# cbs228/sameold

Hardware: AMD Instinct MI355X
Metric: Msamples/s demodulated (batched 22.05 kHz channels) + % HBM roofline, 1/8 GPU (higher is better)
Workload: dtype f32

## Files before the change

### include/same_rx.h

```cpp
#ifndef SAME_RX_H
#define SAME_RX_H

#include <stddef.h>
#include <stdint.h>

#ifdef __cplusplus
extern "C" {
#endif

#define SAME_RX_ABI_VERSION 2

enum {
    SAME_OK = 0,
    SAME_EINVAL = -1,
    SAME_EDCLEN = -2,
    SAME_EAGCLIMITS = -3,
    SAME_EEQORDER = -4,
    SAME_ENODEVICE = -5,
    SAME_EHIP = -6,
    SAME_EOVERFLOW = -7,
    SAME_ENOMEM = -8,
    SAME_ERATE = -9,
    SAME_EKERNEL = -10
};
// ... 73 lines not shown
    SAME_BATCH_TRACE_SYMBOLS = 1u << 1,
    SAME_BATCH_GENERIC_KERNEL = 1u << 2,
    SAME_BATCH_TIME_PARALLEL = 1u << 3,
    SAME_BATCH_RELAXED = 1u << 4,
    SAME_BATCH_CALL_INVARIANT = 1u << 5,
    SAME_BATCH_MESSAGES_ONLY = 1u << 6
};
#define SAME_TP_EVENT_TOLERANCE_SYMBOLS 2

typedef struct same_batch same_batch;

int same_batch_new(const same_rx_builder *b, uint32_t n_channels, int device,
                   uint32_t flags, same_batch **out);
void same_batch_free(same_batch *rx);
int same_batch_reset(same_batch *rx);
int same_batch_reset_channels(same_batch *rx, const uint32_t *channels, size_t n);
uint64_t same_batch_channel_input_sample_counter(const same_batch *rx, uint32_t channel);
uint32_t same_batch_input_rate(const same_batch *rx);
uint32_t same_batch_n_channels(const same_batch *rx);
uint64_t same_batch_input_sample_counter(const same_batch *rx);
int same_batch_device(const same_batch *rx);

#define SAME_STREAM_OWN ((void *)(intptr_t)-1)
int same_batch_process_device(same_batch *rx, const float *d_x, size_t n_samples,
                              uint32_t layout, void *hip_stream);
int same_batch_set_call_window(same_batch *rx, uint32_t samples);
int same_batch_order_after(same_batch *rx, void *producer_stream);
int same_batch_process_device_i16(same_batch *rx, const int16_t *d_x, size_t n_samples,
                                  uint32_t layout, void *hip_stream);
int same_batch_process_host(same_batch *rx, const float *h_x, size_t n_samples, uint32_t layout);
int same_batch_process_host_i16(same_batch *rx, const int16_t *h_x, size_t n_samples, uint32_t layout);
int same_batch_process_device_ragged(same_batch *rx, const float *d_x, size_t n_rows, const uint32_t *counts,
                                     uint32_t layout, void *hip_stream);
int same_batch_process_device_ragged_i16(same_batch *rx, const int16_t *d_x, size_t n_rows, const uint32_t *counts,
                                         uint32_t layout, void *hip_stream);
int same_batch_process_host_ragged(same_batch *rx, const float *h_x, size_t n_rows, const uint32_t *counts, uint32_t layout);
int same_batch_process_host_ragged_i16(same_batch *rx, const int16_t *h_x, size_t n_rows, const uint32_t *counts,
                                       uint32_t layout);
int same_batch_flush(same_batch *rx);
int same_batch_sync(same_batch *rx);

int same_batch_poll_events(same_batch *rx, same_rx_event *out, size_t cap, size_t *n_out,
                           size_t *n_left);
size_t same_batch_pending_events(same_batch *rx);
int same_batch_peek_events(same_batch *rx, const same_rx_event **events, size_t *n);
int same_batch_drop_events(same_batch *rx, size_t n);
#define SAME_BURST_RECORD_BYTES 304
int same_batch_pack_bursts(same_batch *rx, uint32_t first_channel, uint8_t *out, size_t cap, size_t *n_records);

int same_batch_time_parallel_config(same_batch *rx, uint32_t max_chunks, uint32_t min_own_samples,
                                    uint32_t warmup_samples);
uint32_t same_batch_time_parallel_chunks(const same_batch *rx);
int same_batch_time_parallel_per_channel(const same_batch *rx);

int same_batch_transport_on_device(const same_batch *rx);

enum {
    SAME_AUDIO_FIRST = 1,
    SAME_AUDIO_END_MESSAGE = 2,
    SAME_AUDIO_END_FLUSH = 4,
    SAME_AUDIO_END_RESET = 8,
    SAME_AUDIO_TRUNCATED = 16
};
typedef struct same_audio_chunk {
    uint32_t channel, flags;
    uint64_t sample_counter;
    uint64_t n_samples;
    const float *samples;
} same_audio_chunk;
int same_batch_set_audio_capture(same_batch *rx, size_t samples_per_launch);
int same_batch_peek_audio(same_batch *rx, const same_audio_chunk **chunks, size_t *n);
int same_batch_drop_audio(same_batch *rx, size_t n);

typedef struct same_symbol_trace {
    uint64_t sample_counter;
    float zero, sym, err, samples_until_next_ted;
} same_symbol_trace;
int same_batch_read_trace(same_batch *rx, uint32_t channel, same_symbol_trace *out,
                          size_t cap, size_t *n_out);

int same_batch_last_kernel_ms(same_batch *rx, float *ms);
int same_batch_last_demod_kernel_ms(same_batch *rx, float *ms);
void same_batch_set_kernel_timing(same_batch *rx, int enable);
const char *same_batch_kernel_name(const same_batch *rx);

typedef struct same_rx same_rx;
int same_rx_build(const same_rx_builder *b, int device, same_rx **out);
void same_rx_free(same_rx *rx);
int same_rx_process(same_rx *rx, const float *x, size_t n, size_t *consumed, same_rx_event *ev);
int same_rx_flush(same_rx *rx, same_rx_event *msg);
int same_rx_reset(same_rx *rx);
uint32_t same_rx_input_rate(const same_rx *rx);
uint64_t same_rx_input_sample_counter(const same_rx *rx);

int same_synth_afsk_device(float *d_x, uint32_t n_channels, size_t n_samples,
                           uint32_t input_rate, uint64_t seed, float noise_sigma,
                           uint32_t flags, int device, void *hip_stream);
uint32_t same_synth_payload(uint64_t seed, uint32_t channel, uint8_t *out, uint32_t cap);
int same_synth_trials_device(float *d_x, uint32_t n_trials, uint32_t first_trial, size_t n_samples,
                             uint32_t input_rate, uint64_t seed, float ebn0_db_lo, float ebn0_db_step,
                             uint32_t n_grid, int device, void *hip_stream);

#ifdef __cplusplus
}
#endif
#endif
// ... 1 lines not shown
```

### sameold_amd/build.py

```python
from __future__ import annotations

import hashlib
import os
import re
import shutil
import subprocess
import sys

HERE = os.path.dirname(os.path.abspath(__file__))
CSRC = os.path.join(HERE, "csrc")
VARIANT = os.environ.get("SAME_BUILD_VARIANT", "")
LIB = os.path.join(HERE, f"libsame_rx.{VARIANT}.so" if VARIANT else "libsame_rx.so")
SOURCES = ["same_kernels.hip", "same_kernels_fast.hip", "same_kernels_pipe.hip", "same_kernels_relaxed.hip", "same_kernels_sym.hip", "same_kernels_sym_hi.hip", "same_synth.hip", "same_transport.hip", "same_capture.hip", "same_resample.hip", "same_batch.cpp", "same_select.cpp", "same_config.cpp", "same_transport.cpp", "same_place.cpp"]
SOURCE_FLAGS = {"same_kernels_sym_hi.hip": ["-mllvm", "-amdgpu-sched-strategy=max-ilp"],
                "same_kernels_pipe.hip": ["-mllvm", "-amdgpu-sched-strategy=max-ilp"]}
HEADERS = ["same_dev_common.h", "same_fast_common.h", "same_relaxed_common.h", "same_pipe_common.h", "same_profile.h", "same_device.h", "same_hipmem.h", "same_launch.h", "same_select.h", "same_config.h", "same_transport.h", "same_transport_dev.h", "same_capture_dev.h", "same_resets.h", "same_resample_dev.h", "same_resample_plan.h", "../../include/same_rx.h", "../../include/same_resample.h",
           "../../include/same_place.h", "samedec_main.cpp"]
SAMEDEC = os.path.join(HERE, "samedec_gpu")
ARCH = "gfx950"


def hipcc() -> str:
    for cand in (os.environ.get("HIPCC"), shutil.which("hipcc"), "/opt/rocm/bin/hipcc"):
        if cand and os.path.exists(cand):
            return cand
    raise RuntimeError("hipcc not found: the MI355X library cannot be built (there is no CPU build)")


def flags() -> list:
    return [
        f"--offload-arch={ARCH}", "-O3", "-std=c++17", "-fPIC",
        "-ffp-contract=off", "-fno-fast-math",
        "-fhip-fp32-correctly-rounded-divide-sqrt",
        "-fgpu-rdc" if False else "-fno-gpu-rdc",
        "-Wall", "-Wno-unused-function", "-Wno-unused-variable",
        "-x", "hip",
    ] + (["-DSAME_PROFILE=1"] if os.environ.get("SAME_PROFILE") else []) \
      + (["-DSAME_P3_MARKS=1"] if os.environ.get("SAME_P3_MARKS") else []) \
      + (["-DSAME_P1_SPLIT=1"] if os.environ.get("SAME_P1_SPLIT") else []) \
      + (["-DSAME_SYM_TL=1"] if os.environ.get("SAME_SYM_TL") else []) \
      + ([f"-DSYM_PRIOS=0x{os.environ['SAME_SYM_PRIOS']}"] if os.environ.get("SAME_SYM_PRIOS") else []) \
      + ([f"-DSYM_TL_GROUP={int(os.environ['SAME_SYM_TL_GROUP'])}u"] if os.environ.get("SAME_SYM_TL_GROUP") else []) \
      + [f"-D{d}" for d in os.environ.get("SAME_EXTRA_DEFS", "").split() if d] \
      + [f for f in os.environ.get("SAME_EXTRA_FLAGS", "").split() if f]


def source_hash() -> str:
    h = hashlib.sha256()
    for f in sorted(SOURCES + HEADERS):
        with open(os.path.join(CSRC, f), "rb") as fh:
            h.update(f.encode() + b"\0" + fh.read() + b"\0")
    h.update(" ".join(flags()).encode())
    h.update(repr(sorted(SOURCE_FLAGS.items())).encode())
    return h.hexdigest()


_MARK = re.compile(rb"SAME_SOURCE_HASH=([0-9a-f]{64})")


def built_hash(path: str = LIB):
    try:
        with open(path, "rb") as fh:
            m = _MARK.search(fh.read())
    except OSError:
        return None
    return m.group(1).decode() if m else None


def is_stale() -> bool:
# ... 55 lines not shown
```

### sameold_amd/csrc/same_batch.cpp

```cpp
#include <hip/hip_runtime.h>

#include <algorithm>
#include <chrono>
#include <cstdarg>
#include <cstdio>
#include <cstdlib>
#include <condition_variable>
#include <cstring>
#include <deque>
#include <functional>
#include <mutex>
#include <new>
#include <string>
#include <thread>
#include <utility>
#include <vector>

#include "../../include/same_rx.h"
#include "same_config.h"
#include "same_device.h"
#include "same_hipmem.h"
#include "same_launch.h"
#include "same_resets.h"
#include "same_transport.h"
// ... 145 lines not shown
                std::unique_lock<std::mutex> lk(mu_);
                cv_.wait(lk, [&] { return stop_ || generation_ != seen; });
                if (stop_) return;
                seen = generation_;
            }
            work();
        }
    }
    std::vector<std::thread> threads_;
    std::mutex mu_;
    std::condition_variable cv_, done_;
    const std::function<void(size_t)> *fn_ = nullptr;
    size_t next_ = 0, count_ = 0, pending_ = 0;
    uint64_t generation_ = 0;
    bool stop_ = false;
};

struct same_batch {
    same_rx_builder builder{};
    same::Params P{};
    same::State S{};
    int device = 0;
    uint32_t flags = 0;
    uint64_t counter = 0;
    hipStream_t own_stream = nullptr;
    hipStream_t last_stream = nullptr;
    same::DevBuf<float4> d_taps;
    same::DevBuf<void> d_state_blob;
    struct Slot {
        same::DevBuf<same::DevEvent> d_events;
        uint32_t event_cap() const { return (uint32_t)d_events.size(); }
        same::DevBuf<uint32_t> d_sort;
        same::PinnedBuf<uint32_t> h_sort;
        same::DevBuf<same::DevEvent> d_sorted;
        uint32_t sort_bins = 0;
        same::DevBuf<uint8_t> d_bursts;
        uint32_t burst_cap() const { return (uint32_t)(d_bursts.size() / same::kBurstCap); }
        same::DevBuf<uint32_t> d_counters;
        same::MappedBuf<uint32_t> h_counters;
        same::Event ev_start, ev_stop, ev_done, ev_planned;
        same::Event ev_k0, ev_k1;
        bool have_k = false;
        bool timed = false;
        same::PinnedBuf<void> h_events, h_bursts;
        bool in_flight = false;
        uint64_t seq = 0;
        uint64_t end_counter = 0;
        bool chunked = false;
        same::ChunkGeom geom{};
        uint64_t end_blocks = 0;
        same::DevBuf<uint64_t> d_handover;
        same::PinnedBuf<uint64_t> h_handover;
        bool per_channel = false;
        same::DevBuf<uint32_t> d_geom;
        same::PinnedBuf<uint32_t> h_geom;
        same::CoherentBuf<uint32_t> h_reset;
        same::CoherentBuf<uint32_t> h_counts;
        same::PinnedBuf<uint64_t> h_wake_up;
        bool dev_transport = false;
        same::CoherentBuf<same::DevMessage> h_near;
        uint32_t near_cap() const { return (uint32_t)h_near.size(); }
        same::DevBuf<same::DevMessage> d_msgs;
        uint32_t msg_cap() const { return (uint32_t)d_msgs.size(); }
        same::PinnedBuf<void> h_msgs;
        bool captured = false;
        same::DevBuf<same::cap::Span> d_spans;
        uint32_t span_cap() const { return (uint32_t)d_spans.size(); }
        same::DevBuf<float> d_pool;
        same::DevBuf<same::cap::Cursors> d_cap_cur;
        same::MappedBuf<same::cap::Cursors> h_cap_cur;
        same::PinnedBuf<void> h_spans, h_pool;
    } slot[2];
    struct TimePar {
        bool enabled = false;
        uint32_t max_chunks = 0, min_own = 0, warmup = 0;
        uint32_t cap_columns = 0;
        uint32_t carved_columns = 0;
        int carved_family = -1;
        same::Params Pv{};
        same::State Sv{};
        same::DevBuf<void> blob;
        same::DevBuf<void> blob_fresh;
        size_t fresh_bytes = 0;
        same::DevBuf<same::StateArrayDesc> d_desc_in, d_desc_out;
        uint32_t n_desc = 0;
        same::DevBuf<uint32_t> d_final_col;
        same::DevBuf<float> d_energy;
        same::DevBuf<float> d_hist;
        same::Event ev_plan_prev; bool plan_recorded = false;
        int knob_plan_stream = 0;
        int sort_mode = -1;
        uint32_t last_chunks = 1;
        bool last_per_channel = false;
        same::Family family = same::Family::kPipe;
        int knob_prologue = 0;
        std::vector<int64_t> sym_off;
        std::vector<TickSynth> synth;
    } tp;
    uint64_t launch_seq = 0;
    hipStream_t copy_stream = nullptr;
    struct Windowed {
        bool on = false;
        uint32_t window = 0;
        uint32_t fill = 0;
        same::DevBuf<void> d_buf;
        same::Event ev_buf;
        hipStream_t buf_stream = nullptr; bool buf_used = false;
        same::Event ev_read[2];
        uint64_t n_reads = 0;
        hipStream_t read_stream = nullptr;
    } inv;
    hipStream_t plan_stream = nullptr;
    float last_ms = 0.0f;
    bool overflowed = false;
    std::string record_path;
    bool kernel_fault = false;
    same::Request want;
    same::Mode mode;
    same::Choice plain;
    same::Params Pfm{};
    same::Family last_family = same::Family::kGeneric;
    bool sym_launched = false;
    bool debug = false;
    int host_threads = 0;
    same::DevBuf<void> d_stage, d_stage2;
    same::DevBuf<void> d_upload;
    same::DevBuf<void> d_zero;
    same::Event ev_order;
    bool timing = false;
    bool have_timing = false;
    float last_demod_ms = 0.0f;
    EventQueue queue;
    size_t queue_head = 0;
    ByteArena arena;
    std::vector<same_rx_event> peeked;
    bool peeked_valid = false;
    bool peeked_release = false;
    size_t peeked_head = 0;
    std::vector<size_t> burst_seq;
    size_t burst_seq_head = 0;
    std::vector<HarvestPart> parts;
    WorkerPool workers;
    std::vector<same::TransportHot> thot;
// ... 57 lines not shown

size_t carve_state(const same::Params &P, char *base, same::State &S)
{
    const size_t C = P.n_channels;
    Carver cv;
#define CARVE(field, type, count) \
    do { size_t o = cv.take<type>(count); if (base) S.field = reinterpret_cast<type *>(base + o); } while (0)
#define CARVE_ROWS(field, type, rows) CARVE(field, type, (size_t)(rows) * C);
    SAME_STATE_ARRAYS(CARVE_ROWS, P)
#undef CARVE_ROWS
    CARVE(fr_msg, uint8_t, (size_t)same::kBurstCap * C);
    if (P.trace_cap) {
        CARVE(trace_n, uint32_t, C);
        CARVE(trace, float, (size_t)P.trace_cap * 4 * C);
        CARVE(trace_idx, uint64_t, (size_t)P.trace_cap * C);
    }
#undef CARVE
    return (cv.off + 255) & ~size_t(255);
}

void list_state_arrays(const same::Params &P, const same::State &src, const same::State &dst,
                       std::vector<same::StateArrayDesc> &out)
{
    out.clear();
#define DESC_ROWS(field, type, rows)                                                                     \
    out.push_back(same::StateArrayDesc{reinterpret_cast<char *>(src.field), reinterpret_cast<char *>(dst.field), \
                                       (uint32_t)(rows), (uint32_t)(sizeof(type) / 4)});
    SAME_STATE_ARRAYS(DESC_ROWS, P)
#undef DESC_ROWS
    static_assert(same::kBurstCap % 4 == 0, "framer rows are copied in words");
    out.push_back(same::StateArrayDesc{reinterpret_cast<char *>(src.fr_msg), reinterpret_cast<char *>(dst.fr_msg), 1u,
                                       (uint32_t)(same::kBurstCap / 4)});
}

void read_knobs(same_batch *rx)
{
    auto num = [](const char *name, int unset) { const char *e = std::getenv(name); return e ? std::atoi(e) : unset; };
    auto tri = [](const char *name) { const char *e = std::getenv(name); return e ? (std::atoi(e) ? 1 : -1) : 0; };
    rx->P.knob_pipe = tri("SAME_PIPE");
    rx->P.knob_pipe_lanes = num("SAME_PIPE_LANES", 0);
    rx->P.knob_pipe_split = tri("SAME_PIPE_SPLIT");
#ifdef SAME_PROFILE
    rx->P.knob_mirror = tri("SAME_MIRROR");
    rx->P.knob_pipe_share = tri("SAME_PIPE_SHARE");
    rx->P.knob_prio = num("SAME_PIPE_PRIO", 0);
#endif
    rx->P.knob_fast_dense = tri("SAME_FAST_DENSE");
    rx->P.knob_sym = tri("SAME_SYM");
    rx->want.sym_max_channels = (uint32_t)std::max(0, num("SAME_SYM_MAX", 1 << 30));
    rx->debug = std::getenv("SAME_DEBUG") != nullptr;
    { const char *e = std::getenv("SAME_RECORD_HARVEST"); rx->record_path = e ? e : ""; }
    rx->host_threads = std::max(0, num("SAME_HOST_THREADS", 0));
    rx->tp.sort_mode = num("SAME_TP_SORT", -1);
    rx->tp.knob_plan_stream = tri("SAME_TP_PLAN_STREAM");
    rx->tp.knob_prologue = tri("SAME_TP_PROLOGUE");
    rx->want.knob_relaxed = tri("SAME_RELAXED");
    { const char *e = std::getenv("SAME_RELAXED_KERNEL"); rx->P.knob_relaxed_kernel = !e ? 0 : (std::strcmp(e, "solo") == 0 ? 1 : (std::strcmp(e, "duo") == 0 ? 2 : 0)); }
    { const char *e = std::getenv("SAME_TP_KERNEL"); rx->want.knob_tp_kernel = !e ? 0 : (std::strcmp(e, "wave") == 0 ? 2 : (std::strcmp(e, "pipe") == 0 ? 1 : 0)); }
}

int ensure_output(same_batch *rx, same_batch::Slot &sl, size_t n_samples, same::Output &O, size_t n_columns = 0)
{
    const size_t n_ch = n_columns ? n_columns : rx->P.n_channels;
    const double symbols = (double)n_samples * 520.83 / (double)rx->P.input_rate;
    const size_t per_chan_events = (size_t)(symbols / 8.0) + 16;
    const size_t per_chan_bursts = (size_t)(symbols / 160.0) + 4;
    size_t ecap = std::min<size_t>(per_chan_events * n_ch, 0x7fffffffu / sizeof(same::DevEvent));
    size_t bcap = std::min<size_t>(per_chan_bursts * n_ch, 0x7fffffffu / same::kBurstCap);
    HIP_TRY(sl.d_events.ensure(ecap));
    HIP_TRY(sl.d_bursts.ensure(bcap * same::kBurstCap));
    if (rx->dev_transport && !n_columns) {
        HIP_TRY(sl.d_msgs.ensure(std::min<size_t>(bcap + 2 * n_ch, 0x7fffffffu / sizeof(same::DevMessage))));
        if (!sl.h_near) HIP_TRY(sl.h_near.ensure(std::max<uint32_t>(4096u, (uint32_t)(n_ch / 4u))));
        if (rx->audio.per_launch)
            HIP_TRY(sl.d_spans.ensure(std::min<size_t>(n_ch + (size_t)sl.near_cap() + sl.msg_cap(), 0x7fffffffu / sizeof(same::cap::Span))));
    }
    HIP_TRY(sl.d_sorted.ensure(sl.d_events.size()));
    HIP_TRY(sl.d_sort.ensure(2 * n_ch + 1 + same::event_sort_extra_words((uint32_t)n_ch)));
    HIP_TRY(sl.h_sort.ensure(n_ch + 1));
    sl.sort_bins = (uint32_t)n_ch;
    O.events = sl.d_events; O.event_cap = sl.event_cap();
    O.bursts = sl.d_bursts; O.burst_cap = sl.burst_cap();
    O.n_events = sl.d_counters; O.n_bursts = sl.d_counters + 1; O.overflow = sl.d_counters + 2;
    return SAME_OK;
}

template <typename SampleT>
hipError_t launch_family(same::Family f, const same::Params &P, const same::State &S, const same::Output &O, const float4 *taps, const SampleT *x,
                         uint32_t n_blocks, uint64_t counter0, hipStream_t stream, const same::PipeChunks &pc = same::PipeChunks{})
{
    switch (f) {
    case same::Family::kSym: return same::launch_demod_sym(P, S, O, taps, x, n_blocks, counter0, stream, pc);
    case same::Family::kPipeFastmath: return same::launch_demod_pipe(P, S, O, taps, x, n_blocks, counter0, stream, pc, true);
    case same::Family::kPipe: return same::launch_demod_pipe(P, S, O, taps, x, n_blocks, counter0, stream, pc, false);
    case same::Family::kWaveRelaxed: return same::launch_demod_relaxed(P, S, O, taps, x, n_blocks, counter0, stream, pc);
    case same::Family::kFast: return same::launch_demod_fast(P, S, O, taps, x, n_blocks, counter0, stream);
    case same::Family::kGeneric: break;
    }
    return hipErrorInvalidValue;
}

void reset_channel_host(same_batch *rx, uint32_t c, uint64_t pos)
{
    if (!rx->thot.empty()) rx->tr(c).reset();
    if (rx->tp.enabled) {
        rx->tp.sym_off[c] = 0;
// ... 2 lines not shown
    }
    if (rx->h_wake) rx->h_wake[c] = 0;
}

int launch_pending_resets(same_batch *rx, same_batch::Slot &sl, hipStream_t stream)
{
    if (rx->resets.device.empty()) return SAME_OK;
    std::vector<uint32_t> &cols = rx->reset_cols;
    rx->resets.take_device(cols);
    const uint32_t n = (uint32_t)cols.size();
    if (n > sl.h_reset.size()) HIP_TRY(sl.h_reset.ensure(std::max<uint32_t>(256u, n + n / 2u)));
    std::memcpy(sl.h_reset, cols.data(), (size_t)n * sizeof(uint32_t));
    hipError_t e = same::launch_reset_columns(rx->P, rx->S, sl.h_reset.dev(), n, stream);
    if (e == hipSuccess && rx->dev_transport)
        e = same::launch_transport_reset(rx->d_thot, rx->d_tcold, rx->P.n_channels, sl.h_reset.dev(), n, 0, stream, rx->audio.d_rec);
    if (e != hipSuccess) return fail(SAME_EHIP, "channel reset launch failed: %s", hipGetErrorString(e));
    return SAME_OK;
}

void prepare_queue_append(same_batch *rx)
{
    rx->peeked_valid = false;
    release_stale_view(rx);
    if (rx->queue_head && rx->queue_head >= rx->queue.size() - rx->queue_head) {
        rx->queue_head = rx->queue.compact(rx->queue_head);
        size_t keep_from = rx->arena.base + rx->arena.size();
        for (size_t i = 0; i < rx->queue.size(); ++i)
            if (rx->queue.data()[i].n_bytes) { keep_from = (size_t)rx->queue.data()[i].payload; break; }
        rx->arena.compact(keep_from - rx->arena.base);
    }
}

struct HarvestTimes { std::chrono::steady_clock::time_point sorted, replayed; uint32_t n_threads = 1; };
struct HarvestInput {
    const uint32_t *first;
    same::DevEvent *events;
    const uint8_t *bursts;
    const uint64_t *handover;
    const uint32_t *geom;
};
int harvest_host(same_batch *rx, same_batch::Slot &sl, const HarvestInput &in, uint32_t n_events, uint32_t n_bursts, std::vector<uint32_t> &rearm,
                 HarvestTimes &times)
{
    const bool dbg = rx->debug;
    const same::DevEvent *evs = in.events;
    const uint8_t *bursts = in.bursts;
    const uint32_t n_ch = rx->P.n_channels;
    const uint32_t n_bins = sl.chunked ? sl.geom.n_chunks * n_ch : n_ch;
    std::vector<uint32_t> first(in.first, in.first + n_bins + 1u);
    same::DevEvent *evs_mut = in.events;
    const uint32_t n_real = first[n_bins];
    if (n_real > n_events) return fail(SAME_EHIP, "internal: event sort counted %u of %u events", n_real, n_events);
    struct Identity { uint32_t operator[](uint32_t i) const { return i; } } order;
    if (dbg && sl.chunked && sl.per_channel) {
        const same::ChunkGeom &g = sl.geom;
        const uint32_t *own = in.geom, *rows = in.geom + n_bins;
        double len_sum = 0, run_sum = 0; uint64_t len_max = 0, run_max = 0, n_len = 0, n_run = 0, n_inf = 0, n_late = 0;
        uint32_t worst_c = 0;
        for (uint32_t k = 0; k + 1u < g.n_chunks; ++k)
            for (uint32_t c = 0; c < n_ch; ++c) {
                const uint64_t end = own[(size_t)(k + 1u) * n_ch + c], len = end - rows[(size_t)k * n_ch + c];
                len_sum += (double)len; if (len > len_max) { len_max = len; worst_c = c; } ++n_len;
                const uint64_t h = in.handover[(size_t)k * n_ch + c];
                if (h == same::kNoHandover) { ++n_inf; continue; }
                const uint64_t run = h - g.counter0 > end ? h - g.counter0 - end : 0;
                run_sum += (double)run; run_max = std::max(run_max, run); ++n_run; n_late += run > 2u * g.block_len;
            }
        std::fprintf(stderr, "[same] longest piece on channel %u, its cuts:", worst_c);
        for (uint32_t k = 0; k < g.n_chunks; ++k) std::fprintf(stderr, " %u", own[(size_t)k * n_ch + worst_c]);
        std::fprintf(stderr, "\n");
        std::fprintf(stderr, "[same] per-channel chunks: length mean %.0f max %llu samples; run-on mean %.0f max %llu, %llu of %llu columns ran on "
                             "more than two blocks, %llu never handed over\n", len_sum / std::max<uint64_t>(n_len, 1), (unsigned long long)len_max,
                     run_sum / std::max<uint64_t>(n_run, 1), (unsigned long long)run_max, (unsigned long long)n_late, (unsigned long long)n_run,
                     (unsigned long long)n_inf);
    }
    std::vector<uint32_t> chan_first;
    if (sl.chunked) {
        chan_first.assign(n_ch + 1u, 0u);
        for (uint32_t k = 0; k < sl.geom.n_chunks; ++k)
            for (uint32_t c = 0; c < n_ch; ++c) chan_first[c + 1u] += first[k * n_ch + c + 1u] - first[k * n_ch + c];
        for (uint32_t c = 0; c < n_ch; ++c) chan_first[c + 1u] += chan_first[c];
    }
    const std::vector<uint32_t> &cfirst = sl.chunked ? chan_first : first;
    const bool link_only = (rx->flags & SAME_BATCH_LINK_ONLY) != 0;
    const bool tp = rx->tp.enabled;
    times.sorted = std::chrono::steady_clock::now();

    using Part = HarvestPart;
    const double sps = (double)rx->P.input_rate / 520.83;
    const uint64_t interburst = same::max_interburst_symbols(), history = same::max_history_duration();
    const bool msgs_only = rx->messages_only;
    auto push_transport = [&](Part &part, const same_rx_event &tev, uint32_t c) {
        if (msgs_only && tev.kind != SAME_TRANSPORT_MSG_START && tev.kind != SAME_TRANSPORT_MSG_END) return;
        QEvent q{};
        q.kind = tev.kind; q.channel = c; q.sample_counter = rx->resets.rebase(c, tev.sample_counter); q.symbol_count = tev.symbol_count;
        q.len = tev.len; q.aux = tev.aux; q.aux2 = tev.aux2;
        q.n_bytes = std::min<uint32_t>(tev.len, SAME_EVENT_MAX_BYTES);
        if (tev.kind != SAME_TRANSPORT_MSG_START) q.n_bytes = 0;
        q.payload = part.bytes.size();
        if (q.n_bytes) part.bytes.insert(part.bytes.end(), tev.bytes, tev.bytes + q.n_bytes);
        part.out.push_back(q);
    };
    auto feed = [&](Part &part, same_rx_event &tev, const same::DevEvent &d, uint32_t c, int64_t off) {
        const uint64_t sym = (uint64_t)((int64_t)d.symbol_count + off);
        auto poll = [&](uint64_t psym, uint64_t pt) {
            if (rx->tr(c).on_link_event(same::kDevTick, pt, psym, nullptr, 0, rx->P.input_rate, &tev)) push_transport(part, tev, c);
        };
        if (tp && !link_only) {
            HP(1);
            rx->tp.synth[c].run_until(sym, d.sample_counter, sps, rx->tr(c).force_eom_at(), poll);
        }
        QEvent q{};
        const uint8_t *payload = nullptr;
        {
        HP(2);
        q.kind = d.kind; q.channel = c; q.sample_counter = rx->resets.rebase(c, d.sample_counter); q.symbol_count = sym;
        if (d.kind == SAME_LINK_BURST) {
            q.len = d.burst_len;
            if (d.burst_slot < n_bursts) {
                q.n_bytes = std::min<uint32_t>(d.burst_len, SAME_EVENT_MAX_BYTES);
                payload = bursts + (size_t)d.burst_slot * same::kBurstCap;
                q.payload = part.bytes.size();
                if (!msgs_only) part.bytes.insert(part.bytes.end(), payload, payload + q.n_bytes);
            } else {
                q.len = 0;
            }
            if (!msgs_only) part.bursts.push_back((uint32_t)part.out.size());
        }
        if (d.kind <= SAME_LINK_BURST && !msgs_only) part.out.push_back(q);
        }
        if (!link_only) {
#ifdef SAME_HOST_PROF
            HpScope hp_tr(d.kind == SAME_LINK_BURST ? 3 : 4);
#endif
            if (rx->tr(c).on_link_event(d.kind, d.sample_counter, sym, payload, q.n_bytes, rx->P.input_rate, &tev)) push_transport(part, tev, c);
            if (!tp && rx->tr(c).force_eom_dirty()) part.rearm.push_back(c);
        }
        { HP(5); if (tp && d.kind <= SAME_LINK_BURST) rx->tp.synth[c].after_event(d.kind, sym, d.sample_counter, interburst, history); }
    };
    auto stitch = [&](Part &part, same_rx_event &ev, uint32_t c) {
        const same::ChunkGeom &g = sl.geom;
        const uint64_t *hand = in.handover;
        const uint32_t *own = sl.per_channel ? in.geom : nullptr, *rows = sl.per_channel ? in.geom + n_bins : nullptr;
        auto owner_of = [&](uint64_t h) -> uint32_t {
            if (!own) return g.owner_of(h);
            uint32_t k = 0;
            while (k + 1u < g.n_chunks && g.counter0 + own[(size_t)(k + 1u) * n_ch + c] <= h) ++k;
            return k;
        };
        TickSynth &ts = rx->tp.synth[c];
        int64_t off = rx->tp.sym_off[c];
        uint32_t cur = 0;
        uint64_t keep_after = 0;
        for (;;) {
            const uint32_t col = cur * n_ch + c;
            const uint64_t h = hand[col];
            const uint64_t upto = std::min(h, sl.end_blocks);
            bool rebased = cur == 0;
            for (uint32_t i = first[col]; i < first[col + 1u]; ++i) {
                const same::DevEvent &d = evs[order[i]];
                if (d.sample_counter <= keep_after) continue;
                if (d.sample_counter > upto) break;
                if (!rebased) {
                    const int64_t est = (int64_t)ts.a_sym + (int64_t)((double)(d.sample_counter - ts.a_t) / sps + 0.5);
                    off = est - (int64_t)d.symbol_count;
                    rebased = true;
                }
                feed(part, ev, d, c, off);
            }
            if (!rebased) {
                const uint64_t row0 = rows ? g.counter0 + rows[col] : g.counter0 + (uint64_t)cur * g.stride_blocks * g.block_len;
                const int64_t est_end = (int64_t)ts.a_sym + (int64_t)((double)(sl.end_blocks - ts.a_t) / sps + 0.5);
                off = est_end - (int64_t)((double)(sl.end_blocks - row0) / sps + 0.5);
            }
            if (h == same::kNoHandover) break;
            const uint32_t nxt = owner_of(h);
            if (nxt <= cur) break;
            const uint32_t ncol = nxt * n_ch + c;
            uint32_t st = 0, j = first[ncol];
            for (; j < first[ncol + 1u] && evs[order[j]].sample_counter <= h; ++j)
                if (evs[order[j]].kind <= SAME_LINK_BURST) st = evs[order[j]].kind;
            keep_after = h;
            if (st == SAME_LINK_READING || st == SAME_LINK_BURST) {
                for (; j < first[ncol + 1u]; ++j)
                    if (evs[order[j]].kind == SAME_LINK_NO_CARRIER) { keep_after = evs[order[j]].sample_counter; break; }
            } else if (st == SAME_LINK_SEARCHING && ts.link == SAME_LINK_NO_CARRIER) {
                same::DevEvent inj{};
                inj.channel = ncol; inj.kind = SAME_LINK_SEARCHING; inj.sample_counter = h;
                inj.symbol_count = ts.a_sym + (uint64_t)((double)(h > ts.a_t ? h - ts.a_t : 0) / sps + 0.5);
                inj.burst_slot = 0xffffffffu;
                feed(part, ev, inj, c, 0);
            }
            cur = nxt;
        }
        for (uint32_t i = first[c]; i < first[c + 1u]; ++i)
            if (evs[order[i]].sample_counter > sl.end_blocks) feed(part, ev, evs[order[i]], c, off);
        rx->tp.sym_off[c] = off;
    };
    auto run_range = [&](uint32_t c0, uint32_t c1, Part &part) {
        part.out.clear(); part.bytes.clear(); part.rearm.clear(); part.bursts.clear();
        part.out.reserve((size_t)(cfirst[c1] - cfirst[c0]) * 3 / 2 + 4);
        same_rx_event ev;
        std::memset(&ev, 0, sizeof(ev));
        for (uint32_t c = c0; c < c1; ++c) {
            if (!link_only && c + 1u < c1) {
                __builtin_prefetch(&rx->thot[c + 1u]);
                if (!sl.chunked) {
                    bool burst = false;
                    for (uint32_t k = first[c + 1u]; k < first[c + 2u]; ++k) burst |= evs[k].kind == SAME_LINK_BURST;
                    const char *nx = reinterpret_cast<const char *>(&rx->tcold[c + 1u]);
                    if (burst) for (size_t o = 0; o < sizeof(same::TransportCold); o += 64) __builtin_prefetch(nx + o);
                }
            }
            { HP(0);
            for (uint32_t col = c; col < n_bins; col += n_ch)
                if (first[col + 1u] - first[col] > 1u)
                    std::sort(evs_mut + first[col], evs_mut + first[col + 1u],
                              [](const same::DevEvent &a, const same::DevEvent &b) { return a.channel < b.channel; });
            }
            if (sl.chunked) stitch(part, ev, c);
            else
                for (uint32_t k = first[c]; k < first[c + 1u]; ++k)
                    feed(part, ev, evs[order[k]], c, tp ? rx->tp.sym_off[c] : 0);
            if (tp && !link_only) {
                TickSynth &ts = rx->tp.synth[c];
                if (ts.link == SAME_LINK_NO_CARRIER && sl.end_counter > ts.a_t) {
                    const uint64_t sym_end = ts.a_sym + (uint64_t)((double)(sl.end_counter - ts.a_t) / sps);
                    auto poll = [&](uint64_t psym, uint64_t pt) {
                        if (rx->tr(c).on_link_event(same::kDevTick, pt, psym, nullptr, 0, rx->P.input_rate, &ev)) push_transport(part, ev, c);
                    };
                    ts.run_until(sym_end + 1u, sl.end_counter + 1u, sps, rx->tr(c).force_eom_at(), poll);
                }
            }
        }
    };
    uint32_t n_threads = 1;
    if (n_real >= 16384u && n_ch >= 64u) {
        const unsigned hw = std::thread::hardware_concurrency();
        n_threads = std::min<uint32_t>({32u, std::max(16u, hw / 8u), hw ? hw : 1u, n_ch / 32u});
        if (rx->host_threads > 0) n_threads = (uint32_t)rx->host_threads;
    }
    if (rx->parts.size() < n_threads) rx->parts.resize(n_threads);
    std::vector<Part> &parts = rx->parts;
    for (Part &p : parts) { p.out.clear(); p.bytes.clear(); p.rearm.clear(); p.bursts.clear(); }
    if (n_threads == 1) {
        run_range(0, n_ch, parts[0]);
    } else {
        std::vector<uint32_t> cut(n_threads + 1u, n_ch);
        cut[0] = 0;
        for (uint32_t t = 1; t < n_threads; ++t) {
            const uint32_t target = (uint32_t)((uint64_t)n_real * t / n_threads);
            cut[t] = (uint32_t)(std::lower_bound(cfirst.begin(), cfirst.end(), target) - cfirst.begin());
            cut[t] = std::min(std::max(cut[t], cut[t - 1u]), n_ch);
        }
        rx->workers.run(n_threads, [&](size_t t) { run_range(cut[t], cut[t + 1u], parts[t]); });
    }
    times.replayed = std::chrono::steady_clock::now();
    times.n_threads = n_threads;
    size_t total = 0, total_bytes = 0;
    for (const Part &p : parts) { total += p.out.size(); total_bytes += p.bytes.size(); }
    prepare_queue_append(rx);
    QEvent *dst = rx->queue.grow(total);
    if (total && !dst) return fail(SAME_ENOMEM, "event queue");
    uint8_t *bdst = rx->arena.grow(total_bytes);
    if (total_bytes && !bdst) return fail(SAME_ENOMEM, "event payloads");
    {
        size_t at = 0, bat = 0;
        if (rx->burst_seq_head > 4096 && rx->burst_seq_head * 2 > rx->burst_seq.size()) {
            rx->burst_seq.erase(rx->burst_seq.begin(), rx->burst_seq.begin() + (std::ptrdiff_t)rx->burst_seq_head);
            rx->burst_seq_head = 0;
        }
        const size_t seq0 = rx->queue.base + (size_t)(dst - rx->queue.data());
        const size_t byte0 = rx->arena.base + (size_t)(bdst - rx->arena.data());
        struct Job { QEvent *q; uint8_t *b; Part *p; size_t byte_off; };
        std::vector<Job> jobs;
        for (size_t t = 0; t < parts.size(); ++t) {
            Part &p = parts[t];
            if (p.out.empty()) continue;
            for (uint32_t i : p.bursts) rx->burst_seq.push_back(seq0 + at + i);
            jobs.push_back(Job{dst + at, bdst + bat, &p, byte0 + bat});
            at += p.out.size(); bat += p.bytes.size();
        }
        rx->workers.run(jobs.size(), [&](size_t j) {
            const Job &job = jobs[j];
            for (QEvent &q : job.p->out) q.payload += job.byte_off;
            std::memcpy(job.q, job.p->out.data(), job.p->out.size() * sizeof(QEvent));
            if (!job.p->bytes.empty()) std::memcpy(job.b, job.p->bytes.data(), job.p->bytes.size());
        });
    }
    for (Part &p : parts) rearm.insert(rearm.end(), p.rearm.begin(), p.rearm.end());
    return SAME_OK;
}

struct HarvestFileHeader {
    uint64_t magic;
    uint32_t n_channels, n_bins, n_events, n_bursts, chunked, per_channel, flags, input_rate, tp_enabled, pad;
    same::ChunkGeom geom;
    uint64_t end_blocks, end_counter;
};
constexpr uint64_t kHarvestMagic = 0x3156524845'4d4153ull;
int record_harvest(same_batch *rx, same_batch::Slot &sl, uint32_t n_events, uint32_t n_bursts, const char *path)
{
    if (sl.seq != 3u) return SAME_OK;
    std::FILE *f = std::fopen(path, "wb");
    if (!f) return fail(SAME_EINVAL, "SAME_RECORD_HARVEST: cannot write %s", path);
    const uint32_t n_ch = rx->P.n_channels, n_bins = sl.chunked ? sl.geom.n_chunks * n_ch : n_ch;
    HarvestFileHeader h{};
    h.magic = kHarvestMagic;
    h.n_channels = n_ch; h.n_bins = n_bins; h.n_events = n_events; h.n_bursts = n_bursts;
    h.chunked = sl.chunked; h.per_channel = sl.per_channel; h.flags = rx->flags; h.input_rate = rx->P.input_rate; h.tp_enabled = rx->tp.enabled;
    h.geom = sl.geom; h.end_blocks = sl.end_blocks; h.end_counter = sl.end_counter;
    bool ok = std::fwrite(&h, sizeof(h), 1, f) == 1;
    ok = ok && std::fwrite(sl.h_sort, sizeof(uint32_t), (size_t)n_bins + 1, f) == (size_t)n_bins + 1;
    ok = ok && (!n_events || std::fwrite(sl.h_events, sizeof(same::DevEvent), n_events, f) == n_events);
    ok = ok && (!n_bursts || std::fwrite(sl.h_bursts, same::kBurstCap, n_bursts, f) == n_bursts);
    if (sl.chunked) {
        ok = ok && std::fwrite(sl.h_handover, sizeof(uint64_t), n_bins, f) == n_bins;
        if (sl.per_channel) ok = ok && std::fwrite(sl.h_geom, sizeof(uint32_t), (size_t)2 * n_bins, f) == (size_t)2 * n_bins;
    }
    std::fclose(f);
    return ok ? SAME_OK : fail(SAME_EINVAL, "SAME_RECORD_HARVEST: short write to %s", path);
}

hipError_t grow_pinned(same::PinnedBuf<void> &b, size_t need)
{
    return need <= b.size() ? hipSuccess : b.ensure(need + need / 2 + 4096);
}

AudioChunk *audio_grow(same_batch *rx, size_t n_chunks, size_t n_samples, float **samples_at, uint64_t *at)
{
    same_batch::Audio &A = rx->audio;
    if (A.head && A.head >= A.queue.size() - A.head) {
        A.head = A.queue.compact(A.head);
        const uint64_t keep_from = A.queue.size() ? A.queue.data()[0].at : A.samples.base + A.samples.size();
        A.samples.compact((size_t)(keep_from - A.samples.base));
    }
    AudioChunk *dst = A.queue.grow(n_chunks);
    if (n_chunks && !dst) return nullptr;
    float *sdst = A.samples.grow(n_samples);
    if (n_samples && !sdst) { A.queue.n -= n_chunks; return nullptr; }
    *samples_at = sdst;
    *at = A.samples.base + (A.samples.size() - n_samples);
    return dst;
}

int audio_end_reset(same_batch *rx, const std::vector<uint32_t> &chans, uint64_t pos)
{
    same_batch::Audio &A = rx->audio;
    if (!A.per_launch) return SAME_OK;
    size_t n = 0;
    for (uint32_t c : chans) n += A.open[c];
    if (!n) return SAME_OK;
    float *sdst = nullptr;
    uint64_t at = 0;
    AudioChunk *dst = audio_grow(rx, n, 0, &sdst, &at);
    if (!dst) return fail(SAME_ENOMEM, "audio queue");
    for (uint32_t c : chans) {
        if (!A.open[c]) continue;
        *dst++ = AudioChunk{c, SAME_AUDIO_END_RESET, rx->resets.rebase(c, pos), 0, at};
        A.open[c] = 0;
    }
    return SAME_OK;
}

int harvest_audio(same_batch *rx, same_batch::Slot &sl)
{
    sl.captured = false;
    same_batch::Audio &A = rx->audio;
    const same::cap::Cursors cur = *sl.h_cap_cur.get();
    if (cur.overflow) rx->overflowed = true;
    const uint32_t n_spans = std::min(cur.n_spans, sl.span_cap());
// ... 102 lines not shown
    const uint32_t C = rx->P.n_channels;
    HIP_TRY(sl.h_wake_up.ensure(C));
    same_batch::Slot &other = rx->slot[(&sl - rx->slot) ^ 1];
    const int oi = (int)(&other - rx->slot);
    for (uint32_t c = 0; c < C; ++c) {
        const uint64_t w = rx->h_wake[c];
        sl.h_wake_up[c] = w && other.in_flight ? w + rx->resets.pending_shift(oi, c) : w;
    }
    if (other.in_flight) {
        HIP_TRY(hipMemcpyAsync(rx->S.wake_sample, sl.h_wake_up, (size_t)C * sizeof(uint64_t), hipMemcpyHostToDevice, rx->last_stream));
        HIP_TRY(hipEventRecord(other.ev_done, rx->last_stream));
    } else {
        HIP_TRY(hipMemcpyAsync(rx->S.wake_sample, sl.h_wake_up, (size_t)C * sizeof(uint64_t), hipMemcpyHostToDevice, rx->copy_stream));
        HIP_TRY(hipStreamSynchronize(rx->copy_stream));
    }
    return SAME_OK;
}

int harvest_slot(same_batch *rx, same_batch::Slot &sl)
{
    if (!sl.in_flight) return SAME_OK;
    const bool dbg = rx->debug;
    auto t_begin = std::chrono::steady_clock::now();
    HIP_TRY(hipEventSynchronize(sl.ev_done));
    sl.in_flight = false;
    if (sl.timed) {
        HIP_TRY(hipEventElapsedTime(&rx->last_ms, sl.ev_start, sl.ev_stop));
        rx->last_demod_ms = rx->last_ms;
        if (sl.have_k) HIP_TRY(hipEventElapsedTime(&rx->last_demod_ms, sl.ev_k0, sl.ev_k1));
        rx->have_timing = true;
    }
    auto t_waited = std::chrono::steady_clock::now();
    const uint32_t n_events = std::min(sl.h_counters[0], sl.event_cap());
    if (dbg)
        std::fprintf(stderr, "[same] harvest: %u device events (%u bursts), cap %u/%u\n", sl.h_counters[0],
                     sl.h_counters[1], sl.event_cap(), sl.burst_cap());
    const uint32_t n_bursts = std::min(sl.h_counters[1], sl.burst_cap());
    if (sl.h_counters[2] & (3u | same::kMessageLogOverflow)) rx->overflowed = true;
    if (sl.h_counters[2] & 4u) rx->kernel_fault = true;
    if (sl.dev_transport) return harvest_messages(rx, sl, t_begin, t_waited);
    const size_t ev_bytes = (size_t)n_events * sizeof(same::DevEvent), bu_bytes = (size_t)n_bursts * same::kBurstCap;
    HIP_TRY(grow_pinned(sl.h_events, ev_bytes));
    HIP_TRY(grow_pinned(sl.h_bursts, bu_bytes));
    const uint32_t n_ch = rx->P.n_channels;
    const uint32_t n_bins = sl.chunked ? sl.geom.n_chunks * n_ch : n_ch;
    if (n_bins != sl.sort_bins) return fail(SAME_EINVAL, "internal: event sort made for %u columns, launch has %u", sl.sort_bins, n_bins);
    HIP_TRY(hipMemcpyAsync(sl.h_sort, sl.d_sort + n_bins, ((size_t)n_bins + 1) * sizeof(uint32_t), hipMemcpyDeviceToHost, rx->copy_stream));
    if (n_events) HIP_TRY(hipMemcpyAsync(sl.h_events, sl.d_sorted, ev_bytes, hipMemcpyDeviceToHost, rx->copy_stream));
    HIP_TRY(hipStreamSynchronize(rx->copy_stream));
    if (n_bursts) HIP_TRY(hipMemcpyAsync(sl.h_bursts, sl.d_bursts, bu_bytes, hipMemcpyDeviceToHost, rx->copy_stream));
    if (sl.chunked) {
        HIP_TRY(hipMemcpyAsync(sl.h_handover, sl.d_handover, (size_t)n_bins * sizeof(uint64_t), hipMemcpyDeviceToHost, rx->copy_stream));
        if (sl.per_channel)
            HIP_TRY(hipMemcpyAsync(sl.h_geom, sl.d_geom, (size_t)2 * n_bins * sizeof(uint32_t), hipMemcpyDeviceToHost, rx->copy_stream));
    }
    if (n_bursts || sl.chunked) HIP_TRY(hipStreamSynchronize(rx->copy_stream));
    auto t_copied = std::chrono::steady_clock::now();
    if (!rx->record_path.empty()) { const int rrc = record_harvest(rx, sl, n_events, n_bursts, rx->record_path.c_str()); if (rrc != SAME_OK) return rrc; }
    std::vector<uint32_t> rearm;
    HarvestTimes times;
    const HarvestInput in{sl.h_sort, static_cast<same::DevEvent *>(sl.h_events.get()), static_cast<const uint8_t *>(sl.h_bursts.get()),
                          sl.h_handover, sl.h_geom};
    int rc = harvest_host(rx, sl, in, n_events, n_bursts, rearm, times);
    if (rc) return rc;
    {
        const int si = (int)(&sl - rx->slot);
        const same::ResetLedger::SlotShift &sh = rx->resets.shift_due(si);
        if (!rx->thot.empty())
            for (size_t i = 0; i < sh.channels.size(); ++i)
                if (rx->tr(sh.channels[i]).shift_force_eom(sh.by[i])) rearm.push_back(sh.channels[i]);
        rx->resets.done_shift(si);
    }
    {
        const int si = (int)(&sl - rx->slot);
        const std::vector<uint32_t> &due = rx->resets.host_due(si);
        for (uint32_t c : due) reset_channel_host(rx, c, rx->resets.rec_pos(si));
        rx->resets.done_host(si);
    }
    if (!rearm.empty()) {
        if (!rx->h_wake) {
            HIP_TRY(rx->h_wake.ensure(rx->P.n_channels));
            std::memset(rx->h_wake, 0, (size_t)rx->P.n_channels * sizeof(uint64_t));
        }
        for (uint32_t c : rearm) rx->h_wake[c] = rx->tr(c).force_eom_at();
        if (rx->wake_ordered) {
            int rc2 = upload_wake_ordered(rx, sl);
            if (rc2) return rc2;
        } else {
        HIP_TRY(hipMemcpyAsync(rx->S.wake_sample, rx->h_wake, (size_t)rx->P.n_channels * sizeof(uint64_t), hipMemcpyHostToDevice, rx->copy_stream));
        HIP_TRY(hipStreamSynchronize(rx->copy_stream));
        }
    }
    if (dbg) {
        auto t_end = std::chrono::steady_clock::now();
        auto ms = [](auto a, auto b) { return std::chrono::duration<double, std::milli>(b - a).count(); };
        std::fprintf(stderr, "[same] harvest timing: wait %.2f ms, copy %.2f ms, sort %.2f ms, replay on %u threads %.2f ms, "
                             "queue %.2f ms\n",
                     ms(t_begin, t_waited), ms(t_waited, t_copied), ms(t_copied, times.sorted), times.n_threads,
                     ms(times.sorted, times.replayed), ms(times.replayed, t_end));
    }
    return SAME_OK;
}

int harvest(same_batch *rx)
{
    same_batch::Slot *order[2] = {&rx->slot[0], &rx->slot[1]};
    if (order[0]->seq > order[1]->seq) std::swap(order[0], order[1]);
    for (same_batch::Slot *sl : order) {
        int rc = harvest_slot(rx, *sl);
        if (rc) return rc;
// ... 81 lines not shown
    uint32_t m = 0;
    uint32_t row_off = 0;
};

struct RaggedLaunch {
    uint32_t row0 = 0;
    size_t n_lock = 0;
};


int begin_launch(same_batch *rx, same_batch::Slot &sl, const same_batch::Slot &prev, hipStream_t stream)
{
    int rc = harvest_slot(rx, sl);
    if (rc) return rc;
    if (prev.in_flight && rx->last_stream != stream) HIP_TRY(hipStreamWaitEvent(stream, prev.ev_done, 0));
    return launch_pending_resets(rx, sl, stream);
}

int begin_timing(same_batch *rx, same_batch::Slot &sl, hipStream_t stream)
{
    sl.timed = rx->timing;
    if (sl.timed) HIP_TRY(hipEventRecord(sl.ev_start, stream));
    return SAME_OK;
}

int tp_reserve(same_batch *rx, same_batch::Slot &sl, uint32_t columns, size_t n, const same::PipeChunks &pc, uint32_t block_len, same::Output &O)
{
    int rc = ensure_wide_state(rx, columns);
    if (rc) return rc;
    rc = ensure_output(rx, sl, std::min<size_t>(n, 3 * (size_t)pc.nominal_blocks * block_len + 65536), O, columns);
    if (rc) return rc;
    return ensure_handover(sl, columns);
}

int tp_start(same_batch *rx, same_batch::Slot &sl, uint32_t columns, const char *layout, hipStream_t stream, bool *sort_bins_empty)
{
    same_batch::TimePar &tp = rx->tp;
    const uint32_t C = rx->P.n_channels;
    *sort_bins_empty = false;
    if (tp.knob_prologue >= 0) {
        HIP_TRY(same::launch_tp_prologue(tp.blob, tp.blob_fresh, tp.fresh_bytes, sl.d_handover, sl.d_sort, columns, sl.d_counters, stream));
        *sort_bins_empty = sl.sort_bins == columns;
    } else {
        HIP_TRY(same::launch_counters(sl.d_counters, sl.h_counters.dev(), 0, stream));
        HIP_TRY(same::launch_init_state(tp.Pv, tp.Sv, 0, stream, C));
        HIP_TRY(same::launch_fill_u64(sl.d_handover, columns, same::kNoHandover, stream));
    }
    if (rx->debug) std::fprintf(stderr, "[same] time-parallel launch: %u columns (%s), start-up: %s\n", columns, layout,
                                tp.knob_prologue >= 0 ? "prologue kernel" : "separate launches");
    HIP_TRY(same::launch_copy_state_columns(tp.d_desc_in, tp.n_desc, C, columns, nullptr, C, stream));
    return SAME_OK;
}

int tp_hand_back(same_batch *rx, same_batch::Slot &sl, const same::ChunkGeom &geom, const uint32_t *own_start, hipStream_t stream)
{
    same_batch::TimePar &tp = rx->tp;
    const uint32_t C = rx->P.n_channels;
    if (own_start) HIP_TRY(same::launch_chunk_final_column_pc(sl.d_handover, own_start, C, geom.n_chunks, rx->counter, tp.d_final_col, stream));
    else HIP_TRY(same::launch_chunk_final_column(sl.d_handover, C, geom, tp.d_final_col, stream));
    HIP_TRY(same::launch_copy_state_columns(tp.d_desc_out, tp.n_desc, geom.n_chunks * C, C, tp.d_final_col, C, stream));
    return SAME_OK;
}

template <typename SampleT>
int demod_tail(same_batch *rx, const same::Output &O, const SampleT *rows, size_t n, uint64_t counter0, hipStream_t stream)
{
    const hipError_t e = same::launch_demod(rx->P, rx->S, O, rx->d_taps, rows, (uint32_t)n, counter0, stream);
    if (e != hipSuccess) return fail(SAME_EHIP, "demod kernel launch failed: %s", hipGetErrorString(e));
    return SAME_OK;
}
int demod_tail_corner(same_batch *rx, const same::Output &O, const float *corner, size_t pitch, size_t r, uint64_t counter0, hipStream_t stream)
{
    const uint32_t C = rx->P.n_channels;
    HIP_TRY(rx->d_stage.ensure(r * C * sizeof(float)));
    HIP_TRY(rx->d_stage2.ensure(r * C * sizeof(float)));
    float *staged = static_cast<float *>(rx->d_stage.get()), *rows = static_cast<float *>(rx->d_stage2.get());
    HIP_TRY(hipMemcpy2DAsync(staged, r * sizeof(float), corner, pitch * sizeof(float), r * sizeof(float), C, hipMemcpyDeviceToDevice, stream));
    const hipError_t e = same::launch_transpose(staged, rows, C, (uint32_t)r, stream);
    if (e != hipSuccess) return fail(SAME_EHIP, "demod kernel launch failed: %s", hipGetErrorString(e));
    return demod_tail(rx, O, rows, r, counter0, stream);
}

template <typename SampleT>
int end_launch(same_batch *rx, same_batch::Slot &sl, same_batch::Slot &prev, hipStream_t stream, const SampleT *rows, size_t n,
               bool sort_bins_empty, const RaggedLaunch *rl = nullptr)
{
    if (sl.timed) HIP_TRY(hipEventRecord(sl.ev_stop, stream));
    HIP_TRY(same::launch_event_sort(sl.d_events, sl.d_counters, sl.event_cap(), sl.sort_bins, sl.d_sort, sl.d_sort + sl.sort_bins,
                                    sl.d_sorted, stream, sort_bins_empty));
    sl.dev_transport = rx->dev_transport && !sl.chunked;
    rx->last_dev_transport = sl.dev_transport;
    if (sl.dev_transport) {
        same::TransportLaunch T{};
        T.n_channels = rx->P.n_channels; T.input_rate = rx->P.input_rate;
        T.first = sl.d_sort + sl.sort_bins; T.sorted = sl.d_sorted; T.counters = sl.d_counters;
        T.bursts = sl.d_bursts; T.burst_cap = sl.burst_cap();
        T.hot = rx->d_thot; T.cold = rx->d_tcold; T.wake_sample = rx->S.wake_sample;
        T.near = sl.h_near.dev(); T.near_cap = sl.near_cap();
        T.log = sl.d_msgs; T.log_cap = sl.msg_cap(); T.log_cursor = sl.d_counters + 3; T.overflow = sl.d_counters + 2;
        sl.captured = rx->audio.per_launch != 0;
        if (sl.captured) {
            same::cap::Launch &K = T.cap;
            const uint64_t fa = rx->audio.flush_at;
            K.start = rx->counter; K.n_rows = (uint32_t)n;
            K.flush_row = fa >= rx->counter + n ? same::cap::kNoFlush : (uint32_t)(fa > rx->counter ? fa - rx->counter : 0);
            K.rec = rx->audio.d_rec; K.spans = sl.d_spans; K.span_cap = sl.span_cap();
            K.n_spans = &sl.d_cap_cur->n_spans; K.pool_used = &sl.d_cap_cur->pool_used; K.pool_cap = rx->audio.per_launch;
            K.overflow = &sl.d_cap_cur->overflow;
        }
        if (rl && rl->n_lock < n)
            HIP_TRY(same::launch_transport_ragged(T, sl.h_counts.dev(), rl->row0, (uint32_t)n, stream));
// ... 17 lines not shown
}

template <typename SampleT>
int process_time_major_launches(same_batch *rx, const SampleT *d_x, size_t n_samples, hipStream_t stream, const Ragged *rg = nullptr)
{
    const size_t kMaxChunk = std::min<size_t>((size_t)1 << 22, (size_t)rx->P.input_rate * 45);
    size_t done = 0;
    while (done < n_samples) {
        const size_t n = std::min(kMaxChunk, n_samples - done);
        same_batch::Slot &sl = rx->slot[rx->launch_seq & 1];
        same_batch::Slot &prev = rx->slot[(rx->launch_seq & 1) ^ 1];
        int rc = begin_launch(rx, sl, prev, stream);
        if (rc) return rc;
        size_t n_lock = n;
        if (rg) {
            const size_t row0 = (size_t)rg->row_off + done;
            n_lock = rg->m > row0 ? std::min<size_t>(rg->m - row0, n) : 0;
            const uint32_t C = rx->P.n_channels;
            HIP_TRY(sl.h_counts.ensure(C));
            std::memcpy(sl.h_counts, rg->counts, (size_t)C * sizeof(uint32_t));
            rx->ragged_by.resize(C);
            for (uint32_t c = 0; c < C; ++c) {
                const size_t have = rg->counts[c] > row0 ? std::min<size_t>(rg->counts[c] - row0, n) : 0;
                rx->ragged_by[c] = (uint32_t)(n - have);
            }
        }
        same::ChunkGeom geom{};
        same::PipeChunks pc{};
        const uint32_t n_chunks = rg ? 1u : plan_chunks(rx, n, geom, pc);
        rx->tp.last_chunks = n_chunks;
        sl.have_k = false;
        bool sort_bins_empty = false;
        same::Output O{};
        if (n_chunks > 1u) {
            const uint32_t C = rx->P.n_channels, columns = n_chunks * C;
            const size_t fbk = geom.block_len;
            rc = tp_reserve(rx, sl, columns, n, pc, geom.block_len, O);
            if (rc) return rc;
            pc.handover = sl.d_handover;
            same_batch::TimePar &tp = rx->tp;
            rc = begin_timing(rx, sl, stream);
            if (rc) return rc;
            rc = tp_start(rx, sl, columns, "time-major", stream, &sort_bins_empty);
            if (rc) return rc;
            const SampleT *xp = d_x + done * C;
            const uint32_t total_blocks = (uint32_t)(n / fbk);
            const hipError_t e = launch_family(tp.family, tp.Pv, tp.Sv, O, rx->d_taps, xp, total_blocks, rx->counter, stream, pc);
            rx->last_family = tp.family;
            if (e != hipSuccess) return fail(SAME_EHIP, "time-parallel demod kernel launch failed: %s", hipGetErrorString(e));
            rc = tp_hand_back(rx, sl, geom, nullptr, stream);
            if (rc) return rc;
            const size_t n_whole = (size_t)total_blocks * fbk;
            if (n_whole < n && (rc = demod_tail(rx, O, xp + n_whole * C, n - n_whole, rx->counter + n_whole, stream)) != SAME_OK) return rc;
            sl.chunked = true; sl.per_channel = false;
            sl.geom = geom;
            sl.end_blocks = rx->counter + n_whole;
            rx->tp.last_per_channel = false;
        } else {
        sl.chunked = false; sl.per_channel = false;
        rc = ensure_output(rx, sl, n, O);
        if (rc) return rc;
        HIP_TRY(same::launch_counters(sl.d_counters, sl.h_counters.dev(), 0, stream));
        rc = begin_timing(rx, sl, stream);
        if (rc) return rc;
        const SampleT *xp = d_x + done * rx->P.n_channels;
        hipError_t e = hipSuccess;
        const same::Choice &plain = rx->plain;
        const size_t fb = plain.block_len;
        const size_t n_fast = fb ? (n_lock / fb) * fb : 0;
        if (n_fast) {
            e = launch_family(plain.family, same::is_fastmath(plain.family) ? rx->Pfm : rx->P, rx->S, O, rx->d_taps, xp, (uint32_t)(n_fast / fb), rx->counter, stream);
            if (e != hipSuccess) return fail(SAME_EHIP, "%s launch failed: %s", same::family_name(plain.family, rx->P.block_len), hipGetErrorString(e));
            rx->sym_launched |= plain.family == same::Family::kSym;
        }
        rx->last_family = plain.family == same::Family::kSym && !rx->sym_launched ? same::Family::kPipeFastmath : plain.family;
        if (n_fast < n_lock &&
            (rc = demod_tail(rx, O, xp + n_fast * rx->P.n_channels, n_lock - n_fast, rx->counter + n_fast, stream)) != SAME_OK) return rc;
        if (n_lock < n) {
            e = same::launch_demod_ragged(rx->P, rx->S, O, rx->d_taps, xp + n_lock * rx->P.n_channels, (uint32_t)(n - n_lock), sl.h_counts.dev(),
                                          (uint32_t)(rg->row_off + done + n_lock), rx->counter + n_lock, stream);
            if (e != hipSuccess) return fail(SAME_EHIP, "ragged demod kernel launch failed: %s", hipGetErrorString(e));
        }
        }
        const RaggedLaunch rl{rg ? (uint32_t)(rg->row_off + done) : 0u, n_lock};
        rc = end_launch(rx, sl, prev, stream, d_x + done * rx->P.n_channels, n, sort_bins_empty, rg ? &rl : nullptr);
        if (rc) return rc;
        done += n;
    }
    return SAME_OK;
}

constexpr uint32_t kInvWindow = 18432;
constexpr uint32_t kInvWindowTimeParallel = 73728;
static int inv_buffer_wait(same_batch *rx, hipStream_t stream)
{
    same_batch::Windowed &iv = rx->inv;
    if (iv.buf_used && iv.buf_stream != stream) HIP_TRY(hipStreamWaitEvent(stream, iv.ev_buf, 0));
    return SAME_OK;
}
static int inv_buffer_done(same_batch *rx, hipStream_t stream)
{
    same_batch::Windowed &iv = rx->inv;
    HIP_TRY(iv.ev_buf.ensure());
    HIP_TRY(hipEventRecord(iv.ev_buf, stream));
    iv.buf_stream = stream; iv.buf_used = true;
    return SAME_OK;
}
static int inv_copy(const float *d_x, float *dst, size_t n, hipStream_t stream)
{
    HIP_TRY(hipMemcpyAsync(dst, d_x, n * sizeof(float), hipMemcpyDeviceToDevice, stream));
    return SAME_OK;
}
// ... 49 lines not shown
{
    same_batch::Windowed &iv = rx->inv;
    if (iv.n_reads) HIP_TRY(hipEventSynchronize(iv.ev_read[(iv.n_reads - 1) & 1]));
    return SAME_OK;
}
template <typename SampleT>
int process_time_major(same_batch *rx, const SampleT *d_x, size_t n_samples, hipStream_t stream)
{
    same_batch::Windowed &iv = rx->inv;
    if (!iv.on) return process_time_major_launches(rx, d_x, n_samples, stream);
    const size_t C = rx->P.n_channels;
    size_t pos = 0;
    if (iv.fill) {
        const size_t take = std::min<size_t>(iv.window - iv.fill, n_samples);
        int rc = inv_append(rx, d_x, take, stream);
        if (rc) return rc;
        pos = take;
        if (iv.fill < iv.window) return SAME_OK;
        rc = inv_launch_waiting(rx, stream);
        if (rc) return rc;
    }
    while (n_samples - pos >= iv.window) {
        int rc = process_time_major_launches(rx, d_x + pos * C, iv.window, stream);
        if (rc) return rc;
        pos += iv.window;
    }
    if (pos < n_samples) return inv_append(rx, d_x + pos * C, n_samples - pos, stream);
    return SAME_OK;
}

int process_channel_major_native(same_batch *rx, const float *d_x, size_t n, hipStream_t stream)
{
    same_batch::TimePar &tp = rx->tp;
    if (!tp.enabled || n > ((size_t)1 << 22)) return 0;
    if (rx->P.ntaps != 42u) return 0;
    same::ChunkGeom geom{};
    same::PipeChunks pc{};
    const uint32_t n_chunks = plan_chunks(rx, n, geom, pc, same::tp_native_column_cap(rx->P, rx->mode, tp.max_chunks), true);
    if (n_chunks < 2u) return 0;
    const uint32_t C = rx->P.n_channels, columns = n_chunks * C, fb = geom.block_len;
    const bool wave = tp.family == same::Family::kWaveRelaxed;
    const same::Params Pv = same::wide_params(rx->P, columns, same::is_fastmath(tp.family), true);
    const size_t n_call = n;
    n -= n % fb;
    if (n_call % 4 != 0 || ((uintptr_t)d_x & 15u) != 0u || n < 64u * (size_t)same::tp_scout_block() || n / same::tp_scout_block() > 7000u || n_chunks > 63u || C % same::kWave != 0u) return 0;
    if (wave ? fb % 2 != 0 : (fb % 4 != 0 || same::pipe_workgroup_channels(Pv) != (uint32_t)same::kWave)) return 0;
    same_batch::Slot &sl = rx->slot[rx->launch_seq & 1];
    same_batch::Slot &prev = rx->slot[(rx->launch_seq & 1) ^ 1];
    int rc = begin_launch(rx, sl, prev, stream);
    if (rc) return rc;
    same::Output O{};
    rc = tp_reserve(rx, sl, columns, n, pc, fb, O);
    if (rc) return rc;
    HIP_TRY(sl.d_geom.ensure((size_t)5 * columns + 3 * (columns / same::kWave)));
    HIP_TRY(sl.h_geom.ensure((size_t)2 * columns));
    same::TpPlan plan{};
    plan.channels = C; plan.n_chunks = n_chunks; plan.block_len = fb;
    {
        const double sps = (double)rx->P.input_rate / 520.83;
        const uint32_t warm = tp.warmup ? tp.warmup : (uint32_t)(40.0 * sps + 0.5);
        plan.warmup_samples = std::min(geom.warmup_blocks, (warm + fb - 1u) / fb) * fb;
    }
    plan.whole_samples = (uint32_t)n; plan.in_samples = n_call;
    plan.scout_blocks = (uint32_t)(n / same::tp_scout_block());
    HIP_TRY(tp.d_energy.ensure((size_t)C * plan.scout_blocks));
    uint32_t *d_own = sl.d_geom, *d_row0 = sl.d_geom + columns, *d_nom = sl.d_geom + 2 * (size_t)columns,
             *d_perm = sl.d_geom + 3 * (size_t)columns, *d_wg = sl.d_geom + 4 * (size_t)columns,
             *d_wg2 = d_wg + columns / same::kWave, *d_perm2 = d_wg2 + 2 * (columns / same::kWave);
    const bool pair_groups = tp.sort_mode == 2 && tp.family == same::Family::kSym;
    const int sort_mode = pair_groups ? 0 : (tp.sort_mode >= 0 ? (tp.sort_mode ? 1 : 0) : (same::tp_more_than_one_round(columns) ? 1 : 0));
    rc = begin_timing(rx, sl, stream);
    if (rc) return rc;
    const bool lpt = sort_mode != 0 || pair_groups;
    const bool side = stream == rx->own_stream && tp.knob_plan_stream >= 0;
    hipStream_t ps = side ? rx->plan_stream : stream;
    if (tp.plan_recorded) HIP_TRY(hipStreamWaitEvent(ps, tp.ev_plan_prev, 0));
    HIP_TRY(same::launch_tp_plan(d_x, plan, tp.d_energy, d_own, d_row0, d_nom, d_perm, d_wg, sort_mode != 0, ps,
                                 lpt ? d_perm2 : nullptr, lpt ? d_wg2 : nullptr, pair_groups));
    HIP_TRY(tp.ev_plan_prev.ensure());
    HIP_TRY(hipEventRecord(tp.ev_plan_prev, ps));
    tp.plan_recorded = true;
    if (side) {
        HIP_TRY(hipEventRecord(sl.ev_planned, ps));
        HIP_TRY(hipStreamWaitEvent(stream, sl.ev_planned, 0));
    }
    if (lpt) { d_perm = d_perm2; d_wg = d_wg2; }
    bool sort_bins_empty = false;
    rc = tp_start(rx, sl, columns, "channel-major", stream, &sort_bins_empty);
    if (rc) return rc;
    pc.handover = sl.d_handover;
    pc.col_row0 = d_row0; pc.col_nominal = d_nom; pc.wg_blocks = d_wg; pc.col_perm = (sort_mode != 0 || pair_groups) ? d_perm : nullptr;
    pc.in_samples = n_call; pc.whole_samples = (uint32_t)n;
    pc.hist_scratch = nullptr;
    if (pc.col_perm && tp.family == same::Family::kSym) {
        HIP_TRY(tp.d_hist.ensure((size_t)columns * same::kSquelchHist));
        pc.hist_scratch = tp.d_hist;
    }
    sl.have_k = sl.timed;
    if (sl.timed) HIP_TRY(hipEventRecord(sl.ev_k0, stream));
    const hipError_t e = launch_family(tp.family, tp.Pv, tp.Sv, O, rx->d_taps, d_x, (uint32_t)(n / fb), rx->counter, stream, pc);
    rx->last_family = tp.family;
    if (e != hipSuccess) return fail(SAME_EHIP, "time-parallel demod kernel launch failed: %s", hipGetErrorString(e));
    if (sl.timed) HIP_TRY(hipEventRecord(sl.ev_k1, stream));
    rc = tp_hand_back(rx, sl, geom, d_own, stream);
    if (rc) return rc;
    if (n < n_call && (rc = demod_tail_corner(rx, O, d_x + n, n_call, n_call - n, rx->counter + n, stream)) != SAME_OK) return rc;
    sl.chunked = true; sl.per_channel = true;
    sl.geom = geom;
    sl.end_blocks = rx->counter + n;
    tp.last_chunks = n_chunks; tp.last_per_channel = true;
    rc = end_launch<float>(rx, sl, prev, stream, nullptr, n_call, sort_bins_empty);
    return rc ? rc : 1;
}
int process_channel_major_native(same_batch *, const int16_t *, size_t, hipStream_t) { return 0; }

template <typename SampleT, typename Launch>
int transpose_in_slabs(same_batch *rx, const SampleT *d_x, size_t pitch, size_t n_rows, hipStream_t stream, Launch &&launch)
{
    const uint32_t C = rx->P.n_channels;
    for (same_batch::Slot &sl : rx->slot)
        if (sl.in_flight && rx->last_stream != stream) HIP_TRY(hipStreamWaitEvent(stream, sl.ev_done, 0));
    const size_t slab = std::min<size_t>(n_rows, (size_t)65520);
    HIP_TRY(rx->d_stage2.ensure(slab * C * sizeof(SampleT)));
    for (size_t t0 = 0; t0 < n_rows; t0 += slab) {
        const size_t n = std::min(slab, n_rows - t0);
        HIP_TRY(rx->d_stage.ensure(n * C * sizeof(SampleT)));
        SampleT *staged = static_cast<SampleT *>(rx->d_stage.get()), *rows = static_cast<SampleT *>(rx->d_stage2.get());
        HIP_TRY(hipMemcpy2DAsync(staged, n * sizeof(SampleT), d_x + t0, pitch * sizeof(SampleT), n * sizeof(SampleT), C,
                                 hipMemcpyDeviceToDevice, stream));
        const hipError_t e = same::launch_transpose(staged, rows, C, (uint32_t)n, stream);
        if (e != hipSuccess) return fail(SAME_EHIP, "transpose launch failed: %s", hipGetErrorString(e));
        const int rc = launch(rows, n, t0);
        if (rc) return rc;
    }
    return SAME_OK;
}

template <typename SampleT>
int process_device_on(same_batch *rx, const SampleT *d_x, size_t n_samples, uint32_t layout, hipStream_t stream);
template <typename SampleT>
int process_device_any(same_batch *rx, const SampleT *d_x, size_t n_samples, uint32_t layout, void *hip_stream)
{
    if (!rx || (!d_x && n_samples)) return fail(SAME_EINVAL, "null argument");
    if (n_samples == 0) return SAME_OK;
    HIP_TRY(hipSetDevice(rx->device));
    hipStream_t stream = hip_stream == SAME_STREAM_OWN ? rx->own_stream : (hipStream_t)hip_stream;
    if (!rx->inv.on) return process_device_on(rx, d_x, n_samples, layout, stream);
    int rc = inv_reads_begin(rx, stream);
    if (rc == SAME_OK) rc = process_device_on(rx, d_x, n_samples, layout, stream);
    const int rc_end = inv_reads_end(rx, stream);
    return rc ? rc : rc_end;
}
template <typename SampleT>
int process_device_on(same_batch *rx, const SampleT *d_x, size_t n_samples, uint32_t layout, hipStream_t stream)
{
    if (layout == SAME_LAYOUT_TIME_MAJOR) return process_time_major(rx, d_x, n_samples, stream);
    if (layout != SAME_LAYOUT_CHANNEL_MAJOR) return fail(SAME_EINVAL, "unknown layout %u", layout);
    const int done = rx->inv.on ? 0 : process_channel_major_native(rx, d_x, n_samples, stream);
    if (done) return done < 0 ? done : SAME_OK;
    return transpose_in_slabs(rx, d_x, n_samples, n_samples, stream,
// ... 550 lines not shown
}

int same_batch_read_trace(same_batch *rx, uint32_t channel, same_symbol_trace *out, size_t cap, size_t *n_out)
{
    if (!rx || !n_out) return fail(SAME_EINVAL, "null argument");
    if (!rx->P.trace_cap) return fail(SAME_EINVAL, "batch was not created with SAME_BATCH_TRACE_SYMBOLS");
    if (channel >= rx->P.n_channels) return fail(SAME_EINVAL, "channel out of range");
    HIP_TRY(hipSetDevice(rx->device));
    int rc = harvest(rx);
    if (rc) return rc;
    uint32_t n = 0;
    HIP_TRY(hipMemcpy(&n, rx->S.trace_n + channel, sizeof(n), hipMemcpyDeviceToHost));
    n = std::min(n, rx->P.trace_cap);
    n = (uint32_t)std::min<size_t>(n, cap);
    std::vector<float> f((size_t)n * 4);
    std::vector<uint64_t> idx(n);
    if (n) {
        HIP_TRY(hipMemcpy(f.data(), rx->S.trace + (size_t)channel * rx->P.trace_cap * 4, f.size() * sizeof(float), hipMemcpyDeviceToHost));
        HIP_TRY(hipMemcpy(idx.data(), rx->S.trace_idx + (size_t)channel * rx->P.trace_cap, n * sizeof(uint64_t), hipMemcpyDeviceToHost));
    }
    for (uint32_t i = 0; i < n; ++i) {
        out[i].sample_counter = idx[i];
        out[i].zero = f[4 * i]; out[i].sym = f[4 * i + 1]; out[i].err = f[4 * i + 2];
        out[i].samples_until_next_ted = f[4 * i + 3];
    }
    *n_out = n;
    return SAME_OK;
}

void same_batch_set_kernel_timing(same_batch *rx, int enable) { if (rx) { rx->timing = enable != 0; rx->have_timing = false; } }
int same_batch_last_kernel_ms(same_batch *rx, float *ms)
{
    if (!rx || !ms) return fail(SAME_EINVAL, "null argument");
    if (!rx->have_timing) return fail(SAME_EINVAL, "no timed launch yet");
    *ms = rx->last_ms;
    return SAME_OK;
}
int same_batch_last_demod_kernel_ms(same_batch *rx, float *ms)
{
    if (!rx || !ms) return fail(SAME_EINVAL, "null argument");
    if (!rx->have_timing) return fail(SAME_EINVAL, "no timed launch yet");
    *ms = rx->last_demod_ms;
    return SAME_OK;
}
int same_batch_time_parallel_config(same_batch *rx, uint32_t max_chunks, uint32_t min_own_samples, uint32_t warmup_samples)
{
    if (!rx) return fail(SAME_EINVAL, "null handle");
    if (!rx->tp.enabled) return fail(SAME_EINVAL, "batch was not created with SAME_BATCH_TIME_PARALLEL");
    rx->tp.max_chunks = max_chunks; rx->tp.min_own = min_own_samples; rx->tp.warmup = warmup_samples;
    return SAME_OK;
}
uint32_t same_batch_time_parallel_chunks(const same_batch *rx) { return rx ? rx->tp.last_chunks : 0; }
int same_batch_transport_on_device(const same_batch *rx) { return rx && rx->last_dev_transport ? 1 : 0; }
int same_batch_time_parallel_per_channel(const same_batch *rx) { return rx && rx->tp.last_chunks > 1u && rx->tp.last_per_channel ? 1 : 0; }

const char *same_batch_kernel_name(const same_batch *rx)
{
    return rx ? same::family_name(rx->last_family, rx->P.block_len) : "";
}


long same_debug_harvest_replay(const char *path, int threads, int reps, double *ms_out)
{
    if (!path || reps <= 0 || !ms_out) return -(long)fail(SAME_EINVAL, "null argument");
    std::FILE *f = std::fopen(path, "rb");
    if (!f) return -(long)fail(SAME_EINVAL, "cannot read %s", path);
    HarvestFileHeader h{};
    bool ok = std::fread(&h, sizeof(h), 1, f) == 1 && h.magic == kHarvestMagic && h.n_bins >= h.n_channels && h.n_channels > 0;
    std::vector<uint32_t> first, geom;
    std::vector<same::DevEvent> ev0, ev;
    std::vector<uint8_t> bursts;
    std::vector<uint64_t> hand0, hand;
    if (ok) {
        first.resize((size_t)h.n_bins + 1); ev0.resize(h.n_events); bursts.resize((size_t)h.n_bursts * same::kBurstCap);
        ok = std::fread(first.data(), sizeof(uint32_t), first.size(), f) == first.size();
        ok = ok && (!h.n_events || std::fread(ev0.data(), sizeof(same::DevEvent), h.n_events, f) == h.n_events);
        ok = ok && (!h.n_bursts || std::fread(bursts.data(), same::kBurstCap, h.n_bursts, f) == h.n_bursts);
        if (ok && h.chunked) {
            hand0.resize(h.n_bins);
            ok = std::fread(hand0.data(), sizeof(uint64_t), h.n_bins, f) == h.n_bins;
            if (ok && h.per_channel) { geom.resize((size_t)2 * h.n_bins); ok = std::fread(geom.data(), sizeof(uint32_t), geom.size(), f) == geom.size(); }
        }
    }
    std::fclose(f);
    if (ok) {
        ok = first[h.n_bins] <= h.n_events && h.n_bins % h.n_channels == 0;
        for (size_t i = 0; ok && i < (size_t)h.n_bins; ++i) ok = first[i] <= first[i + 1];
        for (size_t i = 0; ok && i < ev0.size(); ++i)
            ok = (ev0[i].burst_slot == 0xffffffffu || ev0[i].burst_slot < h.n_bursts) && (ev0[i].kind == same::kDevEventNone || ev0[i].kind <= 8u);
        if (ok && h.chunked) {
            ok = h.geom.n_chunks >= 1 && (uint64_t)h.geom.n_chunks * h.n_channels == h.n_bins && h.geom.block_len >= 1 && h.geom.stride_blocks >= 1;
            for (size_t i = 0; ok && h.per_channel && i < geom.size(); ++i) ok = geom[i] <= 0x7fffffffu;
        } else if (ok) {
            ok = h.n_bins == h.n_channels;
        }
    }
    if (!ok) return -(long)fail(SAME_EINVAL, "%s is not a (consistent) harvest record", path);
    same_batch *rx = new (std::nothrow) same_batch;
    if (!rx) return -(long)fail(SAME_ENOMEM, "out of memory");
    rx->P.n_channels = h.n_channels; rx->P.input_rate = h.input_rate; rx->flags = h.flags;
    if (std::getenv("SAME_REPLAY_LINK_ONLY")) rx->flags |= SAME_BATCH_LINK_ONLY;
    rx->tp.enabled = h.tp_enabled != 0; rx->host_threads = threads;
    if (!(h.flags & SAME_BATCH_LINK_ONLY)) { rx->thot.resize(h.n_channels); rx->tcold.resize(h.n_channels); }
    if (rx->tp.enabled) { rx->tp.sym_off.assign(h.n_channels, 0); rx->tp.synth.assign(h.n_channels, TickSynth{}); }
    rx->resets.init(h.n_channels);
    same_batch::Slot &sl = rx->slot[0];
    ev = ev0; hand = hand0;
    const HarvestInput in{first.data(), ev.data(), bursts.data(), hand.data(), geom.data()};
    sl.chunked = h.chunked != 0; sl.per_channel = h.per_channel != 0; sl.sort_bins = h.n_bins;
    const uint64_t span = h.end_counter - h.geom.counter0;
    const double sps = (double)h.input_rate / 520.83;
    const uint64_t span_sym = (uint64_t)((double)span / sps);
    long produced = 0;
    int rc = SAME_OK;
    for (int r = 0; r < reps && rc == SAME_OK; ++r) {
        const uint64_t dt = span * (uint64_t)r, ds = span_sym * (uint64_t)r;
        for (size_t i = 0; i < ev0.size(); ++i) { ev[i] = ev0[i]; ev[i].sample_counter += dt; if (!sl.chunked) ev[i].symbol_count += ds; }
        for (size_t i = 0; i < hand0.size(); ++i) hand[i] = hand0[i] == same::kNoHandover ? hand0[i] : hand0[i] + dt;
        sl.geom = h.geom; sl.geom.counter0 += dt;
        sl.end_blocks = h.end_blocks + dt; sl.end_counter = h.end_counter + dt;
        std::vector<uint32_t> rearm;
        HarvestTimes times;
        const auto t0 = std::chrono::steady_clock::now();
        rc = harvest_host(rx, sl, in, h.n_events, h.n_bursts, rearm, times);
        ms_out[r] = std::chrono::duration<double, std::milli>(std::chrono::steady_clock::now() - t0).count();
        produced = (long)(rx->queue.size() - rx->queue_head);
        rx->queue_head = rx->queue.size();
        rx->burst_seq_head = rx->burst_seq.size();
    }
#ifdef SAME_HOST_PROF
    { uint64_t tot = 0; for (int k = 0; k < 7; ++k) tot += g_hp[k];
      for (int k = 0; k < 7; ++k) std::fprintf(stderr, "[same prof] %-24s %8.3f Mclk per harvest (%4.1f %% of the instrumented parts)\n", g_hp_name[k], (double)g_hp[k] / reps / 1e6, tot ? 100.0 * (double)g_hp[k] / (double)tot : 0.0); }
#endif
    delete rx;
    return rc == SAME_OK ? produced : -(long)rc;
}

}

struct same_rx {
    same_batch *batch = nullptr;
    uint64_t reported = 0;
    uint64_t zeros_until = 0;
    std::deque<same_rx_event> events;
};

static int rx_pump(same_rx *rx)
{
    same_rx_event buf[64];
    for (;;) {
        size_t n = 0, left = 0;
        int rc = same_batch_poll_events(rx->batch, buf, 64, &n, &left);
        if (rc) return rc;
        for (size_t i = 0; i < n; ++i) rx->events.push_back(buf[i]);
        if (!left) return SAME_OK;
    }
}

extern "C" {

int same_rx_build(const same_rx_builder *b, int device, same_rx **out)
{
// ... 113 lines not shown
```

### sameold_amd/csrc/same_device.h

```cpp
#pragma once

#include <stddef.h>
#include <stdint.h>

namespace same {

constexpr int kWave = 64;
constexpr int kMaxEqTaps = 16;
constexpr int kBurstCap = 288;
constexpr int kSquelchHist = 64;
constexpr int kMaxTaps = 512;

struct Params {
    uint32_t n_channels;
    uint32_t input_rate;
    uint32_t dc_len;
    float dc_inv_len;
    float dc_k;
    float agc_bw, agc_min, agc_max, agc_gain0;
    uint32_t ntaps;
    uint32_t win_ring;
    float samples_per_ted, period_min, period_max;
    float alpha_unlocked, beta_unlocked, alpha_locked, beta_locked;
    uint32_t sync_word, sq_max_errors;
// ... 32 lines not shown
    F_EQ_BITS_SHIFT = 16,
    F_EQ_BITS_MASK = 0xffu << 16,
};
constexpr int kTickRing = 8;

struct State {
    float *dc_ff_ring;
    float *dc_fb_ring;
    float *dc_sum0, *dc_sum1;
    float *agc_gain;
    float *win_ring;
    uint32_t *ted_clock;
    float *until_next_ted;
    float *ted_h0, *ted_h1, *ted_h2;
    float *period_avg, *period_inst;
    uint32_t *sq_data;
    float *sq_power;
    uint32_t *sq_phist;
    uint32_t *sq_fill;
    int32_t *sq_clock;
    uint64_t *sq_symbols;
    float *sq_hist;
    float *eq_ffc, *eq_fbc;
    float *eq_ffw, *eq_fbw;
    uint32_t *eq_word, *eq_count;
    float *eq_snap_ffc, *eq_snap_fbc, *eq_snap_ffw, *eq_snap_fbw;
    uint32_t *fr_word, *fr_count, *fr_invalid, *fr_len;
    uint8_t *fr_msg;
    uint32_t *flags;
    uint64_t *tk_next;
    uint64_t *tk_last;
    uint64_t *tk_ring;
    uint32_t *tk_n;
    uint64_t *wake_sample;
    uint64_t *wake_fired;
    uint32_t *trace_n;
    float *trace;
    uint64_t *trace_idx;
};

struct PipeChunks {
    uint32_t n_chunks;
    uint32_t in_channels;
    uint32_t stride_blocks;
    uint32_t nominal_blocks;
    uint64_t *handover;
    const uint32_t *col_row0;
    const uint32_t *col_nominal;
    const uint32_t *wg_blocks;
    const uint32_t *col_perm;
    float *hist_scratch;
    uint64_t in_samples;
    uint32_t whole_samples;
};

struct ChunkGeom {
    uint64_t counter0;
    uint32_t n_chunks, block_len, stride_blocks, warmup_blocks;
#if defined(__HIPCC__)
    __host__ __device__
#endif
    uint32_t owner_of(uint64_t h) const
    {
        const uint64_t blocks = (h - counter0) / block_len;
        if (blocks < warmup_blocks) return 0u;
        const uint64_t k = (blocks - warmup_blocks) / stride_blocks;
        return k >= n_chunks ? n_chunks - 1u : (uint32_t)k;
    }
#if defined(__HIPCC__)
    __host__ __device__
#endif
    uint64_t own_start(uint32_t k) const
    { return k == 0u ? counter0 : counter0 + ((uint64_t)k * stride_blocks + warmup_blocks) * block_len; }
};
constexpr uint64_t kNoHandover = ~0ull;

struct StateArrayDesc { char *src; char *dst; uint32_t rows; uint32_t elem_words; };

constexpr uint32_t kDevEventNone = 0xffffffffu;
struct DevEvent {
    uint32_t channel;
    uint32_t kind;
    uint64_t sample_counter;
    uint64_t symbol_count;
    uint32_t burst_len;
    uint32_t burst_slot;
};

constexpr uint32_t kDevMessageText = 272;
struct DevMessage {
    uint32_t channel;
    uint32_t kind;
    uint64_t sample_counter;
    uint64_t symbol_count;
    uint32_t len, aux, aux2;
    uint32_t seq;
    uint8_t text[kDevMessageText];
};

struct Output {
    DevEvent *events;
    uint32_t *n_events;
    uint32_t event_cap;
    uint8_t *bursts;
    uint32_t *n_bursts;
    uint32_t burst_cap;
// ... 5 lines not shown
```

### sameold_amd/csrc/same_kernels.hip

```cpp
#include <hip/hip_runtime.h>

#include <algorithm>

#include "same_dev_common.h"
#include "same_device.h"
#include "same_launch.h"

namespace same {

template <int B, typename SampleT>
__global__ __launch_bounds__(kWave) void demod_kernel(Params P, State S, Output O,
                                                      const float4 *__restrict__ taps,
                                                      const SampleT *__restrict__ x,
                                                      uint32_t n_samples, uint64_t counter0)
{
    extern __shared__ float lds[];
    const uint32_t lane = threadIdx.x;
    const uint32_t C = P.n_channels;
    const uint32_t c_raw = blockIdx.x * kWave + lane;
    if (c_raw >= C) return;
    const uint32_t c = c_raw;
    const uint32_t DL = P.dc_len;
    float *ff = lds;
    float *fb = lds + DL * kWave;
    float *win = lds + 2 * DL * kWave;
    const uint32_t wmask = P.win_ring - 1u;

    uint32_t dpos = (uint32_t)(counter0 % DL);
    uint32_t wpos = (uint32_t)(counter0 & wmask);

    for (uint32_t i = 0; i < DL; ++i) {
        ff[i * kWave + lane] = S.dc_ff_ring[i * C + c];
        fb[i * kWave + lane] = S.dc_fb_ring[i * C + c];
    }
    for (uint32_t i = 0; i < P.win_ring; ++i) win[i * kWave + lane] = S.win_ring[i * C + c];

    Lane L;
    lane_load(L, S, c);
    GlobalCtx X{S, c, C};

    for (uint32_t t0 = 0; t0 < n_samples; t0 += B) {
        const uint32_t nb = min((uint32_t)B, n_samples - t0);
        float xs[B];
#pragma unroll
        for (int k = 0; k < B; ++k)
            xs[k] = (k < (int)nb) ? (float)x[(size_t)(t0 + k) * C + c] : 0.0f;

        float ys[B];
        int fire_k = -1;
        float fire_rem = 0.0f, fire_gain = 0.0f;
        const float unlocked0 = (L.flags & F_AGC_LOCKED) ? 0.0f : 1.0f;
#pragma unroll
        for (int k = 0; k < B; ++k) {
            if (k < (int)nb) {
                const uint32_t dnext = (dpos + 1u == DL) ? 0u : dpos + 1u;
                float aged0 = ff[dpos * kWave + lane];
                ff[dpos * kWave + lane] = xs[k];
                float d0 = xs[k] - aged0;
                L.sum0 += d0;
// ... 385 lines not shown

hipError_t launch_reset_columns(const Params &P, const State &S, const uint32_t *cols, uint32_t n, hipStream_t stream)
{
    if (!n) return hipSuccess;
    hipLaunchKernelGGL(reset_columns_kernel, dim3((n + 63u) / 64u), dim3(64), 0, stream, P, S, cols, n);
    return hipGetLastError();
}

__global__ void copy_state_columns_kernel(const StateArrayDesc *desc, uint32_t Csrc, uint32_t Cdst,
                                          const uint32_t *src_col, uint32_t n_cols, uint32_t src_base)
{
    const uint32_t col = blockIdx.x * blockDim.x + threadIdx.x;
    if (col >= n_cols) return;
    const StateArrayDesc d = desc[blockIdx.y];
    const uint32_t sc = src_col ? src_col[col] : col + src_base;
    const uint32_t w = d.elem_words;
    const uint32_t *src = reinterpret_cast<const uint32_t *>(d.src);
    uint32_t *dst = reinterpret_cast<uint32_t *>(d.dst);
    const uint32_t n = d.rows * w;
    for (uint32_t k = blockIdx.z; k < n; k += gridDim.z) {
        const uint32_t r = k / w, i = k - r * w;
        dst[((size_t)r * Cdst + col) * w + i] = src[((size_t)r * Csrc + sc) * w + i];
    }
}
hipError_t launch_copy_state_columns(const StateArrayDesc *desc, uint32_t n_desc, uint32_t src_channels,
                                     uint32_t dst_channels, const uint32_t *src_col, uint32_t n_cols, hipStream_t stream,
                                     uint32_t src_base)
{
    hipLaunchKernelGGL(copy_state_columns_kernel, dim3((n_cols + 255) / 256, n_desc, 16), dim3(256), 0, stream, desc,
                       src_channels, dst_channels, src_col, n_cols, src_base);
    return hipGetLastError();
}
__global__ void chunk_final_column_kernel(const uint64_t *handover, uint32_t C, ChunkGeom g, uint32_t *final_col)
{
    const uint32_t c = blockIdx.x * blockDim.x + threadIdx.x;
    if (c >= C) return;
    uint32_t cur = 0;
    for (;;) {
        const uint64_t h = handover[(size_t)cur * C + c];
        if (h == kNoHandover) break;
        const uint32_t nxt = g.owner_of(h);
        if (nxt <= cur) break;
        cur = nxt;
    }
    final_col[c] = cur * C + c;
}
hipError_t launch_chunk_final_column(const uint64_t *handover, uint32_t in_channels, ChunkGeom g, uint32_t *final_col,
                                     hipStream_t stream)
{
    hipLaunchKernelGGL(chunk_final_column_kernel, dim3((in_channels + 255) / 256), dim3(256), 0, stream, handover, in_channels, g, final_col);
    return hipGetLastError();
}
__global__ void chunk_final_column_pc_kernel(const uint64_t *handover, const uint32_t *own_start, uint32_t C, uint32_t K,
                                             uint64_t counter0, uint32_t *final_col)
{
    const uint32_t c = blockIdx.x * blockDim.x + threadIdx.x;
    if (c >= C) return;
    uint32_t cur = 0;
    for (;;) {
        const uint64_t h = handover[(size_t)cur * C + c];
        if (h == kNoHandover) break;
        uint32_t nxt = cur;
        for (uint32_t k = cur + 1u; k < K; ++k)
            if (counter0 + own_start[(size_t)k * C + c] <= h) nxt = k;
        if (nxt <= cur) break;
        cur = nxt;
    }
    final_col[c] = cur * C + c;
}
hipError_t launch_chunk_final_column_pc(const uint64_t *handover, const uint32_t *own_start, uint32_t in_channels, uint32_t n_chunks,
                                        uint64_t counter0, uint32_t *final_col, hipStream_t stream)
{
    hipLaunchKernelGGL(chunk_final_column_pc_kernel, dim3((in_channels + 255) / 256), dim3(256), 0, stream, handover, own_start,
                       in_channels, n_chunks, counter0, final_col);
    return hipGetLastError();
}
#ifndef SAME_SCOUT_BLOCK
#define SAME_SCOUT_BLOCK 256
#endif
constexpr uint32_t kScoutBlock = SAME_SCOUT_BLOCK;
uint32_t tp_scout_block() { return kScoutBlock; }
__global__ void tp_scout_kernel(const float *__restrict__ x, TpPlan g, float *__restrict__ energy)
{
    const size_t t = (size_t)blockIdx.x * blockDim.x + threadIdx.x;
    const size_t i = t >> 2;
    const uint32_t q = (uint32_t)t & 3u;
    const bool live = i < (size_t)g.channels * g.scout_blocks;
    float e = 0.0f;
    if (live) {
        const uint32_t c = (uint32_t)(i / g.scout_blocks), j = (uint32_t)(i % g.scout_blocks);
        const float4 v = reinterpret_cast<const float4 *>(x + (size_t)c * g.in_samples + (size_t)j * kScoutBlock)[q];
        e = (fabsf(v.x) + fabsf(v.y)) + (fabsf(v.z) + fabsf(v.w));
    }
    e += __shfl_xor(e, 1);
    e += __shfl_xor(e, 2);
    if (live && q == 0u) energy[i] = e;
}
__global__ __launch_bounds__(kWave) void tp_boundaries_kernel(const float *__restrict__ energy, TpPlan g, uint32_t *__restrict__ own_start,
                                                               uint32_t *__restrict__ row0, uint32_t *__restrict__ nominal)
{
    extern __shared__ float tp_lds[];
    const uint32_t c = blockIdx.x, lane = threadIdx.x;
    const int NB = (int)g.scout_blocks, K = (int)g.n_chunks;
    float *e = tp_lds;
    int *lastq = reinterpret_cast<int *>(tp_lds + NB);
    int *cut = lastq + NB;
    constexpr int kQuietBefore = 2048 / (int)kScoutBlock, kQuietAfter = 1;
    float m = 0.0f;
    for (int j = (int)lane; j < NB; j += (int)kWave) { const float v = energy[(size_t)c * NB + j]; e[j] = v; m = fmaxf(m, v); }
    for (int off = 32; off > 0; off >>= 1) m = fmaxf(m, __shfl_xor(m, off));
    const float thr = 0.08f * m;
    __syncthreads();
    const int S = (NB + (int)kWave - 1) / (int)kWave, j0 = (int)lane * S, j1 = min(j0 + S, NB);
    int run = -1;
    for (int j = j0; j < j1; ++j) {
        bool ok = j - kQuietBefore >= 0 && j + kQuietAfter < NB;
        if (ok) for (int t = j - kQuietBefore; t <= j + kQuietAfter; ++t) if (e[t] > thr) { ok = false; break; }
        if (ok) run = j;
        lastq[j] = run;
    }
    int before = run;
    for (int off = 1; off < (int)kWave; off <<= 1) { const int o = __shfl_up(before, off); if ((int)lane >= off) before = max(before, o); }
    before = __shfl_up(before, 1);
    if (lane == 0) before = -1;
    for (int j = j0; j < j1; ++j) if (lastq[j] < 0) lastq[j] = before;
    __syncthreads();
    const uint32_t kB = g.block_len;
    const int min_blocks = 2;
    auto plan = [&](int L, bool store, bool forced) __attribute__((always_inline)) {
        int pos = 0, n = 1;
        while (NB - pos > L) {
            int q = lastq[min(pos + L, NB - 1)];
            if (q < pos + min_blocks) { if (!forced) return 1 << 20; q = pos + L; }
            if (q > NB - min_blocks) q = NB - min_blocks;
            if (q <= pos) return 1 << 20;
            if (n < 64 && store) cut[n] = q;
            pos = q; ++n;
            if (n > K) return n;
        }
        return n;
    };
    const bool forced = plan(NB - 1, false, false) > K;
    int lo = (NB + K - 1) / K, hi = NB;
    while (lo < hi) {
        const int step = (hi - lo + (int)kWave - 1) / (int)kWave;
        const int cand = lo + step * (int)lane;
        const bool ok = cand >= hi || plan(cand, false, forced) <= K;
        const unsigned long long okm = __builtin_amdgcn_ballot_w64(ok);
        if (okm == 0ull) { lo += step * ((int)kWave - 1) + 1; continue; }
        const int first = __builtin_ctzll(okm);
        hi = min(lo + step * first, hi);
        if (first > 0) lo += step * (first - 1) + 1;
    }
    int used = 0;
    if (lane == 0) used = plan(lo, true, forced);
    used = __shfl(used, 0);
    __syncthreads();
    auto own = [&](int k) __attribute__((always_inline)) -> uint32_t {
        const int i = k < used ? k : used - 1;
        uint32_t p = (k >= 1 && i >= 1) ? (uint32_t)cut[i] * kScoutBlock : 0u;
        return p - p % kB;
    };
    for (int k = (int)lane; k < K; k += (int)kWave) {
        const uint32_t p = own(k);
        const uint32_t r = (k == 0 || p < g.warmup_samples) ? 0u : p - g.warmup_samples;
        const size_t v = (size_t)k * g.channels + c;
        own_start[v] = p;
        row0[v] = r;
        nominal[v] = k + 1 < K ? (own(k + 1) - r + kB - 1u) / kB : 0xffffffffu;
    }
}
constexpr uint32_t kSortBuckets = 4096, kSortBucketBlocks = 4;
__device__ __forceinline__ void tp_sort_key(const TpPlan &g, const uint32_t *row0, const uint32_t *nominal, uint32_t v,
                                            uint32_t *group, uint32_t *bucket)
{
    const uint32_t chunk = v / g.channels;
    const uint32_t avail = (g.whole_samples - row0[v]) / g.block_len;
    *group = chunk + 1u == g.n_chunks ? 0u : (chunk == 0u ? 1u : 2u);
    const uint32_t len = *group == 0u ? avail : min(nominal[v], avail);
    *bucket = kSortBuckets - 1u - min(len / kSortBucketBlocks, kSortBuckets - 1u);
}
constexpr uint32_t kSortThreads = 1024;
__global__ __launch_bounds__(kSortThreads) void tp_sort_kernel(TpPlan g, const uint32_t *__restrict__ row0, const uint32_t *__restrict__ nominal,
                                                                uint32_t *__restrict__ perm)
{
    __shared__ uint32_t hist[3u * kSortBuckets];
    __shared__ uint32_t wave_sum[kSortThreads / kWave];
    const uint32_t tid = threadIdx.x, lane = tid & (kWave - 1u), wave = tid / kWave, n = g.n_chunks * g.channels;
    for (uint32_t i = tid; i < 3u * kSortBuckets; i += kSortThreads) hist[i] = 0u;
    __syncthreads();
    for (uint32_t v = tid; v < n; v += kSortThreads) {
        uint32_t grp, b;
        tp_sort_key(g, row0, nominal, v, &grp, &b);
        if (grp != 0u) atomicAdd(&hist[grp * kSortBuckets + b], 1u);
    }
    __syncthreads();
    constexpr uint32_t PER = kSortBuckets / kSortThreads;
    static_assert(PER * kSortThreads == kSortBuckets, "buckets per thread");
    const uint32_t base[3] = {0u, g.channels, 2u * g.channels};
    for (uint32_t grp = 0; grp < 3u; ++grp) {
        uint32_t *h = hist + grp * kSortBuckets + tid * PER;
        uint32_t mine = 0;
        for (uint32_t i = 0; i < PER; ++i) mine += h[i];
        uint32_t incl = mine;
        for (int off = 1; off < (int)kWave; off <<= 1) { const uint32_t t = (uint32_t)__shfl_up((int)incl, off); if ((int)lane >= off) incl += t; }
        if (lane == kWave - 1u) wave_sum[wave] = incl;
        __syncthreads();
        uint32_t before = base[grp] + incl - mine;
        for (uint32_t w = 0; w < wave; ++w) before += wave_sum[w];
        for (uint32_t i = 0; i < PER; ++i) { const uint32_t c = h[i]; h[i] = before; before += c; }
        __syncthreads();
    }
    for (uint32_t v = tid; v < n; v += kSortThreads) {
        uint32_t grp, b;
        tp_sort_key(g, row0, nominal, v, &grp, &b);
        if (grp == 0u) perm[v - (g.n_chunks - 1u) * g.channels] = v;
        else perm[atomicAdd(&hist[grp * kSortBuckets + b], 1u)] = v;
    }
}
__global__ void tp_iota_kernel(uint32_t *perm, uint32_t n)
{
    const uint32_t i = blockIdx.x * blockDim.x + threadIdx.x;
    if (i < n) perm[i] = i;
}
__global__ void tp_align_kernel(TpPlan g, const uint32_t *__restrict__ perm, uint32_t *__restrict__ row0, const uint32_t *__restrict__ nominal,
                                uint32_t *__restrict__ wg_blocks, uint32_t *__restrict__ wg_len)
{
    const uint32_t v = perm[blockIdx.x * kWave + threadIdx.x];
    const uint32_t chunk = v / g.channels;
    uint32_t avail = (g.whole_samples - row0[v]) / g.block_len;
    uint32_t m = avail;
    for (int off = 32; off > 0; off >>= 1) m = max(m, (uint32_t)__shfl_xor((int)m, off));
    if (chunk + 1u == g.n_chunks) row0[v] = g.whole_samples - m * g.block_len;
    if (threadIdx.x == 0) wg_blocks[blockIdx.x] = m;
    if (wg_len) {
        uint32_t len = chunk + 1u == g.n_chunks ? m : min(nominal[v], avail);
        for (int off = 32; off > 0; off >>= 1) len = max(len, (uint32_t)__shfl_xor((int)len, off));
        if (threadIdx.x == 0) wg_len[blockIdx.x] = len;
    }
}
__global__ void tp_wg_order_kernel(uint32_t n_wg, const uint32_t *__restrict__ perm, const uint32_t *__restrict__ wg_blocks,
                                   const uint32_t *__restrict__ wg_len, uint32_t *__restrict__ perm_out, uint32_t *__restrict__ wg_blocks_out,
                                   uint32_t pairs)
{
    const uint32_t w = blockIdx.x, lane = threadIdx.x;
    const uint32_t mine = wg_len[w];
    uint32_t rank = 0;
    for (uint32_t j = lane; j < n_wg; j += kWave) { const uint32_t b = wg_len[j]; rank += (b > mine || (b == mine && j < w)) ? 1u : 0u; }
    for (int off = 32; off > 0; off >>= 1) rank += (uint32_t)__shfl_xor((int)rank, off);
    const uint32_t pos = (pairs && (n_wg & 1u) == 0u) ? (rank < n_wg / 2u ? 2u * rank : 2u * (n_wg - 1u - rank) + 1u) : rank;
    perm_out[pos * kWave + lane] = perm[w * kWave + lane];
    if (lane == 0) wg_blocks_out[pos] = wg_blocks[w];
}
hipError_t launch_tp_plan(const float *x, const TpPlan &g, float *energy, uint32_t *own_start, uint32_t *row0,
                          uint32_t *nominal, uint32_t *perm, uint32_t *wg_blocks, bool sorted, hipStream_t stream,
                          uint32_t *perm_out, uint32_t *wg_blocks_out, bool pairs)
{
    const size_t n = (size_t)g.channels * g.scout_blocks;
    const uint32_t columns = g.n_chunks * g.channels;
    hipLaunchKernelGGL(tp_scout_kernel, dim3((unsigned)((4 * n + 255) / 256)), dim3(256), 0, stream, x, g, energy);
    hipLaunchKernelGGL(tp_boundaries_kernel, dim3(g.channels), dim3(kWave), (size_t)g.scout_blocks * 8 + 64 * sizeof(int), stream, energy, g, own_start, row0, nominal);
    if (sorted) {
        hipLaunchKernelGGL(tp_sort_kernel, dim3(1), dim3(kSortThreads), 0, stream, g, row0, nominal, perm);
    } else {
        hipLaunchKernelGGL(tp_iota_kernel, dim3((columns + 255) / 256), dim3(256), 0, stream, perm, columns);
    }
    uint32_t *wg_len = perm_out ? wg_blocks_out + columns / kWave : nullptr;
    hipLaunchKernelGGL(tp_align_kernel, dim3(columns / kWave), dim3(kWave), 0, stream, g, perm, row0, nominal, wg_blocks, wg_len);
    if (perm_out)
        hipLaunchKernelGGL(tp_wg_order_kernel, dim3(columns / kWave), dim3(kWave), 0, stream, columns / kWave, perm, wg_blocks, wg_len,
                           perm_out, wg_blocks_out, pairs ? 1u : 0u);
    return hipGetLastError();
}

__global__ __launch_bounds__(256) void tp_prologue_kernel(uint4 *__restrict__ dst, const uint4 *__restrict__ src, size_t n16,
                                                          uint64_t *__restrict__ handover, uint32_t *__restrict__ sort_cnt, uint32_t n_cols,
                                                          uint32_t *__restrict__ counters)
{
    const size_t t = (size_t)blockIdx.x * blockDim.x + threadIdx.x, stride = (size_t)gridDim.x * blockDim.x;
    for (size_t i = t; i < n16; i += stride) dst[i] = src[i];
    for (size_t i = t; i < n_cols; i += stride) { handover[i] = kNoHandover; if (sort_cnt) sort_cnt[i] = 0u; }
    if (t < 3 && counters) counters[t] = 0u;
}
hipError_t launch_tp_prologue(void *blob, const void *fresh, size_t bytes, uint64_t *handover, uint32_t *sort_cnt, uint32_t n_cols,
                              uint32_t *counters, hipStream_t stream)
{
    const size_t n16 = bytes / 16;
    const unsigned grid = (unsigned)std::min<size_t>((n16 + 255) / 256, 256 * 16);
    hipLaunchKernelGGL(tp_prologue_kernel, dim3(grid ? grid : 1u), dim3(256), 0, stream, reinterpret_cast<uint4 *>(blob),
                       reinterpret_cast<const uint4 *>(fresh), n16, handover, sort_cnt, n_cols, counters);
    return hipGetLastError();
}
__global__ void cast_i16_f32_kernel(const int16_t *__restrict__ in, float *__restrict__ out, size_t n)
{
    for (size_t i = (size_t)blockIdx.x * blockDim.x + threadIdx.x; i < n; i += (size_t)gridDim.x * blockDim.x) out[i] = (float)in[i];
}
hipError_t launch_cast_i16_f32(const int16_t *in, float *out, size_t n, hipStream_t stream)
{
    if (!n) return hipSuccess;
    hipLaunchKernelGGL(cast_i16_f32_kernel, dim3((unsigned)std::min<size_t>((n + 255) / 256, 65536)), dim3(256), 0, stream, in, out, n);
    return hipGetLastError();
}
__global__ void fill_u64_kernel(uint64_t *p, size_t n, uint64_t v)
{
    const size_t i = (size_t)blockIdx.x * blockDim.x + threadIdx.x;
    if (i < n) p[i] = v;
}
hipError_t launch_fill_u64(uint64_t *p, size_t n, uint64_t v, hipStream_t stream)
{
    hipLaunchKernelGGL(fill_u64_kernel, dim3((unsigned)((n + 255) / 256)), dim3(256), 0, stream, p, n, v);
    return hipGetLastError();
}

hipError_t launch_transpose(const float *in, float *out, uint32_t n_channels, uint32_t n_samples,
                            hipStream_t stream)
{
    dim3 grid((n_samples + 63) / 64, (n_channels + 63) / 64);
    hipLaunchKernelGGL(transpose_to_time_major<float>, grid, dim3(256), 0, stream, in, out, n_channels, n_samples);
    return hipGetLastError();
}
hipError_t launch_transpose(const int16_t *in, int16_t *out, uint32_t n_channels, uint32_t n_samples,
// ... 9 lines not shown
```

### sameold_amd/csrc/same_kernels_pipe.hip

```cpp
#include <hip/hip_runtime.h>

#include <cmath>
#include <cstdlib>
#include <type_traits>

#include "same_dev_common.h"
#include "same_device.h"
#include "same_fast_common.h"
#include "same_launch.h"
#include "same_pipe_common.h"
#include "same_profile.h"
#include "same_relaxed_common.h"

namespace same {

template <int NT> struct PipeGeom;
template <> struct PipeGeom<42> { static constexpr int DCL = 16, B = kBlockPipe22; };
template <> struct PipeGeom<92> { static constexpr int DCL = 35, B = kBlockPipe48; };
template <> struct PipeGeom<84> { static constexpr int DCL = 32, B = kBlockPipe44; };
template <int NT> struct PipeLayout {
    static constexpr int B = PipeGeom<NT>::B, RING = 5 * B;
    static constexpr bool YLDS = B >= kBlock48k;
    static constexpr uint32_t yring_floats = YLDS ? 3u * (uint32_t)B * kWave : 0u;
    static constexpr uint32_t dcw_blocks = 4u;
// ... 499 lines not shown
#pragma unroll
        for (int j = DEPTH - 2; j >= 0; --j) {
            const uint32_t blk = s - 2u + (uint32_t)(DEPTH - 1 - j);
            if (blk < n_blocks) { g0[j] = g; push(P, wcol, j, blk, g, -1, bw1, bw1); }
        }
        gain = g;
    }
    __device__ __forceinline__ void store(const Params &P, const State &S, uint32_t c, uint32_t C, uint64_t counter1, const float *wcol)
    {
        S.agc_gain[c] = gain;
        const uint32_t G = P.win_ring;
#pragma unroll 2
        for (uint32_t m = 1; m <= G; ++m) {
            const uint32_t g = (uint32_t)(counter1 - (uint64_t)m) & (G - 1u);
            const uint32_t j = wnext >= m ? wnext - m : wnext + (uint32_t)RING - m;
            float *row = S.win_ring + (size_t)g * C;
            row[c] = wcol[(j + (uint32_t)RING) * LP];
        }
    }
};

template <int NT, int LANES, bool SPLIT> constexpr bool pipe_dcw() { return SPLIT && ((NT == 42 && LANES <= 32) || (NT != 42 && LANES == 64)); }
template <int NT, int NFF, int NFB, bool MED3, bool SHARE, int LANES, bool SPLIT, typename SampleT, bool FM = false, int CMODE = 2>
__global__ __launch_bounds__((pipe_dcw<NT, LANES, SPLIT>() ? 5 : 4) * kWave, SHARE ? 2 : 1) void demod_pipe_kernel(Params P, State S, Output O,
                                                                const float4 *__restrict__ taps,
                                                                const SampleT *__restrict__ x,
                                                                uint32_t n_blocks, uint64_t counter0, PipeChunks K)
{
    static_assert(!FM || (SPLIT && LANES == 64 && SHARE == (NT == 42)),
                  "FASTMATH is built for 64-channel workgroups: two per CU at 22.05 kHz, one (with the DC wavefront) at 44.1 / 48 kHz");
    constexpr int NTP = PipeLayout<NT>::NTP;
    if constexpr (CMODE == 0) { K.col_row0 = nullptr; K.col_perm = nullptr; }
    constexpr int kB = PipeLayout<NT>::B, RING = PipeLayout<NT>::RING;
    constexpr uint32_t LP = kWave, kPipeTapFloats = PipeLayout<NT>::tap_floats;
    constexpr bool PACKED = SPLIT && LANES <= 32;
    constexpr bool HELPER_BOTH = PACKED || (SPLIT && SHARE && NT == 42) || FM;
    constexpr bool DCW = pipe_dcw<NT, LANES, SPLIT>();
    static_assert(kB <= 64, "the sample index travels in six bits of the stage 3 -> 4 word");
    extern __shared__ float lds[];
    const uint32_t lane = threadIdx.x & (kWave - 1u);
    const uint32_t role = (uint32_t)__builtin_amdgcn_readfirstlane((int)(threadIdx.x >> 6));
    const uint32_t C = P.n_channels;
    const uint32_t c = (K.n_chunks > 1u && K.col_perm) ? K.col_perm[blockIdx.x * (uint32_t)LANES + lane]
                                                       : blockIdx.x * (uint32_t)LANES + lane;
    uint32_t cin = c, Cin = C, n_nominal = n_blocks;
    bool may_leave = false;
    int32_t row_l = 0;
    const SampleT *xl = nullptr;
    uint32_t avail_l = 0;
    if (K.n_chunks > 1u) {
        Cin = K.in_channels;
        if (K.col_row0) {
            const uint32_t chunk_l = c / Cin;
            cin = c - chunk_l * Cin;
            may_leave = (uint32_t)__builtin_amdgcn_readfirstlane((int)chunk_l) + 1u < K.n_chunks;
            const uint32_t row_abs = K.col_row0[c];
            xl = x + (size_t)cin * K.in_samples + row_abs;
            avail_l = (K.whole_samples - row_abs) / (uint32_t)kB;
            n_blocks = K.wg_blocks[blockIdx.x];
            n_nominal = may_leave ? K.col_nominal[c] : n_blocks;
            const uint32_t row_first = (uint32_t)__builtin_amdgcn_readfirstlane((int)row_abs);
            counter0 += (uint64_t)row_first;
            row_l = (int32_t)(row_abs - row_first);
        } else {
            const uint32_t wgs = K.in_channels / (uint32_t)LANES;
            const uint32_t chunk = (uint32_t)__builtin_amdgcn_readfirstlane((int)(blockIdx.x / wgs));
            cin = (blockIdx.x - chunk * wgs) * (uint32_t)LANES + lane;
            may_leave = chunk + 1u < K.n_chunks;
            const uint32_t first_block = chunk * K.stride_blocks;
            x += (size_t)first_block * kB * Cin;
            counter0 += (uint64_t)first_block * kB;
            n_blocks -= first_block;
            n_nominal = may_leave ? K.nominal_blocks : n_blocks;
        }
    }
    float4 *tlds = reinterpret_cast<float4 *>(lds);
    lds_u32 *mail = (lds_u32 *)(lds + kPipeTapFloats);
    lds_u32 *symbox = mail;
    lds_u32 *fbbox = mail + 2u * kP3SymWords;
    lds_u32 *iobox = fbbox + 2u * kP3FbWords;
    lds_u32 *phasebox = iobox + 2u * kP3IoWords;
    lds_u32 *againbox = phasebox + kWave;
    lds_u32 *chunkbox = fbbox + kWave + 2u;
    lds_u32 *seqbox = fbbox + kWave + 4u;
    lds_u32 *posbox = againbox + kWave;
    lds_u32 *spacebox = posbox + 2u * kWave;
    lds_u32 *markbox = spacebox + kWave;
    lds_u32 *tkbox = markbox + kWave;
    float *hcol = lds + kPipeTapFloats + kP3MailWords + lane;
    float *wring = lds + kPipeTapFloats + kP3MailWords + (kSquelchHist - kB) * LP;
    float *wcol = wring + lane;
    const uint64_t counter1 = counter0 + (uint64_t)n_blocks * kB;
    const uint32_t n_steps = n_blocks + 3u;
    const uint32_t last_fb_step = n_blocks + 1u;

    float *dcw_ring = wring + (2u * (uint32_t)RING) * LP;
    if (DCW && role == 4u) {
        if (LANES < (int)kWave && lane >= (uint32_t)LANES) return;
        P3_HWID(4);
        DcStage<NT, SampleT> D;
        D.load(P, S, x, c, C, cin, Cin, counter0, n_blocks);
        float *ycol = dcw_ring + lane;
        constexpr uint32_t YMASK = PipeLayout<NT>::dcw_blocks - 1u;
        D.template fetch<0>(x, 0u, n_blocks, cin, Cin);
        D.block(P, ycol);
        lds_barrier();
        uint32_t stop_at = 0xffffffffu;
// ... 618 lines not shown
```

### sameold_amd/csrc/same_kernels_relaxed.hip

```cpp
#include <hip/hip_runtime.h>

#include <cmath>
#include <type_traits>

#include "same_dev_common.h"
#include "same_device.h"
#include "same_fast_common.h"
#include "same_launch.h"
#include "same_profile.h"
#include "same_relaxed_common.h"

namespace same {

template <int NT> struct RelaxGeom;
template <> struct RelaxGeom<42> { static constexpr int DCL = 16, SB = 21; };
template <int NT> struct RelaxLayout {
    static constexpr int SB = RelaxGeom<NT>::SB, B = 2 * SB, DCL = RelaxGeom<NT>::DCL;
    static constexpr int RING = 3 * SB, MIRROR = kRelaxChunk - 1;
    static constexpr uint32_t tap_floats = (uint32_t)((NT * 4 + 63) / 64 * 64);
    static constexpr size_t lds_bytes = ((size_t)tap_floats + (size_t)(RING + MIRROR) * kWave) * sizeof(float);
    static_assert(NT - 1 + SB <= RING, "a filter at the start of a sub-block reaches into the sub-block being written");
    static_assert(NT % kRelaxChunk == 0, "whole chunks");
    static_assert(SB >= DCL && SB - DCL >= 1, "the DC windows are the tail of the previous sub-block");
};
// ... 2 lines not shown
{
    S.dc_sum0[c] = L.sum0; S.dc_sum1[c] = L.sum1; S.agc_gain[c] = L.gain;
    S.until_next_ted[c] = L.until_next_ted; S.ted_clock[c] = L.ted_clock;
    S.ted_h0[c] = L.h0; S.ted_h1[c] = L.h1; S.ted_h2[c] = L.h2;
    S.period_avg[c] = L.period_avg; S.period_inst[c] = L.period_inst;
    S.sq_data[c] = L.sq_data; S.sq_power[c] = L.sq_power; S.sq_phist[c] = L.sq_phist;
    S.sq_fill[c] = L.sq_fill; S.sq_clock[c] = L.sq_clock; S.sq_symbols[c] = L.sq_symbols;
    S.eq_word[c] = L.eq_word; S.eq_count[c] = L.eq_count;
    S.fr_word[c] = L.fr_word; S.fr_count[c] = L.fr_count; S.fr_invalid[c] = L.fr_invalid;
    S.fr_len[c] = L.fr_len; S.flags[c] = L.flags;
}
__device__ __forceinline__ void lane_load_link(Lane &L, const State &S, uint32_t c)
{
    L.sum0 = S.dc_sum0[c]; L.sum1 = S.dc_sum1[c]; L.gain = S.agc_gain[c];
    L.until_next_ted = S.until_next_ted[c]; L.ted_clock = S.ted_clock[c];
    L.h0 = S.ted_h0[c]; L.h1 = S.ted_h1[c]; L.h2 = S.ted_h2[c];
    L.period_avg = S.period_avg[c]; L.period_inst = S.period_inst[c];
    L.sq_data = S.sq_data[c]; L.sq_power = S.sq_power[c]; L.sq_phist = S.sq_phist[c];
    L.sq_fill = S.sq_fill[c]; L.sq_clock = S.sq_clock[c]; L.sq_symbols = S.sq_symbols[c];
    L.eq_word = S.eq_word[c]; L.eq_count = S.eq_count[c];
    L.fr_word = S.fr_word[c]; L.fr_count = S.fr_count[c]; L.fr_invalid = S.fr_invalid[c];
    L.fr_len = S.fr_len[c]; L.flags = S.flags[c];
    L.tk_next = 0; L.tk_last = 0; L.wake_sample = 0; L.wake_fired = 0; L.ended = 0;
}

template <int NT, int NFF, int NFB, typename SampleT, bool CM, bool TICKS, int OCC>
__global__ __launch_bounds__(kWave, OCC) void demod_relaxed_kernel(Params P, State S, Output O,
                                                                   const float4 *__restrict__ taps,
                                                                   const SampleT *__restrict__ x,
                                                                   uint32_t n_blocks, uint64_t counter0, PipeChunks K)
{
    using LY = RelaxLayout<NT>;
    constexpr int SB = LY::SB, B = LY::B, DCL = LY::DCL, RING = LY::RING, MIR = LY::MIRROR;
    constexpr int HOFF = SB - DCL;
    constexpr uint32_t LP = kWave;
    static_assert(!CM || std::is_same<SampleT, float>::value, "channel-major streams are f32");
    extern __shared__ float lds[];
    const uint32_t lane = threadIdx.x;
    float4 *tlds = reinterpret_cast<float4 *>(lds);
    for (uint32_t i = lane; i < (uint32_t)NT; i += kWave) tlds[i] = taps[i];
    __syncthreads();
    const uint32_t C = P.n_channels;
    uint32_t c = blockIdx.x * kWave + lane;
    if (c >= C) return;
    if (K.n_chunks > 1u && K.col_perm) c = K.col_perm[c];
    uint32_t cin = c, Cin = C, n_nominal = n_blocks;
    bool may_leave = false;
    int32_t row_l = 0;
    const float *xl = nullptr;
    uint32_t avail_l = 0xffffffffu;
    if constexpr (CM) {
        Cin = K.in_channels;
        const uint32_t chunk_l = c / Cin;
        cin = c - chunk_l * Cin;
        may_leave = (uint32_t)__builtin_amdgcn_readfirstlane((int)chunk_l) + 1u < K.n_chunks;
        const uint32_t row_abs = K.col_row0[c];
        xl = reinterpret_cast<const float *>(x) + (size_t)cin * K.in_samples + row_abs;
        avail_l = (K.whole_samples - row_abs) / (uint32_t)B;
        n_blocks = K.wg_blocks[blockIdx.x];
        n_nominal = may_leave ? K.col_nominal[c] : n_blocks;
        const uint32_t row_first = (uint32_t)__builtin_amdgcn_readfirstlane((int)row_abs);
        counter0 += (uint64_t)row_first;
        row_l = (int32_t)(row_abs - row_first);
    } else if (K.n_chunks > 1u) {
        Cin = K.in_channels;
        const uint32_t wgs = K.in_channels / kWave;
        const uint32_t chunk = blockIdx.x / wgs;
        cin = (blockIdx.x - chunk * wgs) * kWave + lane;
        may_leave = chunk + 1u < K.n_chunks;
        const uint32_t first_block = chunk * K.stride_blocks;
        x += (size_t)first_block * B * Cin;
        counter0 += (uint64_t)first_block * B;
        n_blocks -= first_block;
        n_nominal = may_leave ? K.nominal_blocks : n_blocks;
    }
    float *wcol = lds + LY::tap_floats + lane;
    const uint32_t taps_lds = lds_addr(lds), wcol_lds = lds_addr(wcol);

    Lane L;
    if constexpr (TICKS) lane_load(L, S, c); else lane_load_link(L, S, c);
    RelaxCtx<NFF, NFB> X;
    X.S = &S; X.c = c; X.C = C;
    X.hist = S.sq_hist + c;
#pragma unroll
    for (int i = 0; i < NFF; ++i) { X.ffc[i] = S.eq_ffc[i * C + c]; X.ffw[i] = S.eq_ffw[i * C + c]; }
#pragma unroll
    for (int i = 0; i < NFB; ++i) { X.fbc[i] = S.eq_fbc[i * C + c]; X.fbw[i] = S.eq_fbw[i * C + c]; }
    {
        const uint32_t G = P.win_ring;
#pragma unroll 2
        for (uint32_t m = 1; m < (uint32_t)NT; ++m) {
            const uint32_t g = (uint32_t)(counter0 - (uint64_t)m) & (G - 1u);
            const float *row = S.win_ring + (size_t)g * C;
            wcol[((uint32_t)RING - m) * LP] = row[c];
        }
    }
    static_assert(RING - (NT - 1) > MIR, "the carried-over window would need mirroring");

    float xa[SB + 1], xb[SB - 1], ma[SB], mb[SB];
    {
        const uint32_t dpos = (uint32_t)(counter0 % (uint64_t)DCL);
#pragma unroll
        for (int k = 0; k < DCL; ++k) {
            uint32_t slot = dpos + (uint32_t)k;
            if (slot >= (uint32_t)DCL) slot -= (uint32_t)DCL;
            const float *r0 = S.dc_ff_ring + (size_t)slot * C, *r1 = S.dc_fb_ring + (size_t)slot * C;
            xb[k + HOFF - 1] = r0[c];
// ... 176 lines not shown
        const uint32_t dpos = (uint32_t)(counter1 % (uint64_t)DCL);
#pragma unroll
        for (int k = 0; k < DCL; ++k) {
            uint32_t slot = dpos + (uint32_t)k;
            if (slot >= (uint32_t)DCL) slot -= (uint32_t)DCL;
            float *r0 = S.dc_ff_ring + (size_t)slot * C, *r1 = S.dc_fb_ring + (size_t)slot * C;
            r0[c] = xb[k + HOFF - 1];
            r1[c] = mb[k + HOFF];
        }
    }
}

template <int NT> struct DuoLayout {
    static constexpr int SB = RelaxGeom<NT>::SB, B = 2 * SB, DCL = RelaxGeom<NT>::DCL;
    static constexpr int RING = 4 * SB, MIRROR = kRelaxChunk - 1;
    static constexpr uint32_t tap_floats = (uint32_t)((NT * 4 + 63) / 64 * 64);
    static constexpr uint32_t mail_words = 2u * kWave + 64u;
    static constexpr size_t lds_bytes = ((size_t)tap_floats + mail_words + (size_t)(RING + MIRROR) * kWave) * sizeof(float);
    static_assert(NT - 1 + SB <= 3 * SB, "B's filters reach into the sub-block A writes");
};
typedef volatile __attribute__((address_space(3))) uint32_t duo_u32;
__device__ __forceinline__ void duo_barrier() { asm volatile("s_waitcnt lgkmcnt(0)\n\ts_barrier" ::: "memory"); }

template <int NT, int NFF, int NFB, typename SampleT, bool CM, bool TICKS>
__global__ __launch_bounds__(2 * kWave, 2) void demod_duo_kernel(Params P, State S, Output O,
                                                                 const float4 *__restrict__ taps,
                                                                 const SampleT *__restrict__ x,
                                                                 uint32_t n_blocks, uint64_t counter0, PipeChunks K)
{
    using LY = DuoLayout<NT>;
    constexpr int SB = LY::SB, B = LY::B, DCL = LY::DCL, RING = LY::RING, MIR = LY::MIRROR;
    constexpr int HOFF = SB - DCL;
    constexpr uint32_t LP = kWave;
    static_assert(!CM || std::is_same<SampleT, float>::value, "channel-major streams are f32");
    extern __shared__ float lds[];
    const uint32_t lane = threadIdx.x & (kWave - 1u);
    const uint32_t role = (uint32_t)__builtin_amdgcn_readfirstlane((int)(threadIdx.x >> 6));
    float4 *tlds = reinterpret_cast<float4 *>(lds);
    if (role == 0u) for (uint32_t i = lane; i < (uint32_t)NT; i += kWave) tlds[i] = taps[i];
    duo_u32 *mail = (duo_u32 *)(lds + LY::tap_floats);
    duo_u32 *fbbox = mail;
    duo_u32 *flagbox = mail + 2u * kWave;
    const uint32_t C = P.n_channels;
    uint32_t c = blockIdx.x * kWave + lane;
    if (K.n_chunks > 1u && K.col_perm) c = K.col_perm[c];
    uint32_t cin = c, Cin = C, n_nominal = n_blocks;
    bool may_leave = false;
    int32_t row_l = 0;
    const float *xl = nullptr;
    uint32_t avail_l = 0xffffffffu;
    if constexpr (CM) {
        Cin = K.in_channels;
        const uint32_t chunk_l = c / Cin;
        cin = c - chunk_l * Cin;
        may_leave = (uint32_t)__builtin_amdgcn_readfirstlane((int)chunk_l) + 1u < K.n_chunks;
        const uint32_t row_abs = K.col_row0[c];
        xl = reinterpret_cast<const float *>(x) + (size_t)cin * K.in_samples + row_abs;
        avail_l = (K.whole_samples - row_abs) / (uint32_t)B;
        n_blocks = K.wg_blocks[blockIdx.x];
        n_nominal = may_leave ? K.col_nominal[c] : n_blocks;
        const uint32_t row_first = (uint32_t)__builtin_amdgcn_readfirstlane((int)row_abs);
        counter0 += (uint64_t)row_first;
        row_l = (int32_t)(row_abs - row_first);
    } else if (K.n_chunks > 1u) {
        Cin = K.in_channels;
        const uint32_t wgs = K.in_channels / kWave;
        const uint32_t chunk = blockIdx.x / wgs;
        cin = (blockIdx.x - chunk * wgs) * kWave + lane;
        may_leave = chunk + 1u < K.n_chunks;
        const uint32_t first_block = chunk * K.stride_blocks;
        x += (size_t)first_block * B * Cin;
        counter0 += (uint64_t)first_block * B;
        n_blocks -= first_block;
        n_nominal = may_leave ? K.nominal_blocks : n_blocks;
    }
    float *wcol = lds + LY::tap_floats + LY::mail_words + lane;
    const uint32_t n_sub = 2u * n_blocks;
    const uint64_t counter1 = counter0 + (uint64_t)n_blocks * B;

    if (role == 0u) {
        float sum0 = S.dc_sum0[c], sum1 = S.dc_sum1[c], gain = S.agc_gain[c];
        bool locked = (S.flags[c] & F_AGC_LOCKED) != 0u;
        {
            const uint32_t G = P.win_ring;
#pragma unroll 2
            for (uint32_t m = 1; m < (uint32_t)NT; ++m) {
                const uint32_t g = (uint32_t)(counter0 - (uint64_t)m) & (G - 1u);
                const float *row = S.win_ring + (size_t)g * C;
                wcol[((uint32_t)RING - m) * LP] = row[c];
            }
        }
        static_assert(RING - (NT - 1) > MIR, "the carried-over window would need mirroring");
        float xa[SB + 1], xb[SB - 1], ma[SB], mb[SB];
        float ys0[SB], ys1[SB];
        float g00 = gain, g01 = gain;
        {
            const uint32_t dpos = (uint32_t)(counter0 % (uint64_t)DCL);
#pragma unroll
            for (int k = 0; k < DCL; ++k) {
                uint32_t slot = dpos + (uint32_t)k;
                if (slot >= (uint32_t)DCL) slot -= (uint32_t)DCL;
                const float *r0 = S.dc_ff_ring + (size_t)slot * C, *r1 = S.dc_fb_ring + (size_t)slot * C;
                xb[k + HOFF - 1] = r0[c];
                mb[k + HOFF] = r1[c];
            }
#pragma unroll
            for (int k = 0; k < SB; ++k) { ys0[k] = 0.0f; ys1[k] = 0.0f; }
// ... 316 lines not shown
```

### sameold_amd/csrc/same_kernels_sym.hip

```cpp
#include <hip/hip_runtime.h>

#include <cmath>
#include <cstdlib>
#include <mutex>
#include <set>
#include <type_traits>
#include <utility>

#include "same_dev_common.h"
#include "same_device.h"
#include "same_fast_common.h"
#include "same_launch.h"
#include "same_pipe_common.h"
#include "same_profile.h"
#include "same_relaxed_common.h"

namespace same {

constexpr int kSymSub = 36;
constexpr uint32_t kSymDrain = 5u;
constexpr uint32_t kSymOffMask = 255u;
template <int NT> struct SymGeom;
template <> struct SymGeom<42> { static constexpr int DCL = 16, NSUB = 1, HALVES = 2; };
template <> struct SymGeom<92> { static constexpr int DCL = 35, NSUB = 2, HALVES = 1; };
// ... 862 lines not shown
    uint64_t p = (uint64_t)(uintptr_t)ka + off;
    asm volatile("" : "+s"(p));
    T r;
    __builtin_memcpy(&r, reinterpret_cast<const __attribute__((address_space(4))) void *>(p), sizeof(T));
    return r;
}

constexpr int kSymRoles = 6;
template <int NT, int NFF, int NFB, typename SampleT, int CMODE>
__global__ __launch_bounds__(SymGeom<NT>::HALVES * kSymRoles * kWave, NT == 42 ? 3 : 2) void demod_sym_kernel(Params P, State S_arg_, Output O_arg_, const float4 *__restrict__ taps,
                                                                         const SampleT *__restrict__ x, uint32_t n_blocks, uint64_t counter0,
                                                                         PipeChunks K)
{
    (void)S_arg_; (void)O_arg_;
    const sym_kernarg_ptr ka = (sym_kernarg_ptr)__builtin_amdgcn_kernarg_segment_ptr();
    auto fresh_state = [&]() __attribute__((always_inline)) -> State { return sym_fresh_arg<State>(ka, offsetof(SymKernArgs, S)); };
    auto fresh_output = [&]() __attribute__((always_inline)) -> Output { return sym_fresh_arg<Output>(ka, offsetof(SymKernArgs, O)); };
    using LY = SymLayout<NT>;
    constexpr int kB = LY::B, RING = LY::RING, kSB = LY::SB, kNSUB = LY::NSUB;
    constexpr uint32_t kSymHalves = (uint32_t)LY::HALVES;
    constexpr uint32_t LP = kWave;
    static_assert(CMODE == 0 || std::is_same<SampleT, float>::value, "channel-major streams are f32");
    if constexpr (CMODE == 0) { K.col_row0 = nullptr; K.col_perm = nullptr; }
    extern __shared__ float lds_all[];
    const uint32_t lane = threadIdx.x & (kWave - 1u);
    const uint32_t wave = (uint32_t)__builtin_amdgcn_readfirstlane((int)(threadIdx.x >> 6));
    constexpr uint64_t kDeal0 = 0xdcba98543210ull;
#ifdef SAME_PROFILE
    const uint32_t deal = ((uint32_t)P.knob_prio >> 14) & 3u;
    constexpr uint64_t kDeal1 = 0x805d192ab3c4ull;
    constexpr uint64_t kDeal2 = 0x08d591a2b3c4ull;
    constexpr uint64_t kDeal3 = 0x2ad51908b3c4ull;
    const uint64_t tbl = deal == 0u ? kDeal0 : (deal == 1u ? kDeal1 : (deal == 2u ? kDeal2 : kDeal3));
#else
    constexpr uint64_t tbl = kDeal0;
#endif
    const uint32_t hr = LY::HALVES == 2 ? (uint32_t)(tbl >> (4u * wave)) & 15u : wave;
    const uint32_t half = LY::HALVES == 2 ? hr >> 3 : 0u;
    const uint32_t role = hr & 7u;
    const uint32_t C = P.n_channels;
    const uint32_t vwg = blockIdx.x * kSymHalves + half;
    if (vwg * kWave >= C) return;
    float *lds = lds_all + half * (uint32_t)(LY::lds_bytes / sizeof(float));
    const uint32_t c = (K.n_chunks > 1u && K.col_perm) ? K.col_perm[vwg * kWave + lane] : vwg * kWave + lane;
    uint32_t cin = c, Cin = C, n_nominal = n_blocks;
    bool may_leave = false;
    int32_t row_l = 0;
    const SampleT *xl = nullptr;
    uint32_t avail_l = 0;
    if (K.n_chunks > 1u) {
        Cin = K.in_channels;
        if (K.col_row0) {
            const uint32_t chunk_l = c / Cin;
            cin = c - chunk_l * Cin;
            may_leave = (uint32_t)__builtin_amdgcn_readfirstlane((int)chunk_l) + 1u < K.n_chunks;
            const uint32_t row_abs = K.col_row0[c];
            xl = x + (size_t)cin * K.in_samples + row_abs;
            avail_l = (K.whole_samples - row_abs) / (uint32_t)kSB;
            n_blocks = K.wg_blocks[vwg];
            n_nominal = may_leave ? K.col_nominal[c] : n_blocks;
            const uint32_t row_first = (uint32_t)__builtin_amdgcn_readfirstlane((int)row_abs);
            counter0 += (uint64_t)row_first;
            row_l = (int32_t)(row_abs - row_first);
        } else {
            const uint32_t wgs = K.in_channels / kWave;
            const uint32_t chunk = (uint32_t)__builtin_amdgcn_readfirstlane((int)(vwg / wgs));
            cin = (vwg - chunk * wgs) * kWave + lane;
            may_leave = chunk + 1u < K.n_chunks;
            const uint32_t first_block = chunk * K.stride_blocks;
            x += (size_t)first_block * kB * Cin;
            counter0 += (uint64_t)first_block * kB;
            n_blocks -= first_block;
            n_nominal = may_leave ? K.nominal_blocks : n_blocks;
        }
    }
    lds_u32 *mail = (lds_u32 *)(lds + LY::tap_floats);
    lds_u32 *symbox = mail;
    lds_u32 *ybox = symbox + 2u * LY::sym_words;
    lds_u32 *fb1box = ybox + 2u * kWave;
    lds_u32 *fb2box = fb1box + 2u * LY::fb_words;
    lds_u32 *iobox = fb2box + 2u * LY::fb_words;
    lds_u32 *phasebox = iobox + 2u * LY::io_words;
    lds_u32 *againbox = phasebox + kWave;
    lds_u32 *flagbox = againbox + kWave;
    lds_u32 *posbox = flagbox + kWave;
    lds_u32 *sabox = posbox + 2u * kWave;
    lds_u32 *tkbox = sabox + kWave;
    lds_u32 *donebox = tkbox + kIoRingWords;
    lds_u32 *chunkbox = fb1box + kWave + 2u;
    lds_u32 *seqbox = fb1box + kWave + 4u;
    static_assert((size_t)(2u * LY::sym_words + 2u * kWave + 4u * LY::fb_words + 2u * LY::io_words + 3u * kWave + 2u * kWave + kWave + kIoRingWords + kWave + kWave) <= LY::mail_words, "mailboxes");
    float *wring = lds + LY::tap_floats + LY::mail_words;
    float *wcol = wring + lane;
    const uint64_t counter1 = counter0 + (uint64_t)n_blocks * kB;
    const uint32_t last_e_step = n_blocks + kSymDrain;
    const uint32_t last_y1_step = last_e_step + 1u, last_y2_step = last_e_step + 2u, last_a_step = last_e_step + 3u;
    const uint32_t n_steps = last_e_step + 4u;
    auto sym_index = [&](uint32_t s_e, uint32_t off) __attribute__((always_inline)) -> int64_t {
        const int64_t base = s_e <= n_blocks ? (int64_t)s_e - 2 : (int64_t)n_blocks - 3;
        return (int64_t)kB * base + (int64_t)off;
    };
    lds_u32 *prog = donebox + kWave;
    lds_u32 *pos2box = prog + kWave + (SYM_TL_WORDS + 63u) / 64u * 64u;
    lds_u32 *partbox = pos2box + 2u * kWave;
#ifdef SAME_SYM_TL
    lds_u32 *tlbox = prog + kWave;
#endif
// ... 752 lines not shown
```

### sameold_amd/csrc/same_launch.h

```cpp
#pragma once

#include <hip/hip_runtime.h>

#include "same_capture_dev.h"
#include "same_device.h"
#include "same_select.h"

namespace same {

hipError_t launch_demod(const Params &P, const State &S, const Output &O, const float4 *taps,
                        const float *x, uint32_t n_samples, uint64_t counter0, hipStream_t stream);
hipError_t launch_demod(const Params &P, const State &S, const Output &O, const float4 *taps,
                        const int16_t *x, uint32_t n_samples, uint64_t counter0, hipStream_t stream);
hipError_t launch_demod_ragged(const Params &P, const State &S, const Output &O, const float4 *taps, const float *x,
                               uint32_t n_rows, const uint32_t *counts, uint32_t row_sub, uint64_t counter0, hipStream_t stream);
hipError_t launch_demod_ragged(const Params &P, const State &S, const Output &O, const float4 *taps, const int16_t *x,
                               uint32_t n_rows, const uint32_t *counts, uint32_t row_sub, uint64_t counter0, hipStream_t stream);
hipError_t launch_demod_pipe(const Params &P, const State &S, const Output &O, const float4 *taps,
                             const float *x, uint32_t n_blocks, uint64_t counter0, hipStream_t stream,
                             const PipeChunks &chunks = PipeChunks{}, bool relaxed = false);
hipError_t launch_demod_pipe(const Params &P, const State &S, const Output &O, const float4 *taps,
                             const int16_t *x, uint32_t n_blocks, uint64_t counter0, hipStream_t stream,
                             const PipeChunks &chunks = PipeChunks{}, bool relaxed = false);
hipError_t launch_demod_sym(const Params &P, const State &S, const Output &O, const float4 *taps,
                            const float *x, uint32_t n_blocks, uint64_t counter0, hipStream_t stream,
                            const PipeChunks &chunks = PipeChunks{});
hipError_t launch_demod_sym(const Params &P, const State &S, const Output &O, const float4 *taps,
                            const int16_t *x, uint32_t n_blocks, uint64_t counter0, hipStream_t stream,
                            const PipeChunks &chunks = PipeChunks{});
hipError_t launch_demod_relaxed(const Params &P, const State &S, const Output &O, const float4 *taps,
                                const float *x, uint32_t n_blocks, uint64_t counter0, hipStream_t stream,
                                const PipeChunks &chunks = PipeChunks{});
hipError_t launch_demod_relaxed(const Params &P, const State &S, const Output &O, const float4 *taps,
                                const int16_t *x, uint32_t n_blocks, uint64_t counter0, hipStream_t stream,
                                const PipeChunks &chunks = PipeChunks{});
hipError_t launch_demod_fast(const Params &P, const State &S, const Output &O, const float4 *taps,
                             const float *x, uint32_t n_blocks, uint64_t counter0, hipStream_t stream);
hipError_t launch_demod_fast(const Params &P, const State &S, const Output &O, const float4 *taps,
                             const int16_t *x, uint32_t n_blocks, uint64_t counter0, hipStream_t stream);
hipError_t launch_counters(uint32_t *dev, uint32_t *host_mapped, int publish, hipStream_t stream);
uint32_t event_sort_extra_words(uint32_t n_bins);
hipError_t launch_event_sort(const DevEvent *ev, const uint32_t *counters, uint32_t cap, uint32_t n_bins, uint32_t *cnt, uint32_t *first,
                             DevEvent *sorted, hipStream_t stream, bool cnt_is_zero = false);
hipError_t launch_init_state(const Params &P, const State &S, int is_reset, hipStream_t stream, uint32_t first_col = 0);
hipError_t launch_reset_columns(const Params &P, const State &S, const uint32_t *cols, uint32_t n, hipStream_t stream);
hipError_t launch_copy_state_columns(const StateArrayDesc *desc, uint32_t n_desc, uint32_t src_channels,
                                     uint32_t dst_channels, const uint32_t *src_col, uint32_t n_cols, hipStream_t stream,
                                     uint32_t src_base = 0);
hipError_t launch_chunk_final_column(const uint64_t *handover, uint32_t in_channels, ChunkGeom g, uint32_t *final_col,
                                     hipStream_t stream);
hipError_t launch_chunk_final_column_pc(const uint64_t *handover, const uint32_t *own_start, uint32_t in_channels, uint32_t n_chunks,
                                        uint64_t counter0, uint32_t *final_col, hipStream_t stream);
hipError_t launch_fill_u64(uint64_t *p, size_t n, uint64_t v, hipStream_t stream);
hipError_t launch_cast_i16_f32(const int16_t *in, float *out, size_t n, hipStream_t stream);
hipError_t launch_tp_prologue(void *blob, const void *fresh, size_t bytes, uint64_t *handover, uint32_t *sort_cnt, uint32_t n_cols,
                              uint32_t *counters, hipStream_t stream);
uint32_t tp_scout_block();
struct TpPlan {
    uint32_t channels, n_chunks, block_len, warmup_samples, whole_samples;
    uint64_t in_samples;
    uint32_t scout_blocks;
};
hipError_t launch_tp_plan(const float *x, const TpPlan &g, float *energy, uint32_t *own_start, uint32_t *row0,
                          uint32_t *nominal, uint32_t *perm, uint32_t *wg_blocks, bool sorted, hipStream_t stream,
                          uint32_t *perm_out = nullptr, uint32_t *wg_blocks_out = nullptr, bool pairs = false);
hipError_t launch_transpose(const float *in, float *out, uint32_t n_channels, uint32_t n_samples,
                            hipStream_t stream);
hipError_t launch_transpose(const int16_t *in, int16_t *out, uint32_t n_channels, uint32_t n_samples,
                            hipStream_t stream);

constexpr uint32_t kMessageLogOverflow = 8u;
struct TransportLaunch {
    uint32_t n_channels, input_rate;
    const uint32_t *first;
    DevEvent *sorted;
    const uint32_t *counters;
    const uint8_t *bursts; uint32_t burst_cap;
    void *hot, *cold;
    uint64_t *wake_sample;
    DevMessage *near; uint32_t near_cap;
    DevMessage *log; uint32_t log_cap;
    uint32_t *log_cursor, *overflow;
    cap::Launch cap;
};
size_t transport_hot_bytes();
size_t transport_cold_bytes();
hipError_t launch_transport(const TransportLaunch &T, hipStream_t stream);
hipError_t launch_transport_ragged(const TransportLaunch &T, const uint32_t *counts, uint32_t row_sub, uint32_t n_rows, hipStream_t stream);
hipError_t launch_transport_reset(void *hot, void *cold, uint32_t n_channels, const uint32_t *cols, uint32_t n, int fresh,
                                  hipStream_t stream, void *capture_rec = nullptr);
hipError_t launch_capture(const cap::Span *spans, cap::Cursors *cur, uint32_t span_cap, float *pool, uint64_t pool_cap,
                          const float *x, uint32_t n_channels, uint32_t n_rows, cap::Cursors *host, hipStream_t stream);
hipError_t launch_capture(const cap::Span *spans, cap::Cursors *cur, uint32_t span_cap, float *pool, uint64_t pool_cap,
                          const int16_t *x, uint32_t n_channels, uint32_t n_rows, cap::Cursors *host, hipStream_t stream);

struct SynthParams {
    uint32_t n_channels;
    uint32_t input_rate;
    uint64_t seed;
    float noise_sigma;
    uint32_t flags;
};
hipError_t launch_synth(const SynthParams &sp, float *x, size_t n_samples, hipStream_t stream);
struct TrialParams {
    uint32_t n_trials;
    uint32_t first_trial;
    uint32_t input_rate;
    uint32_t n_grid;
    uint64_t seed;
    float ebn0_db_lo, ebn0_db_step;
};
hipError_t launch_trials(const TrialParams &tp, float *x, size_t n_samples, hipStream_t stream);
uint32_t synth_payload(uint64_t seed, uint32_t channel, uint8_t *out, uint32_t cap);

}
```

### sameold_amd/receiver.py

```python
from __future__ import annotations

import ctypes as C
import os
import sys
from typing import Iterator, List, Optional, Sequence

import numpy as np

_HERE = os.path.dirname(os.path.abspath(__file__))
LIB_PATH = os.path.join(_HERE, f"libsame_rx.{os.environ['SAME_LIB_VARIANT']}.so" if os.environ.get("SAME_LIB_VARIANT") else "libsame_rx.so")

LINK_NO_CARRIER, LINK_SEARCHING, LINK_READING, LINK_BURST = 0, 1, 2, 3
TRANSPORT_IDLE, TRANSPORT_ASSEMBLING, TRANSPORT_MSG_START, TRANSPORT_MSG_END, TRANSPORT_MSG_ERR = 16, 17, 18, 19, 20
LAYOUT_TIME_MAJOR, LAYOUT_CHANNEL_MAJOR = 0, 1
BATCH_LINK_ONLY, BATCH_TRACE_SYMBOLS, BATCH_GENERIC_KERNEL, BATCH_TIME_PARALLEL, BATCH_RELAXED, BATCH_CALL_INVARIANT = 1, 2, 4, 8, 16, 32
BATCH_MESSAGES_ONLY = 64
TP_EVENT_TOLERANCE_SYMBOLS = 2
STREAM_OWN = (1 << 64) - 1
EVENT_MAX_BYTES = 288
AUDIO_FIRST, AUDIO_END_MESSAGE, AUDIO_END_FLUSH, AUDIO_END_RESET, AUDIO_TRUNCATED = 1, 2, 4, 8, 16
AUDIO_END = AUDIO_END_MESSAGE | AUDIO_END_FLUSH | AUDIO_END_RESET

ERRORS = {-1: "EINVAL", -2: "EDCLEN", -3: "EAGCLIMITS", -4: "EEQORDER", -5: "ENODEVICE",
          -6: "EHIP", -7: "EOVERFLOW", -8: "ENOMEM", -9: "ERATE", -10: "EKERNEL"}
# ... 88 lines not shown
    P, vp, u32, u64, f32 = C.POINTER, C.c_void_p, C.c_uint32, C.c_uint64, C.c_float

    def sig(name, res, *args):
        fn = getattr(L, name)
        fn.restype = res
        fn.argtypes = list(args)

    sig("same_last_error", C.c_char_p)
    sig("same_rx_abi_version", u32)
    sig("same_rx_builder_new", vp, u32)
    sig("same_rx_builder_default", vp)
    sig("same_rx_builder_clone", vp, vp)
    sig("same_rx_builder_free", None, vp)
    sig("same_rx_builder_with_dc_blocker_length", None, vp, f32)
    sig("same_rx_builder_with_agc_bandwidth", None, vp, f32)
    sig("same_rx_builder_with_agc_gain_limits", None, vp, f32, f32)
    sig("same_rx_builder_with_timing_bandwidth", None, vp, f32, f32)
    sig("same_rx_builder_with_timing_max_deviation", None, vp, f32)
    sig("same_rx_builder_with_squelch_power", None, vp, f32, f32)
    sig("same_rx_builder_with_squelch_bandwidth", None, vp, f32)
    sig("same_rx_builder_with_preamble_max_errors", None, vp, u32)
    sig("same_rx_builder_with_adaptive_equalizer", None, vp, u32, u32, f32, f32)
    sig("same_rx_builder_without_adaptive_equalizer", None, vp)
    sig("same_rx_builder_with_frame_prefix_max_errors", None, vp, u32)
    sig("same_rx_builder_with_frame_max_invalid", None, vp, u32)
    sig("same_rx_builder_input_rate", u32, vp)
    sig("same_rx_builder_dc_blocker_length", f32, vp)
    sig("same_rx_builder_agc_bandwidth", f32, vp)
    sig("same_rx_builder_agc_gain_limits", None, vp, P(f32))
    sig("same_rx_builder_timing_bandwidth", None, vp, P(f32), P(f32))
    sig("same_rx_builder_timing_max_deviation", f32, vp)
    sig("same_rx_builder_squelch_power", None, vp, P(f32), P(f32))
    sig("same_rx_builder_squelch_bandwidth", f32, vp)
    sig("same_rx_builder_preamble_max_errors", u32, vp)
    sig("same_rx_builder_adaptive_equalizer", C.c_int, vp, P(u32), P(u32), P(f32), P(f32))
    sig("same_rx_builder_frame_prefix_max_errors", u32, vp)
    sig("same_rx_builder_frame_max_invalid", u32, vp)

    sig("same_batch_new", C.c_int, vp, u32, C.c_int, u32, P(vp))
    sig("same_batch_free", None, vp)
    sig("same_batch_reset", C.c_int, vp)
    sig("same_batch_reset_channels", C.c_int, vp, P(u32), C.c_size_t)
    sig("same_batch_channel_input_sample_counter", u64, vp, u32)
    sig("same_batch_input_rate", u32, vp)
    sig("same_batch_n_channels", u32, vp)
    sig("same_batch_input_sample_counter", u64, vp)
    sig("same_batch_device", C.c_int, vp)
    sig("same_batch_process_device", C.c_int, vp, vp, C.c_size_t, u32, vp)
    sig("same_batch_order_after", C.c_int, vp, vp)
    sig("same_batch_set_call_window", C.c_int, vp, C.c_uint32)
    sig("same_batch_time_parallel_config", C.c_int, vp, u32, u32, u32)
    sig("same_batch_time_parallel_chunks", u32, vp)
    sig("same_batch_time_parallel_per_channel", C.c_int, vp)
    sig("same_batch_transport_on_device", C.c_int, vp)
    sig("same_batch_set_audio_capture", C.c_int, vp, C.c_size_t)
    sig("same_batch_peek_audio", C.c_int, vp, P(P(AudioChunk)), P(C.c_size_t))
    sig("same_batch_drop_audio", C.c_int, vp, C.c_size_t)
    sig("same_rx_source_hash", C.c_char_p)
    sig("same_batch_process_device_i16", C.c_int, vp, vp, C.c_size_t, u32, vp)
    sig("same_batch_process_host", C.c_int, vp, vp, C.c_size_t, u32)
    sig("same_batch_process_host_i16", C.c_int, vp, vp, C.c_size_t, u32)
    sig("same_batch_process_device_ragged", C.c_int, vp, vp, C.c_size_t, P(u32), u32, vp)
    sig("same_batch_process_device_ragged_i16", C.c_int, vp, vp, C.c_size_t, P(u32), u32, vp)
    sig("same_batch_process_host_ragged", C.c_int, vp, vp, C.c_size_t, P(u32), u32)
    sig("same_batch_process_host_ragged_i16", C.c_int, vp, vp, C.c_size_t, P(u32), u32)
    sig("same_batch_flush", C.c_int, vp)
    sig("same_batch_sync", C.c_int, vp)
    sig("same_batch_poll_events", C.c_int, vp, P(Event), C.c_size_t, P(C.c_size_t), P(C.c_size_t))
    sig("same_batch_pending_events", C.c_size_t, vp)
    sig("same_batch_peek_events", C.c_int, vp, P(P(Event)), P(C.c_size_t))
    sig("same_batch_drop_events", C.c_int, vp, C.c_size_t)
    sig("same_batch_pack_bursts", C.c_int, vp, u32, vp, C.c_size_t, P(C.c_size_t))
    sig("same_batch_read_trace", C.c_int, vp, u32, P(SymbolTrace), C.c_size_t, P(C.c_size_t))
    sig("same_batch_last_kernel_ms", C.c_int, vp, P(f32))
    sig("same_batch_last_demod_kernel_ms", C.c_int, vp, P(f32))
    sig("same_batch_set_kernel_timing", None, vp, C.c_int)
    sig("same_batch_kernel_name", C.c_char_p, vp)

    sig("same_rx_build", C.c_int, vp, C.c_int, P(vp))
    sig("same_rx_free", None, vp)
    sig("same_rx_process", C.c_int, vp, vp, C.c_size_t, P(C.c_size_t), P(Event))
    sig("same_rx_flush", C.c_int, vp, P(Event))
    sig("same_rx_reset", C.c_int, vp)
    sig("same_rx_input_rate", u32, vp)
    sig("same_rx_input_sample_counter", u64, vp)

    sig("same_synth_afsk_device", C.c_int, vp, u32, C.c_size_t, u32, u64, f32, u32, C.c_int, vp)
    sig("same_synth_payload", u32, u64, u32, C.c_char_p, u32)
    _lib = L
    return L


def _check(rc: int):
    if rc < 0:
        raise SameError(rc, load_library().same_last_error().decode(errors="replace"))
    return rc


class SameReceiverBuilder:

    def __init__(self, input_rate: int = 22050):
        self._L = load_library()
        self._h = C.c_void_p(self._L.same_rx_builder_new(input_rate))

    def __del__(self):
        if getattr(self, "_h", None):
# ... 110 lines not shown
        _check(self._L.same_batch_new(builder._h, n_channels, device, flags, C.byref(h)))
        self._h = h
        self._inflight = []

    def __del__(self):
        if getattr(self, "_h", None):
            self._L.same_batch_free(self._h)
            self._h = None

    @property
    def n_channels(self) -> int:
        return self._L.same_batch_n_channels(self._h)

    def input_rate(self) -> int:
        return self._L.same_batch_input_rate(self._h)

    def input_sample_counter(self) -> int:
        return self._L.same_batch_input_sample_counter(self._h)

    def kernel_name(self) -> str:
        return self._L.same_batch_kernel_name(self._h).decode()

    def set_call_window(self, samples: int) -> None:
        _check(self._L.same_batch_set_call_window(self._h, int(samples)))

    def reset(self):
        _check(self._L.same_batch_reset(self._h))

    def reset_channels(self, channels) -> None:
        if hasattr(channels, "detach"):
            channels = channels.detach().numpy()
        arr = np.atleast_1d(np.asarray(channels))
        if arr.size and (arr.dtype.kind not in "iu" or arr.min() < 0 or arr.max() >= 1 << 32):
            raise ValueError("channels must be non-negative integers")
        arr = np.ascontiguousarray(arr.reshape(-1), dtype=np.uint32)
        _check(self._L.same_batch_reset_channels(self._h, arr.ctypes.data_as(C.POINTER(C.c_uint32)), arr.size))

    def channel_input_sample_counter(self, channel: int) -> int:
        if not 0 <= channel < self.n_channels:
            raise IndexError(f"channel {channel} of {self.n_channels}")
        return int(self._L.same_batch_channel_input_sample_counter(self._h, channel))

    def time_parallel_config(self, max_chunks: int = 0, min_own_samples: int = 0, warmup_samples: int = 0):
        _check(self._L.same_batch_time_parallel_config(self._h, max_chunks, min_own_samples, warmup_samples))

    def time_parallel_chunks(self) -> int:
        return self._L.same_batch_time_parallel_chunks(self._h)

    def transport_on_device(self) -> int:
        return int(self._L.same_batch_transport_on_device(self._h))

    def time_parallel_per_channel(self) -> bool:
        return bool(self._L.same_batch_time_parallel_per_channel(self._h))

    def set_audio_capture(self, samples_per_launch: int) -> None:
        _check(self._L.same_batch_set_audio_capture(self._h, int(samples_per_launch)))

    def poll_audio(self) -> list:
        ptr, n = C.POINTER(AudioChunk)(), C.c_size_t()
        _check(self._L.same_batch_peek_audio(self._h, C.byref(ptr), C.byref(n)))
        out = []
        for i in range(n.value):
            ch = ptr[i]
            k = int(ch.n_samples)
            a = np.ctypeslib.as_array(ch.samples, shape=(k,)).copy() if k else np.zeros(0, np.float32)
            out.append((int(ch.channel), int(ch.sample_counter), int(ch.flags), a))
        if n.value:
            _check(self._L.same_batch_drop_audio(self._h, n.value))
        return out

    def process_device_ptr(self, ptr: int, n_samples: int, layout: int = LAYOUT_TIME_MAJOR,
                           stream: Optional[int] = None, i16: bool = False):
        fn = self._L.same_batch_process_device_i16 if i16 else self._L.same_batch_process_device
        _check(fn(self._h, C.c_void_p(ptr), n_samples, layout, C.c_void_p(STREAM_OWN if stream is None else stream)))

    def order_after(self, producer_stream: int):
        _check(self._L.same_batch_order_after(self._h, C.c_void_p(producer_stream)))

    def process_tensor(self, x, layout: int = LAYOUT_TIME_MAJOR, stream: Optional[int] = None):
        import torch
        assert x.is_cuda and x.is_contiguous()
        if layout == LAYOUT_TIME_MAJOR:
            n, ch = x.shape
        else:
            ch, n = x.shape
        assert ch == self.n_channels
        if x.dtype not in (torch.float32, torch.int16):
            raise TypeError("float32 or int16 input")
        if stream is None:
            self.order_after(torch.cuda.current_stream(x.device).cuda_stream)
        self._inflight.append(x)
        self.process_device_ptr(x.data_ptr(), n, layout, stream, x.dtype == torch.int16)
        if len(self._inflight) > 2:
            del self._inflight[0]

    def process_host(self, x: np.ndarray, layout: int = LAYOUT_TIME_MAJOR):
        x = np.ascontiguousarray(x)
        if x.ndim == 1:
            x = x.reshape(-1, 1) if layout == LAYOUT_TIME_MAJOR else x.reshape(1, -1)
        n, ch = x.shape if layout == LAYOUT_TIME_MAJOR else x.shape[::-1]
        assert ch == self.n_channels, (ch, self.n_channels)
        if x.dtype == np.int16:
            _check(self._L.same_batch_process_host_i16(self._h, C.c_void_p(x.ctypes.data), n, layout))
        else:
            x = np.ascontiguousarray(x, dtype=np.float32)
            _check(self._L.same_batch_process_host(self._h, C.c_void_p(x.ctypes.data), n, layout))
# ... 273 lines not shown
```

Before: 470,500.

## Lend spare time-parallel columns from quiet channels to busy channels

Adds a planning step in which channels that need fewer time chunks than the per-channel budget donate their spare columns to channels that need more. The columns of each channel are then chained through a next-column link table. The kernel uses per-column input-channel and next-column maps, and the host-side handover and event-ordering walk follows the links rather than a fixed stride. The aim is to balance work across columns and shorten the longest column, at the cost of extra plan scratch, a larger geometry copy, and more complex handover logic.

Result: slower. 450,200 (-4.3%).

```diff
diff --git a/include/same_rx.h b/include/same_rx.h
--- a/include/same_rx.h
+++ b/include/same_rx.h
@@ -149,6 +149,8 @@
                                     uint32_t warmup_samples);
 uint32_t same_batch_time_parallel_chunks(const same_batch *rx);
 int same_batch_time_parallel_per_channel(const same_batch *rx);
+uint32_t same_batch_time_parallel_lent_columns(const same_batch *rx);
+uint32_t same_batch_time_parallel_longest_column(const same_batch *rx);
 
 int same_batch_transport_on_device(const same_batch *rx);
 
diff --git a/sameold_amd/build.py b/sameold_amd/build.py
--- a/sameold_amd/build.py
+++ b/sameold_amd/build.py
@@ -14,7 +14,7 @@
 SOURCES = ["same_kernels.hip", "same_kernels_fast.hip", "same_kernels_pipe.hip", "same_kernels_relaxed.hip", "same_kernels_sym.hip", "same_kernels_sym_hi.hip", "same_synth.hip", "same_transport.hip", "same_capture.hip", "same_resample.hip", "same_batch.cpp", "same_select.cpp", "same_config.cpp", "same_transport.cpp", "same_place.cpp"]
 SOURCE_FLAGS = {"same_kernels_sym_hi.hip": ["-mllvm", "-amdgpu-sched-strategy=max-ilp"],
                 "same_kernels_pipe.hip": ["-mllvm", "-amdgpu-sched-strategy=max-ilp"]}
-HEADERS = ["same_dev_common.h", "same_fast_common.h", "same_relaxed_common.h", "same_pipe_common.h", "same_profile.h", "same_device.h", "same_hipmem.h", "same_launch.h", "same_select.h", "same_config.h", "same_transport.h", "same_transport_dev.h", "same_capture_dev.h", "same_resets.h", "same_resample_dev.h", "same_resample_plan.h", "../../include/same_rx.h", "../../include/same_resample.h",
+HEADERS = ["same_dev_common.h", "same_fast_common.h", "same_relaxed_common.h", "same_pipe_common.h", "same_profile.h", "same_device.h", "same_hipmem.h", "same_launch.h", "same_select.h", "same_config.h", "same_transport.h", "same_transport_dev.h", "same_capture_dev.h", "same_resets.h", "same_resample_dev.h", "same_resample_plan.h", "same_tp_plan.h", "../../include/same_rx.h", "../../include/same_resample.h",
            "../../include/same_place.h", "samedec_main.cpp"]
 SAMEDEC = os.path.join(HERE, "samedec_gpu")
 ARCH = "gfx950"
diff --git a/sameold_amd/csrc/same_batch.cpp b/sameold_amd/csrc/same_batch.cpp
--- a/sameold_amd/csrc/same_batch.cpp
+++ b/sameold_amd/csrc/same_batch.cpp
@@ -221,6 +221,7 @@
         same::DevBuf<uint64_t> d_handover;
         same::PinnedBuf<uint64_t> h_handover;
         bool per_channel = false;
+        bool linked = false;
         same::DevBuf<uint32_t> d_geom;
         same::PinnedBuf<uint32_t> h_geom;
         same::CoherentBuf<uint32_t> h_reset;
@@ -258,6 +259,9 @@
         same::DevBuf<float> d_hist;
         same::Event ev_plan_prev; bool plan_recorded = false;
         int knob_plan_stream = 0;
+        int knob_lend = 0;
+        same::DevBuf<uint32_t> d_plan;
+        uint32_t last_limit = 0, last_lent = 0, last_longest = 0;
         int sort_mode = -1;
         uint32_t last_chunks = 1;
         bool last_per_channel = false;
@@ -421,6 +425,7 @@
     { const char *e = std::getenv("SAME_RECORD_HARVEST"); rx->record_path = e ? e : ""; }
     rx->host_threads = std::max(0, num("SAME_HOST_THREADS", 0));
     rx->tp.sort_mode = num("SAME_TP_SORT", -1);
+    rx->tp.knob_lend = tri("SAME_TP_LEND");
     rx->tp.knob_plan_stream = tri("SAME_TP_PLAN_STREAM");
     rx->tp.knob_prologue = tri("SAME_TP_PROLOGUE");
     rx->want.knob_relaxed = tri("SAME_RELAXED");
@@ -529,7 +534,7 @@
     const uint32_t n_real = first[n_bins];
     if (n_real > n_events) return fail(SAME_EHIP, "internal: event sort counted %u of %u events", n_real, n_events);
     struct Identity { uint32_t operator[](uint32_t i) const { return i; } } order;
-    if (dbg && sl.chunked && sl.per_channel) {
+    if (dbg && sl.chunked && sl.per_channel && !sl.linked) {
         const same::ChunkGeom &g = sl.geom;
         const uint32_t *own = in.geom, *rows = in.geom + n_bins;
         double len_sum = 0, run_sum = 0; uint64_t len_max = 0, run_max = 0, n_len = 0, n_run = 0, n_inf = 0, n_late = 0;
@@ -619,21 +624,24 @@
         const same::ChunkGeom &g = sl.geom;
         const uint64_t *hand = in.handover;
         const uint32_t *own = sl.per_channel ? in.geom : nullptr, *rows = sl.per_channel ? in.geom + n_bins : nullptr;
-        auto owner_of = [&](uint64_t h) -> uint32_t {
-            if (!own) return g.owner_of(h);
-            uint32_t k = 0;
-            while (k + 1u < g.n_chunks && g.counter0 + own[(size_t)(k + 1u) * n_ch + c] <= h) ++k;
+        const uint32_t *next = sl.linked ? in.geom + 2u * (size_t)n_bins + 4u + n_bins : nullptr;
+        auto next_of = [&](uint32_t v) -> uint32_t { return next ? next[v] : (v + n_ch < n_bins ? v + n_ch : 0xffffffffu); };
+        auto owner_of = [&](uint64_t h, uint32_t from) -> uint32_t {
+            if (!own) return g.owner_of(h) * n_ch + c;
+            uint32_t k = from, v = next_of(from);
+            for (uint32_t n = 0; v < n_bins && n < 64u; v = next_of(v), ++n)
+                if (g.counter0 + own[v] <= h) k = v;
             return k;
         };
         TickSynth &ts = rx->tp.synth[c];
         int64_t off = rx->tp.sym_off[c];
-        uint32_t cur = 0;
+        uint32_t col = c;
         uint64_t keep_after = 0;
-        for (;;) {
-            const uint32_t col = cur * n_ch + c;
+        for (uint32_t hops = 0; hops < 64u; ++hops) {
+            const uint32_t cur = col / n_ch;
             const uint64_t h = hand[col];
             const uint64_t upto = std::min(h, sl.end_blocks);
-            bool rebased = cur == 0;
+            bool rebased = col == c;
             for (uint32_t i = first[col]; i < first[col + 1u]; ++i) {
                 const same::DevEvent &d = evs[order[i]];
                 if (d.sample_counter <= keep_after) continue;
@@ -651,9 +659,8 @@
                 off = est_end - (int64_t)((double)(sl.end_blocks - row0) / sps + 0.5);
             }
             if (h == same::kNoHandover) break;
-            const uint32_t nxt = owner_of(h);
-            if (nxt <= cur) break;
-            const uint32_t ncol = nxt * n_ch + c;
+            const uint32_t ncol = owner_of(h, col);
+            if (own ? ncol == col : ncol <= col) break;
             uint32_t st = 0, j = first[ncol];
             for (; j < first[ncol + 1u] && evs[order[j]].sample_counter <= h; ++j)
                 if (evs[order[j]].kind <= SAME_LINK_BURST) st = evs[order[j]].kind;
@@ -668,7 +675,7 @@
                 inj.burst_slot = 0xffffffffu;
                 feed(part, ev, inj, c, 0);
             }
-            cur = nxt;
+            col = ncol;
         }
         for (uint32_t i = first[c]; i < first[c + 1u]; ++i)
             if (evs[order[i]].sample_counter > sl.end_blocks) feed(part, ev, evs[order[i]], c, off);
@@ -690,7 +697,9 @@
                 }
             }
             { HP(0);
-            for (uint32_t col = c; col < n_bins; col += n_ch)
+            const uint32_t *next = (sl.chunked && sl.linked) ? in.geom + 2u * (size_t)n_bins + 4u + n_bins : nullptr;
+            uint32_t hops = 0;
+            for (uint32_t col = c; col < n_bins && hops < 64u; col = next ? next[col] : col + n_ch, ++hops)
                 if (first[col + 1u] - first[col] > 1u)
                     std::sort(evs_mut + first[col], evs_mut + first[col + 1u],
                               [](const same::DevEvent &a, const same::DevEvent &b) { return a.channel < b.channel; });
@@ -785,7 +794,7 @@
     HarvestFileHeader h{};
     h.magic = kHarvestMagic;
     h.n_channels = n_ch; h.n_bins = n_bins; h.n_events = n_events; h.n_bursts = n_bursts;
-    h.chunked = sl.chunked; h.per_channel = sl.per_channel; h.flags = rx->flags; h.input_rate = rx->P.input_rate; h.tp_enabled = rx->tp.enabled;
+    h.chunked = sl.chunked; h.per_channel = sl.per_channel ? (sl.linked ? 2u : 1u) : 0u; h.flags = rx->flags; h.input_rate = rx->P.input_rate; h.tp_enabled = rx->tp.enabled;
     h.geom = sl.geom; h.end_blocks = sl.end_blocks; h.end_counter = sl.end_counter;
     bool ok = std::fwrite(&h, sizeof(h), 1, f) == 1;
     ok = ok && std::fwrite(sl.h_sort, sizeof(uint32_t), (size_t)n_bins + 1, f) == (size_t)n_bins + 1;
@@ -793,7 +802,8 @@
     ok = ok && (!n_bursts || std::fwrite(sl.h_bursts, same::kBurstCap, n_bursts, f) == n_bursts);
     if (sl.chunked) {
         ok = ok && std::fwrite(sl.h_handover, sizeof(uint64_t), n_bins, f) == n_bins;
-        if (sl.per_channel) ok = ok && std::fwrite(sl.h_geom, sizeof(uint32_t), (size_t)2 * n_bins, f) == (size_t)2 * n_bins;
+        const size_t n_geom = sl.linked ? (size_t)4 * n_bins + 4 : (size_t)2 * n_bins;
+        if (sl.per_channel) ok = ok && std::fwrite(sl.h_geom, sizeof(uint32_t), n_geom, f) == n_geom;
     }
     std::fclose(f);
     return ok ? SAME_OK : fail(SAME_EINVAL, "SAME_RECORD_HARVEST: short write to %s", path);
@@ -1002,10 +1012,14 @@
     if (sl.chunked) {
         HIP_TRY(hipMemcpyAsync(sl.h_handover, sl.d_handover, (size_t)n_bins * sizeof(uint64_t), hipMemcpyDeviceToHost, rx->copy_stream));
         if (sl.per_channel)
-            HIP_TRY(hipMemcpyAsync(sl.h_geom, sl.d_geom, (size_t)2 * n_bins * sizeof(uint32_t), hipMemcpyDeviceToHost, rx->copy_stream));
+            HIP_TRY(hipMemcpyAsync(sl.h_geom, sl.d_geom, ((size_t)(sl.linked ? 4 : 2) * n_bins + 4) * sizeof(uint32_t), hipMemcpyDeviceToHost, rx->copy_stream));
     }
     if (n_bursts || sl.chunked) HIP_TRY(hipStreamSynchronize(rx->copy_stream));
     auto t_copied = std::chrono::steady_clock::now();
+    if (sl.chunked && sl.per_channel) {
+        const uint32_t *info = sl.h_geom + 2u * (size_t)n_bins;
+        rx->tp.last_limit = info[0]; rx->tp.last_lent = info[1]; rx->tp.last_longest = info[2];
+    }
     if (!rx->record_path.empty()) { const int rrc = record_harvest(rx, sl, n_events, n_bursts, rx->record_path.c_str()); if (rrc != SAME_OK) return rrc; }
     std::vector<uint32_t> rearm;
     HarvestTimes times;
@@ -1193,11 +1207,12 @@
     return SAME_OK;
 }
 
-int tp_hand_back(same_batch *rx, same_batch::Slot &sl, const same::ChunkGeom &geom, const uint32_t *own_start, hipStream_t stream)
+int tp_hand_back(same_batch *rx, same_batch::Slot &sl, const same::ChunkGeom &geom, const uint32_t *own_start, hipStream_t stream,
+                 const uint32_t *col_next = nullptr)
 {
     same_batch::TimePar &tp = rx->tp;
     const uint32_t C = rx->P.n_channels;
-    if (own_start) HIP_TRY(same::launch_chunk_final_column_pc(sl.d_handover, own_start, C, geom.n_chunks, rx->counter, tp.d_final_col, stream));
+    if (own_start) HIP_TRY(same::launch_chunk_final_column_pc(sl.d_handover, own_start, C, geom.n_chunks, rx->counter, tp.d_final_col, stream, col_next));
     else HIP_TRY(same::launch_chunk_final_column(sl.d_handover, C, geom, tp.d_final_col, stream));
     HIP_TRY(same::launch_copy_state_columns(tp.d_desc_out, tp.n_desc, geom.n_chunks * C, C, tp.d_final_col, C, stream));
     return SAME_OK;
@@ -1321,12 +1336,12 @@
             if (rc) return rc;
             const size_t n_whole = (size_t)total_blocks * fbk;
             if (n_whole < n && (rc = demod_tail(rx, O, xp + n_whole * C, n - n_whole, rx->counter + n_whole, stream)) != SAME_OK) return rc;
-            sl.chunked = true; sl.per_channel = false;
+            sl.chunked = true; sl.per_channel = false; sl.linked = false;
             sl.geom = geom;
             sl.end_blocks = rx->counter + n_whole;
             rx->tp.last_per_channel = false;
         } else {
-        sl.chunked = false; sl.per_channel = false;
+        sl.chunked = false; sl.per_channel = false; sl.linked = false;
         rc = ensure_output(rx, sl, n, O);
         if (rc) return rc;
         HIP_TRY(same::launch_counters(sl.d_counters, sl.h_counters.dev(), 0, stream));
@@ -1482,8 +1497,8 @@
     same::Output O{};
     rc = tp_reserve(rx, sl, columns, n, pc, fb, O);
     if (rc) return rc;
-    HIP_TRY(sl.d_geom.ensure((size_t)5 * columns + 3 * (columns / same::kWave)));
-    HIP_TRY(sl.h_geom.ensure((size_t)2 * columns));
+    HIP_TRY(sl.d_geom.ensure((size_t)7 * columns + 4 + 3 * (columns / same::kWave)));
+    HIP_TRY(sl.h_geom.ensure((size_t)4 * columns + 4));
     same::TpPlan plan{};
     plan.channels = C; plan.n_chunks = n_chunks; plan.block_len = fb;
     {
@@ -1494,8 +1509,11 @@
     plan.whole_samples = (uint32_t)n; plan.in_samples = n_call;
     plan.scout_blocks = (uint32_t)(n / same::tp_scout_block());
     HIP_TRY(tp.d_energy.ensure((size_t)C * plan.scout_blocks));
-    uint32_t *d_own = sl.d_geom, *d_row0 = sl.d_geom + columns, *d_nom = sl.d_geom + 2 * (size_t)columns,
-             *d_perm = sl.d_geom + 3 * (size_t)columns, *d_wg = sl.d_geom + 4 * (size_t)columns,
+    HIP_TRY(tp.d_plan.ensure(same::tp_lend_scratch_words(plan)));
+    const bool lend = tp.knob_lend >= 0;
+    uint32_t *d_own = sl.d_geom, *d_row0 = sl.d_geom + columns, *d_info = sl.d_geom + 2 * (size_t)columns, *d_cin = d_info + 4,
+             *d_next = d_cin + columns, *d_nom = d_next + columns,
+             *d_perm = d_nom + columns, *d_wg = d_perm + columns,
              *d_wg2 = d_wg + columns / same::kWave, *d_perm2 = d_wg2 + 2 * (columns / same::kWave);
     const bool pair_groups = tp.sort_mode == 2 && tp.family == same::Family::kSym;
     const int sort_mode = pair_groups ? 0 : (tp.sort_mode >= 0 ? (tp.sort_mode ? 1 : 0) : (same::tp_more_than_one_round(columns) ? 1 : 0));
@@ -1506,7 +1524,7 @@
     hipStream_t ps = side ? rx->plan_stream : stream;
     if (tp.plan_recorded) HIP_TRY(hipStreamWaitEvent(ps, tp.ev_plan_prev, 0));
     HIP_TRY(same::launch_tp_plan(d_x, plan, tp.d_energy, d_own, d_row0, d_nom, d_perm, d_wg, sort_mode != 0, ps,
-                                 lpt ? d_perm2 : nullptr, lpt ? d_wg2 : nullptr, pair_groups));
+                                 same::TpLend{tp.d_plan, d_cin, d_next, d_info, lend}, lpt ? d_perm2 : nullptr, lpt ? d_wg2 : nullptr, pair_groups));
     HIP_TRY(tp.ev_plan_prev.ensure());
     HIP_TRY(hipEventRecord(tp.ev_plan_prev, ps));
     tp.plan_recorded = true;
@@ -1521,6 +1539,7 @@
     pc.handover = sl.d_handover;
     pc.col_row0 = d_row0; pc.col_nominal = d_nom; pc.wg_blocks = d_wg; pc.col_perm = (sort_mode != 0 || pair_groups) ? d_perm : nullptr;
     pc.in_samples = n_call; pc.whole_samples = (uint32_t)n;
+    pc.col_cin = lend ? d_cin : nullptr; pc.col_next = lend ? d_next : nullptr;
     pc.hist_scratch = nullptr;
     if (pc.col_perm && tp.family == same::Family::kSym) {
         HIP_TRY(tp.d_hist.ensure((size_t)columns * same::kSquelchHist));
@@ -1532,10 +1551,10 @@
     rx->last_family = tp.family;
     if (e != hipSuccess) return fail(SAME_EHIP, "time-parallel demod kernel launch failed: %s", hipGetErrorString(e));
     if (sl.timed) HIP_TRY(hipEventRecord(sl.ev_k1, stream));
-    rc = tp_hand_back(rx, sl, geom, d_own, stream);
+    rc = tp_hand_back(rx, sl, geom, d_own, stream, lend ? d_next : nullptr);
     if (rc) return rc;
     if (n < n_call && (rc = demod_tail_corner(rx, O, d_x + n, n_call, n_call - n, rx->counter + n, stream)) != SAME_OK) return rc;
-    sl.chunked = true; sl.per_channel = true;
+    sl.chunked = true; sl.per_channel = true; sl.linked = lend;
     sl.geom = geom;
     sl.end_blocks = rx->counter + n;
     tp.last_chunks = n_chunks; tp.last_per_channel = true;
@@ -2192,6 +2211,8 @@
 }
 uint32_t same_batch_time_parallel_chunks(const same_batch *rx) { return rx ? rx->tp.last_chunks : 0; }
 int same_batch_transport_on_device(const same_batch *rx) { return rx && rx->last_dev_transport ? 1 : 0; }
+uint32_t same_batch_time_parallel_lent_columns(const same_batch *rx) { return rx && rx->tp.last_per_channel ? rx->tp.last_lent : 0; }
+uint32_t same_batch_time_parallel_longest_column(const same_batch *rx) { return rx && rx->tp.last_per_channel ? rx->tp.last_longest : 0; }
 int same_batch_time_parallel_per_channel(const same_batch *rx) { return rx && rx->tp.last_chunks > 1u && rx->tp.last_per_channel ? 1 : 0; }
 
 const char *same_batch_kernel_name(const same_batch *rx)
@@ -2219,7 +2240,7 @@
         if (ok && h.chunked) {
             hand0.resize(h.n_bins);
             ok = std::fread(hand0.data(), sizeof(uint64_t), h.n_bins, f) == h.n_bins;
-            if (ok && h.per_channel) { geom.resize((size_t)2 * h.n_bins); ok = std::fread(geom.data(), sizeof(uint32_t), geom.size(), f) == geom.size(); }
+            if (ok && h.per_channel) { geom.resize(h.per_channel == 2u ? (size_t)4 * h.n_bins + 4 : (size_t)2 * h.n_bins); ok = std::fread(geom.data(), sizeof(uint32_t), geom.size(), f) == geom.size(); }
         }
     }
     std::fclose(f);
@@ -2230,7 +2251,8 @@
             ok = (ev0[i].burst_slot == 0xffffffffu || ev0[i].burst_slot < h.n_bursts) && (ev0[i].kind == same::kDevEventNone || ev0[i].kind <= 8u);
         if (ok && h.chunked) {
             ok = h.geom.n_chunks >= 1 && (uint64_t)h.geom.n_chunks * h.n_channels == h.n_bins && h.geom.block_len >= 1 && h.geom.stride_blocks >= 1;
-            for (size_t i = 0; ok && h.per_channel && i < geom.size(); ++i) ok = geom[i] <= 0x7fffffffu;
+            for (size_t i = 0; ok && h.per_channel && i < (size_t)2 * h.n_bins; ++i) ok = geom[i] <= 0x7fffffffu;
+            for (size_t i = (size_t)3 * h.n_bins + 4; ok && i < geom.size(); ++i) ok = geom[i] < h.n_bins || geom[i] == 0xffffffffu;
         } else if (ok) {
             ok = h.n_bins == h.n_channels;
         }
@@ -2247,7 +2269,7 @@
     same_batch::Slot &sl = rx->slot[0];
     ev = ev0; hand = hand0;
     const HarvestInput in{first.data(), ev.data(), bursts.data(), hand.data(), geom.data()};
-    sl.chunked = h.chunked != 0; sl.per_channel = h.per_channel != 0; sl.sort_bins = h.n_bins;
+    sl.chunked = h.chunked != 0; sl.per_channel = h.per_channel != 0; sl.linked = h.per_channel == 2u; sl.sort_bins = h.n_bins;
     const uint64_t span = h.end_counter - h.geom.counter0;
     const double sps = (double)h.input_rate / 520.83;
     const uint64_t span_sym = (uint64_t)((double)span / sps);
diff --git a/sameold_amd/csrc/same_device.h b/sameold_amd/csrc/same_device.h
--- a/sameold_amd/csrc/same_device.h
+++ b/sameold_amd/csrc/same_device.h
@@ -108,6 +108,8 @@
     float *hist_scratch;
     uint64_t in_samples;
     uint32_t whole_samples;
+    const uint32_t *col_cin;
+    const uint32_t *col_next;
 };
 
 struct ChunkGeom {
diff --git a/sameold_amd/csrc/same_kernels.hip b/sameold_amd/csrc/same_kernels.hip
--- a/sameold_amd/csrc/same_kernels.hip
+++ b/sameold_amd/csrc/same_kernels.hip
@@ -5,6 +5,7 @@
 #include "same_dev_common.h"
 #include "same_device.h"
 #include "same_launch.h"
+#include "same_tp_plan.h"
 
 namespace same {
 
@@ -496,27 +497,28 @@
     return hipGetLastError();
 }
 __global__ void chunk_final_column_pc_kernel(const uint64_t *handover, const uint32_t *own_start, uint32_t C, uint32_t K,
-                                             uint64_t counter0, uint32_t *final_col)
+                                             uint64_t counter0, uint32_t *final_col, const uint32_t *__restrict__ col_next)
 {
     const uint32_t c = blockIdx.x * blockDim.x + threadIdx.x;
     if (c >= C) return;
-    uint32_t cur = 0;
-    for (;;) {
-        const uint64_t h = handover[(size_t)cur * C + c];
+    auto next_of = [&](uint32_t v) -> uint32_t { return col_next ? col_next[v] : (v + C < K * C ? v + C : 0xffffffffu); };
+    uint32_t cur = c;
+    for (uint32_t hops = 0; hops < 64u; ++hops) {
+        const uint64_t h = handover[cur];
         if (h == kNoHandover) break;
-        uint32_t nxt = cur;
-        for (uint32_t k = cur + 1u; k < K; ++k)
-            if (counter0 + own_start[(size_t)k * C + c] <= h) nxt = k;
-        if (nxt <= cur) break;
+        uint32_t nxt = cur, v = next_of(cur);
+        for (uint32_t n = 0; v < K * C && n < 64u; v = next_of(v), ++n)
+            if (counter0 + own_start[v] <= h) nxt = v;
+        if (nxt == cur) break;
         cur = nxt;
     }
-    final_col[c] = cur * C + c;
+    final_col[c] = cur;
 }
 hipError_t launch_chunk_final_column_pc(const uint64_t *handover, const uint32_t *own_start, uint32_t in_channels, uint32_t n_chunks,
-                                        uint64_t counter0, uint32_t *final_col, hipStream_t stream)
+                                        uint64_t counter0, uint32_t *final_col, hipStream_t stream, const uint32_t *col_next)
 {
     hipLaunchKernelGGL(chunk_final_column_pc_kernel, dim3((in_channels + 255) / 256), dim3(256), 0, stream, handover, own_start,
-                       in_channels, n_chunks, counter0, final_col);
+                       in_channels, n_chunks, counter0, final_col, col_next);
     return hipGetLastError();
 }
 #ifndef SAME_SCOUT_BLOCK
@@ -540,27 +542,50 @@
     e += __shfl_xor(e, 2);
     if (live && q == 0u) energy[i] = e;
 }
-__global__ __launch_bounds__(kWave) void tp_boundaries_kernel(const float *__restrict__ energy, TpPlan g, uint32_t *__restrict__ own_start,
-                                                               uint32_t *__restrict__ row0, uint32_t *__restrict__ nominal)
+struct TpScratch {
+    int *excess, *bad, *n_cols, *lent;
+    uint32_t *slot0_need, *slot_column;
+    uint16_t *min_limit;
+    int16_t *lastq;
+};
+__host__ __device__ inline size_t tp_align4(size_t words) { return (words + 3u) & ~(size_t)3u; }
+static TpScratch tp_carve(uint32_t *w, const TpPlan &g)
+{
+    const size_t NB1 = tp_align4((size_t)g.scout_blocks + 1u), C = tp_align4(g.channels);
+    TpScratch t{};
+    t.excess = reinterpret_cast<int *>(w); w += NB1;
+    t.bad = reinterpret_cast<int *>(w); w += NB1;
+    t.n_cols = reinterpret_cast<int *>(w); w += C;
+    t.slot0_need = w; w += C;
+    t.lent = reinterpret_cast<int *>(w); w += C;
+    t.slot_column = w; w += tp_align4((size_t)g.n_chunks * g.channels);
+    t.min_limit = reinterpret_cast<uint16_t *>(w); w += (size_t)g.channels * 32u;
+    t.lastq = reinterpret_cast<int16_t *>(w);
+    return t;
+}
+size_t tp_lend_scratch_words(const TpPlan &g)
+{
+    return 2u * tp_align4((size_t)g.scout_blocks + 1u) + 3u * tp_align4(g.channels) + tp_align4((size_t)g.n_chunks * g.channels) +
+           (size_t)g.channels * 32u + tp_align4(((size_t)g.channels * g.scout_blocks + 1u) / 2u);
+}
+constexpr int kTpTop = tp::kMaxPieces + 1;
+__global__ __launch_bounds__(kWave) void tp_boundaries_kernel(const float *__restrict__ energy, TpPlan g, TpScratch w, int lend)
 {
     extern __shared__ float tp_lds[];
     const uint32_t c = blockIdx.x, lane = threadIdx.x;
     const int NB = (int)g.scout_blocks, K = (int)g.n_chunks;
     float *e = tp_lds;
     int *lastq = reinterpret_cast<int *>(tp_lds + NB);
-    int *cut = lastq + NB;
-    constexpr int kQuietBefore = 2048 / (int)kScoutBlock, kQuietAfter = 1;
+    constexpr int kQuietBefore = tp::kQuietSamples / (int)kScoutBlock;
     float m = 0.0f;
     for (int j = (int)lane; j < NB; j += (int)kWave) { const float v = energy[(size_t)c * NB + j]; e[j] = v; m = fmaxf(m, v); }
     for (int off = 32; off > 0; off >>= 1) m = fmaxf(m, __shfl_xor(m, off));
-    const float thr = 0.08f * m;
+    const float thr = tp::quiet_threshold(m);
     __syncthreads();
     const int S = (NB + (int)kWave - 1) / (int)kWave, j0 = (int)lane * S, j1 = min(j0 + S, NB);
     int run = -1;
     for (int j = j0; j < j1; ++j) {
-        bool ok = j - kQuietBefore >= 0 && j + kQuietAfter < NB;
-        if (ok) for (int t = j - kQuietBefore; t <= j + kQuietAfter; ++t) if (e[t] > thr) { ok = false; break; }
-        if (ok) run = j;
+        if (tp::allowed(e, NB, j, thr, kQuietBefore)) run = j;
         lastq[j] = run;
     }
     int before = run;
@@ -569,49 +594,148 @@
     if (lane == 0) before = -1;
     for (int j = j0; j < j1; ++j) if (lastq[j] < 0) lastq[j] = before;
     __syncthreads();
-    const uint32_t kB = g.block_len;
-    const int min_blocks = 2;
-    auto plan = [&](int L, bool store, bool forced) __attribute__((always_inline)) {
-        int pos = 0, n = 1;
-        while (NB - pos > L) {
-            int q = lastq[min(pos + L, NB - 1)];
-            if (q < pos + min_blocks) { if (!forced) return 1 << 20; q = pos + L; }
-            if (q > NB - min_blocks) q = NB - min_blocks;
-            if (q <= pos) return 1 << 20;
-            if (n < 64 && store) cut[n] = q;
-            pos = q; ++n;
-            if (n > K) return n;
+    for (int j = (int)lane; j < NB; j += (int)kWave) w.lastq[(size_t)c * NB + j] = (int16_t)lastq[j];
+    uint16_t *ml = w.min_limit + (size_t)c * 64u;
+    if (tp::needs_forced_cuts(lastq, NB, K)) {
+        int lo = tp::lowest_limit(NB, K), hi = NB;
+        while (lo < hi) {
+            const int step = (hi - lo + (int)kWave - 1) / (int)kWave;
+            const int cand = lo + step * (int)lane;
+            const bool ok = cand >= hi || tp::greedy(lastq, NB, cand, K, true, (int *)nullptr) <= K;
+            const unsigned long long okm = __builtin_amdgcn_ballot_w64(ok);
+            if (okm == 0ull) { lo += step * ((int)kWave - 1) + 1; continue; }
+            const int first = __builtin_ctzll(okm);
+            hi = min(lo + step * first, hi);
+            if (first > 0) lo += step * (first - 1) + 1;
         }
-        return n;
-    };
-    const bool forced = plan(NB - 1, false, false) > K;
-    int lo = (NB + K - 1) / K, hi = NB;
-    while (lo < hi) {
-        const int step = (hi - lo + (int)kWave - 1) / (int)kWave;
-        const int cand = lo + step * (int)lane;
-        const bool ok = cand >= hi || plan(cand, false, forced) <= K;
-        const unsigned long long okm = __builtin_amdgcn_ballot_w64(ok);
-        if (okm == 0ull) { lo += step * ((int)kWave - 1) + 1; continue; }
-        const int first = __builtin_ctzll(okm);
-        hi = min(lo + step * first, hi);
-        if (first > 0) lo += step * (first - 1) + 1;
-    }
-    int used = 0;
-    if (lane == 0) used = plan(lo, true, forced);
-    used = __shfl(used, 0);
+        if (lane == 0) { ml[0] = 1; ml[K] = (uint16_t)lo; }
+        return;
+    }
+    if (lane == 0) ml[0] = 0;
+    auto need = [&](int n) { return n < kTpTop ? tp::need_of(n, K) : 0; };
+    auto spare = [&](int n) { return n < kTpTop ? tp::spare_of(n, K, false) : 0; };
+    int prev = -1;
+    for (int base = tp::lowest_limit(NB, K); base <= NB; base += (int)kWave) {
+        const int L = base + (int)lane;
+        int n = 1;
+        if (L <= NB) n = min(tp::greedy(lastq, NB, L, tp::kMaxPieces, false, (int *)nullptr), kTpTop);
+        int left = __shfl_up(n, 1);
+        if (lane == 0) left = prev;
+        if (L <= NB && left != n) {
+            for (int k = n; k < (left < 0 ? kTpTop : left); ++k) ml[k] = (uint16_t)L;
+            if (lend) {
+                const int d = (need(n) - spare(n)) - (left < 0 ? 0 : need(left) - spare(left));
+                const int db = (n == kTpTop ? 1 : 0) - (left == kTpTop ? 1 : 0);
+                if (d) atomicAdd(&w.excess[L], d);
+                if (db) atomicAdd(&w.bad[L], db);
+            }
+        }
+        prev = __shfl(n, (int)kWave - 1);
+        if (prev <= 1) break;
+    }
+}
+constexpr uint32_t kSortThreads = 1024;
+__device__ __forceinline__ int tp_block_scan(int v, int *wave_sum, int *total)
+{
+    const uint32_t tid = threadIdx.x, lane = tid & (kWave - 1u), wave = tid / kWave;
+    int incl = v;
+    for (int off = 1; off < (int)kWave; off <<= 1) { const int t = __shfl_up(incl, off); if ((int)lane >= off) incl += t; }
     __syncthreads();
-    auto own = [&](int k) __attribute__((always_inline)) -> uint32_t {
-        const int i = k < used ? k : used - 1;
-        uint32_t p = (k >= 1 && i >= 1) ? (uint32_t)cut[i] * kScoutBlock : 0u;
-        return p - p % kB;
-    };
-    for (int k = (int)lane; k < K; k += (int)kWave) {
-        const uint32_t p = own(k);
-        const uint32_t r = (k == 0 || p < g.warmup_samples) ? 0u : p - g.warmup_samples;
-        const size_t v = (size_t)k * g.channels + c;
-        own_start[v] = p;
-        row0[v] = r;
-        nominal[v] = k + 1 < K ? (own(k + 1) - r + kB - 1u) / kB : 0xffffffffu;
+    if (lane == kWave - 1u) wave_sum[wave] = incl;
+    __syncthreads();
+    int before = incl - v, all = 0;
+    for (uint32_t k = 0; k < kSortThreads / kWave; ++k) { const int t = wave_sum[k]; if (k < wave) before += t; all += t; }
+    *total = all;
+    return before;
+}
+__global__ __launch_bounds__(kSortThreads) void tp_lend_kernel(TpPlan g, TpScratch w, uint32_t *__restrict__ info, int lend)
+{
+    __shared__ int wave_sum[kSortThreads / kWave];
+    __shared__ int s_limit;
+    const int tid = (int)threadIdx.x, NB = (int)g.scout_blocks, K = (int)g.n_chunks, C = (int)g.channels;
+    int limit = 0;
+    if (lend) {
+        const int lo0 = tp::lowest_limit(NB, K), per = (NB - lo0 + 1 + (int)kSortThreads - 1) / (int)kSortThreads;
+        const int L0 = lo0 + tid * per, L1 = min(L0 + per, NB + 1);
+        int se = 0, sb = 0, te, tb;
+        for (int L = L0; L < L1; ++L) { se += w.excess[L]; sb += w.bad[L]; }
+        int pe = tp_block_scan(se, wave_sum, &te), pb = tp_block_scan(sb, wave_sum, &tb);
+        if (tid == 0) s_limit = NB;
+        __syncthreads();
+        for (int L = L0; L < L1; ++L) {
+            pe += w.excess[L]; pb += w.bad[L];
+            if (pe <= 0 && pb == 0) { atomicMin(&s_limit, L); break; }
+        }
+        __syncthreads();
+        limit = s_limit;
+    }
+    int total = 0;
+    for (int c0 = 0; c0 < C; c0 += (int)kSortThreads) {
+        const int c = c0 + tid;
+        int n = K;
+        if (c < C && lend) {
+            const uint16_t *ml = w.min_limit + (size_t)c * 64u;
+            const uint4 lo = reinterpret_cast<const uint4 *>(ml)[0], hi = reinterpret_cast<const uint4 *>(ml)[1];
+            const uint32_t word[8] = {lo.x, lo.y, lo.z, lo.w, hi.x, hi.y, hi.z, hi.w};
+            if ((word[0] & 0xffffu) == 0u) {
+                n = 16;
+                for (int k = 15; k >= 1; --k)
+                    if ((int)((word[k >> 1] >> (16 * (k & 1))) & 0xffffu) <= limit) n = k;
+                while (n >= 16 && n < tp::kMaxPieces && (int)ml[n] > limit) ++n;
+            }
+        }
+        if (c < C) w.n_cols[c] = n;
+        int t;
+        tp_block_scan(c < C ? tp::need_of(n, K) : 0, wave_sum, &t);
+        total += t;
+    }
+    int need_before = 0, spare_before = 0;
+    for (int c0 = 0; c0 < C; c0 += (int)kSortThreads) {
+        const int c = c0 + tid;
+        const int n = c < C ? w.n_cols[c] : K;
+        const bool forced = c < C && w.min_limit[(size_t)c * 64u] != 0;
+        const int nd = c < C ? tp::need_of(n, K) : 0, sp = (c < C && lend) ? tp::spare_of(n, K, forced) : 0;
+        int tn, ts;
+        const int pn = need_before + tp_block_scan(nd, wave_sum, &tn), ps = spare_before + tp_block_scan(sp, wave_sum, &ts);
+        need_before += tn; spare_before += ts;
+        if (c < C) {
+            const int g0 = min(total, ps), given = min(total, ps + sp) - g0;
+            w.slot0_need[c] = (uint32_t)pn;
+            w.lent[c] = given;
+            w.n_cols[c] = K + nd - given;
+            for (int j = 0; j < given; ++j) w.slot_column[g0 + j] = tp::lent_column(c, j, given, C, K);
+        }
+    }
+    if (tid == 0) { info[0] = (uint32_t)limit; info[1] = (uint32_t)total; }
+}
+__global__ void tp_columns_kernel(TpPlan g, TpScratch w, uint32_t *__restrict__ own_start, uint32_t *__restrict__ row0,
+                                  uint32_t *__restrict__ nominal, uint32_t *__restrict__ col_cin, uint32_t *__restrict__ col_next)
+{
+    const int c = (int)(blockIdx.x * blockDim.x + threadIdx.x), C = (int)g.channels, K = (int)g.n_chunks, NB = (int)g.scout_blocks;
+    if (c >= C) return;
+    const uint16_t *ml = w.min_limit + (size_t)c * 64u;
+    const int16_t *lq = w.lastq + (size_t)c * NB;
+    const bool forced = ml[0] != 0;
+    const int n = w.n_cols[c], lent = w.lent[c], L = forced ? (int)ml[K] : (int)ml[n];
+    const uint32_t slot0 = w.slot0_need[c], kB = g.block_len;
+    auto at = [&](int cut) -> uint32_t { const uint32_t s = (uint32_t)cut * kScoutBlock; return s - s % kB; };
+    int cut = 0;
+    bool ended = false;
+    uint32_t col = (uint32_t)c, own = 0u;
+    for (int i = 0; i < n; ++i) {
+        int nxt = cut;
+        if (!ended) {
+            const int q = tp::greedy_next(lq, NB, L, forced, cut);
+            if (q > 0) nxt = q; else ended = true;
+        }
+        if (col >= (uint32_t)(K * C)) break;
+        const uint32_t r = tp::first_row(own, i, g.warmup_samples);
+        const uint32_t ncol = i + 1 < n ? tp::column_of(c, i + 1, n, lent, slot0, w.slot_column, C, K) : tp::kNoColumn;
+        own_start[col] = own;
+        row0[col] = r;
+        nominal[col] = i + 1 < n ? tp::nominal_blocks(r, at(nxt), kB) : 0xffffffffu;
+        if (col_cin) { col_cin[col] = (uint32_t)c; col_next[col] = ncol; }
+        cut = nxt; own = at(nxt); col = ncol;
     }
 }
 constexpr uint32_t kSortBuckets = 4096, kSortBucketBlocks = 4;
@@ -624,7 +748,6 @@
     const uint32_t len = *group == 0u ? avail : min(nominal[v], avail);
     *bucket = kSortBuckets - 1u - min(len / kSortBucketBlocks, kSortBuckets - 1u);
 }
-constexpr uint32_t kSortThreads = 1024;
 __global__ __launch_bounds__(kSortThreads) void tp_sort_kernel(TpPlan g, const uint32_t *__restrict__ row0, const uint32_t *__restrict__ nominal,
                                                                 uint32_t *__restrict__ perm)
 {
@@ -668,19 +791,22 @@
     if (i < n) perm[i] = i;
 }
 __global__ void tp_align_kernel(TpPlan g, const uint32_t *__restrict__ perm, uint32_t *__restrict__ row0, const uint32_t *__restrict__ nominal,
-                                uint32_t *__restrict__ wg_blocks, uint32_t *__restrict__ wg_len)
+                                uint32_t *__restrict__ wg_blocks, uint32_t *__restrict__ wg_len, uint32_t *__restrict__ info,
+                                uint32_t *__restrict__ col_cin)
 {
     const uint32_t v = perm[blockIdx.x * kWave + threadIdx.x];
+    if (col_cin && col_cin[v] >= g.channels) col_cin[v] = v % g.channels;
     const uint32_t chunk = v / g.channels;
     uint32_t avail = (g.whole_samples - row0[v]) / g.block_len;
     uint32_t m = avail;
     for (int off = 32; off > 0; off >>= 1) m = max(m, (uint32_t)__shfl_xor((int)m, off));
     if (chunk + 1u == g.n_chunks) row0[v] = g.whole_samples - m * g.block_len;
     if (threadIdx.x == 0) wg_blocks[blockIdx.x] = m;
-    if (wg_len) {
-        uint32_t len = chunk + 1u == g.n_chunks ? m : min(nominal[v], avail);
-        for (int off = 32; off > 0; off >>= 1) len = max(len, (uint32_t)__shfl_xor((int)len, off));
-        if (threadIdx.x == 0) wg_len[blockIdx.x] = len;
+    uint32_t len = chunk + 1u == g.n_chunks ? m : min(nominal[v], avail);
+    for (int off = 32; off > 0; off >>= 1) len = max(len, (uint32_t)__shfl_xor((int)len, off));
+    if (threadIdx.x == 0) {
+        if (wg_len) wg_len[blockIdx.x] = len;
+        atomicMax(&info[2], len * g.block_len);
     }
 }
 __global__ void tp_wg_order_kernel(uint32_t n_wg, const uint32_t *__restrict__ perm, const uint32_t *__restrict__ wg_blocks,
@@ -698,19 +824,28 @@
 }
 hipError_t launch_tp_plan(const float *x, const TpPlan &g, float *energy, uint32_t *own_start, uint32_t *row0,
                           uint32_t *nominal, uint32_t *perm, uint32_t *wg_blocks, bool sorted, hipStream_t stream,
-                          uint32_t *perm_out, uint32_t *wg_blocks_out, bool pairs)
+                          const TpLend &lend, uint32_t *perm_out, uint32_t *wg_blocks_out, bool pairs)
 {
     const size_t n = (size_t)g.channels * g.scout_blocks;
     const uint32_t columns = g.n_chunks * g.channels;
+    if (g.scout_blocks > 32767u || g.n_chunks > (uint32_t)tp::kMaxPieces || g.n_chunks < 2u) return hipErrorInvalidValue;
+    const TpScratch w = tp_carve(lend.scratch, g);
+    hipError_t e = hipMemsetAsync(w.excess, 0, 2u * tp_align4((size_t)g.scout_blocks + 1u) * sizeof(int), stream);
+    if (e == hipSuccess) e = hipMemsetAsync(lend.info, 0, 4u * sizeof(uint32_t), stream);
+    if (e != hipSuccess) return e;
     hipLaunchKernelGGL(tp_scout_kernel, dim3((unsigned)((4 * n + 255) / 256)), dim3(256), 0, stream, x, g, energy);
-    hipLaunchKernelGGL(tp_boundaries_kernel, dim3(g.channels), dim3(kWave), (size_t)g.scout_blocks * 8 + 64 * sizeof(int), stream, energy, g, own_start, row0, nominal);
+    hipLaunchKernelGGL(tp_boundaries_kernel, dim3(g.channels), dim3(kWave), (size_t)g.scout_blocks * 8, stream, energy, g, w, lend.lend ? 1 : 0);
+    hipLaunchKernelGGL(tp_lend_kernel, dim3(1), dim3(kSortThreads), 0, stream, g, w, lend.info, lend.lend ? 1 : 0);
+    hipLaunchKernelGGL(tp_columns_kernel, dim3((g.channels + kWave - 1u) / kWave), dim3(kWave), 0, stream, g, w, own_start, row0, nominal,
+                       lend.lend ? lend.col_cin : nullptr, lend.lend ? lend.col_next : nullptr);
     if (sorted) {
         hipLaunchKernelGGL(tp_sort_kernel, dim3(1), dim3(kSortThreads), 0, stream, g, row0, nominal, perm);
     } else {
         hipLaunchKernelGGL(tp_iota_kernel, dim3((columns + 255) / 256), dim3(256), 0, stream, perm, columns);
     }
     uint32_t *wg_len = perm_out ? wg_blocks_out + columns / kWave : nullptr;
-    hipLaunchKernelGGL(tp_align_kernel, dim3(columns / kWave), dim3(kWave), 0, stream, g, perm, row0, nominal, wg_blocks, wg_len);
+    hipLaunchKernelGGL(tp_align_kernel, dim3(columns / kWave), dim3(kWave), 0, stream, g, perm, row0, nominal, wg_blocks, wg_len, lend.info,
+                       lend.lend ? lend.col_cin : nullptr);
     if (perm_out)
         hipLaunchKernelGGL(tp_wg_order_kernel, dim3(columns / kWave), dim3(kWave), 0, stream, columns / kWave, perm, wg_blocks, wg_len,
                            perm_out, wg_blocks_out, pairs ? 1u : 0u);
diff --git a/sameold_amd/csrc/same_kernels_pipe.hip b/sameold_amd/csrc/same_kernels_pipe.hip
--- a/sameold_amd/csrc/same_kernels_pipe.hip
+++ b/sameold_amd/csrc/same_kernels_pipe.hip
@@ -575,7 +575,7 @@
         Cin = K.in_channels;
         if (K.col_row0) {
             const uint32_t chunk_l = c / Cin;
-            cin = c - chunk_l * Cin;
+            cin = K.col_cin ? K.col_cin[c] : c - chunk_l * Cin;
             may_leave = (uint32_t)__builtin_amdgcn_readfirstlane((int)chunk_l) + 1u < K.n_chunks;
             const uint32_t row_abs = K.col_row0[c];
             xl = x + (size_t)cin * K.in_samples + row_abs;
diff --git a/sameold_amd/csrc/same_kernels_relaxed.hip b/sameold_amd/csrc/same_kernels_relaxed.hip
--- a/sameold_amd/csrc/same_kernels_relaxed.hip
+++ b/sameold_amd/csrc/same_kernels_relaxed.hip
@@ -78,7 +78,7 @@
     if constexpr (CM) {
         Cin = K.in_channels;
         const uint32_t chunk_l = c / Cin;
-        cin = c - chunk_l * Cin;
+        cin = K.col_cin ? K.col_cin[c] : c - chunk_l * Cin;
         may_leave = (uint32_t)__builtin_amdgcn_readfirstlane((int)chunk_l) + 1u < K.n_chunks;
         const uint32_t row_abs = K.col_row0[c];
         xl = reinterpret_cast<const float *>(x) + (size_t)cin * K.in_samples + row_abs;
@@ -361,7 +361,7 @@
     if constexpr (CM) {
         Cin = K.in_channels;
         const uint32_t chunk_l = c / Cin;
-        cin = c - chunk_l * Cin;
+        cin = K.col_cin ? K.col_cin[c] : c - chunk_l * Cin;
         may_leave = (uint32_t)__builtin_amdgcn_readfirstlane((int)chunk_l) + 1u < K.n_chunks;
         const uint32_t row_abs = K.col_row0[c];
         xl = reinterpret_cast<const float *>(x) + (size_t)cin * K.in_samples + row_abs;
diff --git a/sameold_amd/csrc/same_kernels_sym.hip b/sameold_amd/csrc/same_kernels_sym.hip
--- a/sameold_amd/csrc/same_kernels_sym.hip
+++ b/sameold_amd/csrc/same_kernels_sym.hip
@@ -938,7 +938,7 @@
         Cin = K.in_channels;
         if (K.col_row0) {
             const uint32_t chunk_l = c / Cin;
-            cin = c - chunk_l * Cin;
+            cin = K.col_cin ? K.col_cin[c] : c - chunk_l * Cin;
             may_leave = (uint32_t)__builtin_amdgcn_readfirstlane((int)chunk_l) + 1u < K.n_chunks;
             const uint32_t row_abs = K.col_row0[c];
             xl = x + (size_t)cin * K.in_samples + row_abs;
diff --git a/sameold_amd/csrc/same_launch.h b/sameold_amd/csrc/same_launch.h
--- a/sameold_amd/csrc/same_launch.h
+++ b/sameold_amd/csrc/same_launch.h
@@ -50,7 +50,7 @@
 hipError_t launch_chunk_final_column(const uint64_t *handover, uint32_t in_channels, ChunkGeom g, uint32_t *final_col,
                                      hipStream_t stream);
 hipError_t launch_chunk_final_column_pc(const uint64_t *handover, const uint32_t *own_start, uint32_t in_channels, uint32_t n_chunks,
-                                        uint64_t counter0, uint32_t *final_col, hipStream_t stream);
+                                        uint64_t counter0, uint32_t *final_col, hipStream_t stream, const uint32_t *col_next = nullptr);
 hipError_t launch_fill_u64(uint64_t *p, size_t n, uint64_t v, hipStream_t stream);
 hipError_t launch_cast_i16_f32(const int16_t *in, float *out, size_t n, hipStream_t stream);
 hipError_t launch_tp_prologue(void *blob, const void *fresh, size_t bytes, uint64_t *handover, uint32_t *sort_cnt, uint32_t n_cols,
@@ -61,9 +61,14 @@
     uint64_t in_samples;
     uint32_t scout_blocks;
 };
+struct TpLend {
+    uint32_t *scratch, *col_cin, *col_next, *info;
+    bool lend;
+};
+size_t tp_lend_scratch_words(const TpPlan &g);
 hipError_t launch_tp_plan(const float *x, const TpPlan &g, float *energy, uint32_t *own_start, uint32_t *row0,
                           uint32_t *nominal, uint32_t *perm, uint32_t *wg_blocks, bool sorted, hipStream_t stream,
-                          uint32_t *perm_out = nullptr, uint32_t *wg_blocks_out = nullptr, bool pairs = false);
+                          const TpLend &lend, uint32_t *perm_out = nullptr, uint32_t *wg_blocks_out = nullptr, bool pairs = false);
 hipError_t launch_transpose(const float *in, float *out, uint32_t n_channels, uint32_t n_samples,
                             hipStream_t stream);
 hipError_t launch_transpose(const int16_t *in, int16_t *out, uint32_t n_channels, uint32_t n_samples,
diff --git a/sameold_amd/csrc/same_tp_plan.h b/sameold_amd/csrc/same_tp_plan.h
--- /dev/null
+++ b/sameold_amd/csrc/same_tp_plan.h
@@ -0,0 +1,144 @@
+#ifndef SAME_TP_PLAN_H
+#define SAME_TP_PLAN_H
+
+#include <cstdint>
+
+#if defined(__HIPCC__)
+#define SAME_TP_HD __host__ __device__ inline
+#else
+#define SAME_TP_HD inline
+#endif
+
+namespace same {
+namespace tp {
+
+constexpr int kQuietSamples = 2048;
+constexpr int kQuietAfter = 1;
+constexpr int kMinBlocks = 1;
+constexpr int kMinBlocksForced = 2;
+constexpr int kMaxPieces = 63;
+constexpr int kInfeasible = 1 << 20;
+constexpr uint32_t kNoColumn = 0xffffffffu;
+
+SAME_TP_HD float quiet_threshold(float loudest) { return 0.08f * loudest; }
+
+SAME_TP_HD bool allowed(const float *e, int NB, int j, float thr, int quiet_before)
+{
+    if (j - quiet_before < 0 || j + kQuietAfter >= NB) return false;
+    for (int t = j - quiet_before; t <= j + kQuietAfter; ++t)
+        if (e[t] > thr) return false;
+    return true;
+}
+
+SAME_TP_HD void quiet_table(const float *e, int NB, int quiet_before, int *lastq)
+{
+    float m = 0.0f;
+    for (int j = 0; j < NB; ++j) m = e[j] > m ? e[j] : m;
+    const float thr = quiet_threshold(m);
+    int run = -1;
+    for (int j = 0; j < NB; ++j) {
+        if (allowed(e, NB, j, thr, quiet_before)) run = j;
+        lastq[j] = run;
+    }
+}
+
+template <typename Q>
+SAME_TP_HD int greedy_next(const Q *lastq, int NB, int L, bool forced, int pos)
+{
+    if (NB - pos <= L) return 0;
+    int q = (int)lastq[pos + L < NB - 1 ? pos + L : NB - 1];
+    if (q < pos + (forced ? kMinBlocksForced : kMinBlocks)) { if (!forced) return -1; q = pos + L; }
+    if (q > NB - kMinBlocksForced) q = NB - kMinBlocksForced;
+    return q > pos ? q : -1;
+}
+template <typename Q>
+SAME_TP_HD int greedy(const Q *lastq, int NB, int L, int cap, bool forced, int *cut)
+{
+    int pos = 0, n = 1;
+    for (;;) {
+        const int q = greedy_next(lastq, NB, L, forced, pos);
+        if (q == 0) return n;
+        if (q < 0) return kInfeasible;
+        if (n <= kMaxPieces && cut) cut[n] = q;
+        pos = q; ++n;
+        if (n > cap) return n;
+    }
+}
+
+template <typename Q>
+SAME_TP_HD bool needs_forced_cuts(const Q *lastq, int NB, int K) { return greedy(lastq, NB, NB - 1, K, false, (int *)nullptr) > K; }
+
+SAME_TP_HD int lowest_limit(int NB, int K) { return (NB + K - 1) / K; }
+
+template <typename Q>
+SAME_TP_HD int own_limit(const Q *lastq, int NB, int n, int K, bool forced)
+{
+    int lo = (NB + n - 1) / n, hi = NB;
+    if (lo < lowest_limit(NB, K)) lo = lowest_limit(NB, K);
+    while (lo < hi) {
+        const int mid = lo + (hi - lo) / 2;
+        if (greedy(lastq, NB, mid, n, forced, (int *)nullptr) <= n) hi = mid; else lo = mid + 1;
+    }
+    return lo;
+}
+
+template <typename Q>
+SAME_TP_HD int pieces_at(const Q *lastq, int NB, int L, int K, bool forced)
+{
+    if (forced) return K;
+    const int n = greedy(lastq, NB, L, kMaxPieces, false, (int *)nullptr);
+    return n > kMaxPieces ? kInfeasible : n;
+}
+SAME_TP_HD int spare_of(int n, int K, bool forced) { return (forced || n >= K) ? 0 : K - (n > 2 ? n : 2); }
+SAME_TP_HD int need_of(int n, int K) { return n > K ? n - K : 0; }
+
+SAME_TP_HD uint32_t own_sample(const int *cut, int used, int i, uint32_t scout_block, uint32_t block_len)
+{
+    const int p = i < used ? i : used - 1;
+    const uint32_t s = (i >= 1 && p >= 1) ? (uint32_t)cut[p] * scout_block : 0u;
+    return s - s % block_len;
+}
+SAME_TP_HD uint32_t first_row(uint32_t own, int i, uint32_t warmup_samples)
+{
+    return (i == 0 || own < warmup_samples) ? 0u : own - warmup_samples;
+}
+SAME_TP_HD uint32_t nominal_blocks(uint32_t row0, uint32_t next_own, uint32_t block_len) { return (next_own - row0 + block_len - 1u) / block_len; }
+
+SAME_TP_HD bool fits(const int *pieces, const uint8_t *forced, int C, int K)
+{
+    long long need = 0, spare = 0;
+    for (int c = 0; c < C; ++c) {
+        if (pieces[c] >= kInfeasible) return false;
+        need += need_of(pieces[c], K);
+        spare += spare_of(pieces[c], K, forced[c] != 0);
+    }
+    return need <= spare;
+}
+
+SAME_TP_HD uint32_t lend(const int *pieces, const uint8_t *forced, int C, int K, int *n_cols, uint32_t *slot0_need, uint32_t *slot0_lent,
+                         int *lent)
+{
+    uint32_t total = 0;
+    for (int c = 0; c < C; ++c) { slot0_need[c] = total; total += (uint32_t)need_of(pieces[c], K); }
+    uint32_t given = 0;
+    for (int c = 0; c < C; ++c) {
+        const uint32_t s = (uint32_t)spare_of(pieces[c], K, forced[c] != 0);
+        const uint32_t g = total - given < s ? total - given : s;
+        slot0_lent[c] = given; lent[c] = (int)g; given += g;
+        n_cols[c] = K + need_of(pieces[c], K) - (int)g;
+    }
+    return total;
+}
+SAME_TP_HD uint32_t lent_column(int c, int j, int lent, int C, int K) { return (uint32_t)(K - 1 - lent + j) * (uint32_t)C + (uint32_t)c; }
+
+SAME_TP_HD uint32_t column_of(int c, int i, int n_cols, int lent, uint32_t slot0_need, const uint32_t *slot_column, int C, int K)
+{
+    if (i == n_cols - 1) return (uint32_t)(K - 1) * (uint32_t)C + (uint32_t)c;
+    const int own_before_last = K - 1 - lent;
+    if (i < own_before_last) return (uint32_t)i * (uint32_t)C + (uint32_t)c;
+    return slot_column[slot0_need + (uint32_t)(i - own_before_last)];
+}
+
+}
+}
+#endif
diff --git a/sameold_amd/receiver.py b/sameold_amd/receiver.py
--- a/sameold_amd/receiver.py
+++ b/sameold_amd/receiver.py
@@ -164,6 +164,8 @@
     sig("same_batch_time_parallel_config", C.c_int, vp, u32, u32, u32)
     sig("same_batch_time_parallel_chunks", u32, vp)
     sig("same_batch_time_parallel_per_channel", C.c_int, vp)
+    sig("same_batch_time_parallel_lent_columns", C.c_uint32, vp)
+    sig("same_batch_time_parallel_longest_column", C.c_uint32, vp)
     sig("same_batch_transport_on_device", C.c_int, vp)
     sig("same_batch_set_audio_capture", C.c_int, vp, C.c_size_t)
     sig("same_batch_peek_audio", C.c_int, vp, P(P(AudioChunk)), P(C.c_size_t))
@@ -380,6 +382,12 @@
 
     def time_parallel_per_channel(self) -> bool:
         return bool(self._L.same_batch_time_parallel_per_channel(self._h))
+
+    def time_parallel_lent_columns(self) -> int:
+        return int(self._L.same_batch_time_parallel_lent_columns(self._h))
+
+    def time_parallel_longest_column(self) -> int:
+        return int(self._L.same_batch_time_parallel_longest_column(self._h))
 
     def set_audio_capture(self, samples_per_launch: int) -> None:
         _check(self._L.same_batch_set_audio_capture(self._h, int(samples_per_launch)))
```
